# VUmcCGP/wisecondor

Measured on NVIDIA B200. Metric: newref_bin_pairs_per_s, higher is better.
Workload: dtype f64

## Files before the change

### wisecondor_b200/csrc/wc_common.cuh

```cuda
#pragma once
#include <cuda.h>
#include <cuda_runtime.h>
#include <stdint.h>
#include <stdio.h>
#include <string.h>
#include <math.h>
#include <string>
#include <vector>
#include <algorithm>
#include "../../include/wisecondor_b200.h"

void wc_set_error(const char* fmt, ...);

#define WC_CUDA(expr)                                                                                   \
    do {                                                                                                \
        cudaError_t _e = (expr);                                                                        \
        if (_e != cudaSuccess) {                                                                        \
            wc_set_error("%s failed: %s (%s:%d)", #expr, cudaGetErrorString(_e), __FILE__, __LINE__);   \
            return WC_ERR_CUDA;                                                                         \
        }                                                                                               \
    } while (0)

#define WC_CHECK_ARG(cond)                                                                              \
    do {                                                                                                \
        if (!(cond)) {                                                                                  \
            wc_set_error("bad argument: %s (%s:%d)", #cond, __FILE__, __LINE__);                        \
            return WC_ERR_ARG;                                                                          \
        }                                                                                               \
    } while (0)

struct wc_buf {
    void* p = nullptr;
    size_t bytes = 0;
};

enum { WC_NBUF = 56, WC_NPHASE = 12, WC_NCOUNTER = 12 };

enum {
    SLOT_XC = 0, SLOT_NORMS, SLOT_ROWCS, SLOT_ROWCE, SLOT_RBMETA, SLOT_CAND_D, SLOT_CAND_J, SLOT_SEGCNT,
    SLOT_SEGFLAG, SLOT_SLOW, SLOT_SCRATCH, SLOT_IO_X, SLOT_IO_IDX, SLOT_IO_DIST, SLOT_ROWTHR,
    SLOT_IN_KEY, SLOT_IN_J, SLOT_IN_CNT, SLOT_N32, SLOT_F16STAT,
    SLOT_PROF = 20, SLOT_PIV_IDS = 21, SLOT_PIV_X = 22, SLOT_PIV_N = 23, SLOT_PIV_META = 37, SLOT_S_STACK = 38,
    SLOT_T_COPY = 24, SLOT_T_ZT, SLOT_T_RT, SLOT_T_NT, SLOT_T_SD, SLOT_T_FLAGS, SLOT_T_TOTALS, SLOT_T_PROJ,
    SLOT_T_REVCNT = 44, SLOT_T_REVCUR, SLOT_T_DIRTY, SLOT_T_PAIRS,
    SLOT_S_ZC = 32, SLOT_S_META, SLOT_S_STATUS, SLOT_S_RC, SLOT_S_AUX,
    SLOT_P_FIRST = 40,
    SLOT_FIN_J = 48, SLOT_FIN_D, SLOT_FIN_P, SLOT_FIN_GRP
};

struct wc_shard_plan {
    int valid = 0;
    int N = 0, S = 0, k = 0, cap = 0, in_cap = 0, world = 1, rank = 0;
    int nb = 0, bp = 0, b0 = 0, b1 = 0;
    int row0 = 0, row1 = 0, rows_per = 0;
    int nkc = 0, nd_last = 0, extra_h = 0, ld = 0, nstages = 0, nrb = 0, nseg = 0, gridA = 0, gridB = 0;
    size_t Npad = 0, smem = 0, nlistA = 0;
    long long tilesA = 0, tilesB = 0, tiles_plain = 0;
    double mcoef = 0.0, madd = 0.0;
    int f16 = 0, ldh = 0;
    int pivots = 0;
    const double* corrected = nullptr;
    const unsigned long long* thr = nullptr;
    int stage = 0;
};

struct wc_ctx {
    int device = 0;
    int sm_count = 0;
    wc_buf buf[WC_NBUF];
    cudaEvent_t ev[2 * WC_NPHASE];
    double phase_ms[WC_NPHASE];
    long long counter[WC_NCOUNTER];
    const int* zs_npairs_d = nullptr;
    int zs_repeats = 0;
    long long zs_pair_limit = 0, zs_all_pairs = 0;
    int32_t* d2h_idx_h = nullptr; double* d2h_dist_h = nullptr; size_t d2h_rows_done = 0;
    cudaStream_t d2h_stream = nullptr; cudaEvent_t d2h_ev = nullptr;
    void* search_plan = nullptr;
    void (*search_plan_free)(void*) = nullptr;
    unsigned long long sched_hash = 0;
    unsigned timed_mask = 0;
    int k5_stages = 0;
    int k5_group = 0;
    int k5_sym = 8;
    int k5_f16 = 2;
    int k5_f16_checked = 1;
    int k5_pivots = 1;
    unsigned long long piv_hash = 0;
    float* dbg_scores = nullptr;
    int dbg_ld = 0;
    const int* k6_stats_d = nullptr;
    int k6_g4 = 0;
    int k6_parts = 4;
    int k6_select = 1;
    int k6_split = 1;
    int k6_chunk = 0, k6_warps = 0, k6_prod = 0;
    int k5_lag = 0;
    int debug_profile = 0;
    void* encode_tiled = nullptr;
    wc_shard_plan shard;
};

int wc_reserve(wc_ctx* ctx, int slot, size_t bytes, void** out);

__device__ __forceinline__ uint32_t smem_u32(const void* p) {
    return static_cast<uint32_t>(__cvta_generic_to_shared(p));
}

__device__ __forceinline__ void mbar_init(uint64_t* bar, uint32_t count) {
    asm volatile("mbarrier.init.shared::cta.b64 [%0], %1;" ::"r"(smem_u32(bar)), "r"(count) : "memory");
}
__device__ __forceinline__ void mbar_fence_init() {
    asm volatile("fence.mbarrier_init.release.cluster;" ::: "memory");
}
__device__ __forceinline__ void mbar_arrive(uint64_t* bar) {
    asm volatile("mbarrier.arrive.shared::cta.b64 _, [%0];" ::"r"(smem_u32(bar)) : "memory");
}
__device__ __forceinline__ void mbar_arrive_expect_tx(uint64_t* bar, uint32_t bytes) {
    asm volatile("mbarrier.arrive.expect_tx.shared::cta.b64 _, [%0], %1;" ::"r"(smem_u32(bar)), "r"(bytes) : "memory");
}
__device__ __forceinline__ bool mbar_try_wait(uint64_t* bar, uint32_t parity) {
    uint32_t ok;
    asm volatile(
        "{\n"
        ".reg .pred p;\n"
        "mbarrier.try_wait.parity.shared::cta.b64 p, [%1], %2;\n"
        "selp.u32 %0, 1, 0, p;\n"
        "}\n"
        : "=r"(ok)
        : "r"(smem_u32(bar)), "r"(parity)
        : "memory");
    return ok != 0;
}
__device__ __forceinline__ bool mbar_test_wait(uint64_t* bar, uint32_t parity) {
    uint32_t ok;
    asm volatile(
        "{\n"
        ".reg .pred p;\n"
        "mbarrier.test_wait.parity.shared::cta.b64 p, [%1], %2;\n"
        "selp.u32 %0, 1, 0, p;\n"
        "}\n"
        : "=r"(ok)
        : "r"(smem_u32(bar)), "r"(parity)
        : "memory");
    return ok != 0;
}
__device__ __forceinline__ void mbar_wait(uint64_t* bar, uint32_t parity) {
    while (!mbar_try_wait(bar, parity)) {
    }
}
__device__ __forceinline__ void tma_load_2d(void* smem_dst, const CUtensorMap* map, int c0, int c1, uint64_t* bar) {
    asm volatile(
        "cp.async.bulk.tensor.2d.shared::cluster.global.mbarrier::complete_tx::bytes [%0], [%1, {%2, %3}], [%4];" ::"r"(
            smem_u32(smem_dst)),
        "l"(reinterpret_cast<uint64_t>(map)), "r"(c0), "r"(c1), "r"(smem_u32(bar))
        : "memory");
}
__device__ __forceinline__ void tma_prefetch_desc(const CUtensorMap* map) {
    asm volatile("prefetch.tensormap [%0];" ::"l"(reinterpret_cast<uint64_t>(map)) : "memory");
}
__device__ __forceinline__ double lds_f64(uint32_t addr) {
    double v;
    asm volatile("ld.shared.f64 %0, [%1];" : "=d"(v) : "r"(addr));
    return v;
}
__device__ __forceinline__ void lds_v2f64(uint32_t addr, double& v0, double& v1) {
    asm volatile("ld.shared.v2.f64 {%0, %1}, [%2];" : "=d"(v0), "=d"(v1) : "r"(addr));
}
__device__ __forceinline__ void dmma_8x8x4(double& c0, double& c1, double a, double b) {
    asm("mma.sync.aligned.m8n8k4.row.col.f64.f64.f64.f64 {%0,%1}, {%2}, {%3}, {%0,%1};"
                 : "+d"(c0), "+d"(c1)
                 : "d"(a), "d"(b));
}
__device__ __forceinline__ void named_bar_sync(int id, int nthreads) {
    asm volatile("bar.sync %0, %1;" ::"r"(id), "r"(nthreads) : "memory");
}
__device__ __forceinline__ double ld_cg_f64(const double* p) {
    double v;
    asm volatile("ld.global.cg.f64 %0, [%1];" : "=d"(v) : "l"(p));
    return v;
}
__device__ __forceinline__ int ld_cg_s32(const int* p) {
    int v;
    asm volatile("ld.global.cg.s32 %0, [%1];" : "=r"(v) : "l"(p));
    return v;
}
```

### wisecondor_b200/csrc/wc_search.cu

```cuda
#include "wc_common.cuh"
#include <cuda_fp16.h>

namespace {

typedef unsigned long long u64;

constexpr int BM = 128;
constexpr int BN = 128;
constexpr int BK = 16;
constexpr int CONSUMER_WARPS = 8;
constexpr int CONSUMER_THREADS = CONSUMER_WARPS * 32;
constexpr int WROWS = BM / CONSUMER_WARPS;
constexpr int PRODUCER_WARPS = 4;
constexpr int TOPK_THREADS = CONSUMER_THREADS + PRODUCER_WARPS * 32;
constexpr int TILE_BYTES = BM * BK * 8;
constexpr int STAGE_BYTES = 2 * TILE_BYTES;
constexpr int MAX_STAGES = 6;
constexpr int HIST_BINS = 256;
constexpr int FIN_THREADS = 128;
constexpr int FIN_CHUNK = 32;
constexpr int FIN_BUCKETS = 1024;
constexpr int FIN_ECAP = 1360;
constexpr int EXH_THREADS = 256;
constexpr int STG = 128;
// ... 282 lines not shown
            else
                prune_row<32>(rk, rj, n, a.k, w_nrm[rw], a.mcoef, madd_of(a), lane, w_sk, w_sj, &thr, &kept);
            if (lane == 0) {
                if (kept > a.cap - BN) {
                    w_flag[rw] = 1;
                    w_thr[rw] = KEY_NEVER;
                    w_cnt[rw] = 0;
                } else {
                    const int row = a.row_begin + rb * BM + r0w + rw;
                    const u64 other = atomicMin(a.row_thr + (row - a.row_begin), thr);
                    w_thr[rw] = other < thr ? other : thr;
                    w_cnt[rw] = kept;
                }
            }
            __syncwarp();
        }
    };
    auto flush_incoming = [&]() {
        __syncwarp();
        int n = *w_stgc;
        if (n > STG) n = STG;
        for (int e = lane; e < n; e += 32) {
            const uint4 v = w_stg[e];
            const int j = (int)v.z;
            const int w = atomicAdd(a.in_cnt + j, 1);
            if (w < a.in_cap) {
                a.in_key[(size_t)j * a.in_cap + w] = ((u64)v.y << 32) | (u64)v.x;
                a.in_j[(size_t)j * a.in_cap + w] = (int)v.w;
            }
        }
        __syncwarp();
        if (lane == 0) *w_stgc = 0;
        __syncwarp();
    };
    int tcount = 0;
    while (true) {
        if (q >= q1) {
            __syncwarp();
            if (SYM) flush_incoming();
            if (a.final_prune) {
                const unsigned need = __ballot_sync(0xffffffffu, lane < WROWS && w_cnt[lane] > a.k + 24 &&
                                                                     w_cnt[lane] <= a.cap && !w_flag[lane]);
                prune_rows(need, a.cand_key + (size_t)seg * seg_stride, a.cand_j + (size_t)seg * seg_stride);
            }
            if (lane < WROWS) {
                a.seg_cnt[(size_t)seg * BM + r0w + lane] = w_cnt[lane] > a.cap ? a.cap : w_cnt[lane];
                a.seg_flag[(size_t)seg * BM + r0w + lane] = w_flag[lane];
            }
            if (++pi >= pe) break;
            pc = a.pieces + (size_t)pi * 5;
            rb = pc[0]; q = pc[1]; q1 = pc[2]; qs = pc[3]; seg = pc[4];
            skip_lo = a.rb_skip_lo[rb]; skip_n = a.rb_skip_n[rb];
            tl = a.tile_list ? a.tile_list + a.rb_list_off[rb] : nullptr;
            new_piece = true;
            continue;
        }
        if (new_piece) {
            new_piece = false;
            __syncwarp();
            if (lane < WROWS) {
                const int row = a.row_begin + rb * BM + r0w + lane;
                const bool valid = row < a.row_end;
                w_nrm[lane] = valid ? a.norms[row] : 0.0;
                w_thr[lane] = valid ? __ldcg(a.row_thr + (row - a.row_begin)) : KEY_NEVER;
                w_cnt[lane] = 0;
                w_flag[lane] = 0;
            }
#pragma unroll
            for (int mt = 0; mt < 2; ++mt) {
                const int row = a.row_begin + rb * BM + r0w + mt * 8 + pg;
                const bool valid = row < a.row_end;
                my_cs[mt] = valid ? a.row_cs[row] : 0;
                my_ce[mt] = valid ? a.row_ce[row] : 0;
            }
            __syncwarp();
        }
        const int t = tl ? tl[q] : (q < skip_lo ? q : q + skip_n);
        const int col0 = t * BN;
        q += qs;
        if (SYM) {
            __syncwarp();
            cp_async_16(w_ct + 2 * lane, a.col_thr + col0 + 2 * lane);
            cp_async_16(w_ct + 64 + 2 * lane, a.col_thr + col0 + 64 + 2 * lane);
            cp_async_commit();
        }
        u64 shared_thr = ~0ull;
        if (lane < WROWS) {
            const int row = a.row_begin + rb * BM + r0w + lane;
            if (row < a.row_end) shared_thr = __ldcg(a.row_thr + (row - a.row_begin));
        }
        const bool tr_on = a.trace != nullptr && blockIdx.x == 0 && (warp & 3) == 0 && lane == 0 && tcount < 64;
        long long* tr = tr_on ? a.trace + ((size_t)(warp >> 2) * 64 + tcount) * 4 : nullptr;
        ++tcount;
        if (tr_on) tr[0] = clock64();

        double acc[2][16][2];
#pragma unroll
        for (int mt = 0; mt < 2; ++mt)
#pragma unroll
            for (int nt = 0; nt < 16; ++nt) acc[mt][nt][0] = acc[mt][nt][1] = 0.0;

        for (int kc = 0; kc < a.nkc; ++kc) {
            if (!ready) {
                const long long pf_w0 = clock64();
                mbar_wait(&sm.full[stage], phase);
                pf_wait += clock64() - pf_w0;
            }
            const uint32_t base = tiles_u32 + (uint32_t)stage * STAGE_BYTES;
            int nstage = stage + 1;
            uint32_t nphase = phase;
            if (nstage == STAGES) { nstage = 0; nphase ^= 1u; }
            const bool ready_next = mbar_test_wait(&sm.full[nstage], nphase);
            const bool last = kc == a.nkc - 1;
            const int nd = last ? a.nd_last : 2;
#pragma unroll
            for (int h = 0; h < 2; ++h) {
                if (h < nd) {
                    double fa[2][2];
#pragma unroll
                    for (int mt = 0; mt < 2; ++mt) lds_v2f64(base + a_off + mt * 1024 + sw[h], fa[mt][0], fa[mt][1]);
#pragma unroll
                    for (int half = 0; half < 2; ++half) {
                        double fb[8][2];
#pragma unroll
                        for (int i = 0; i < 8; ++i)
                            lds_v2f64(base + b_off + (half * 8 + i) * 1024 + sw[h], fb[i][0], fb[i][1]);
#pragma unroll
                        for (int u = 0; u < 2; ++u)
#pragma unroll
                            for (int mt = 0; mt < 2; ++mt)
#pragma unroll
                                for (int i = 0; i < 8; ++i)
                                    dmma_8x8x4(acc[mt][half * 8 + i][0], acc[mt][half * 8 + i][1], fa[mt][u], fb[i][u]);
                    }
                }
            }
            if (last) {
                double fa[2][2];
#pragma unroll
                for (int mt = 0; mt < 2; ++mt) lds_v2f64(base + a_off + mt * 1024 + swx, fa[mt][0], fa[mt][1]);
#pragma unroll
                for (int half = 0; half < 2; ++half) {
                    double fb[8][2];
#pragma unroll
                    for (int i = 0; i < 8; ++i)
                        lds_v2f64(base + b_off + (half * 8 + i) * 1024 + swx, fb[i][0], fb[i][1]);
#pragma unroll
                    for (int u = 0; u < 2; ++u)
#pragma unroll
                        for (int mt = 0; mt < 2; ++mt)
#pragma unroll
                            for (int i = 0; i < 8; ++i)
                                dmma_8x8x4(acc[mt][half * 8 + i][0], acc[mt][half * 8 + i][1], fa[mt][u], fb[i][1 - u]);
                }
            }
            __syncwarp();
            if (lane == 0) mbar_arrive(&sm.empty[stage]);
            if (gate_left > 0 && --gate_left == 0) {
                if (lane == 0) mbar_arrive(&sm.gate);
                gate_left = -1;
            }
            stage = nstage;
            phase = nphase;
            ready = ready_next;
        }

        const long long pf_e0 = clock64();
        if (tr_on) tr[1] = pf_e0;
        if (lane < WROWS && shared_thr < w_thr[lane]) w_thr[lane] = shared_thr;
        if (SYM) cp_async_wait<0>();
        __syncwarp();
        u64* ck = a.cand_key + (size_t)seg * seg_stride;
        int* cj = a.cand_j + (size_t)seg * seg_stride;
#pragma unroll
        for (int mt = 0; mt < 2; ++mt) {
            const int rw = mt * 8 + pg;
            const u64 thr = w_thr[rw];
            unsigned mask = 0, cmask = 0;
#pragma unroll
            for (int nt = 0; nt < 16; ++nt) {
#pragma unroll
                for (int e = 0; e < 2; ++e) {
                    const u64 bits = (u64)__double_as_longlong(acc[mt][nt][e]);
                    if (bits <= thr) mask |= 1u << (nt * 2 + e);
                    if (SYM && bits <= w_ct[nt * 8 + 4 * e + q4]) cmask |= 1u << (nt * 2 + e);
                }
            }
            if (mask | cmask) {
                u64* tmp = w_sk + lane;
#pragma unroll
                for (int nt = 0; nt < 16; ++nt) {
                    tmp[(nt * 2) * 32] = (u64)__double_as_longlong(acc[mt][nt][0]);
                    tmp[(nt * 2 + 1) * 32] = (u64)__double_as_longlong(acc[mt][nt][1]);
                }
                const int cs = my_cs[mt];
                const unsigned clen = (unsigned)(my_ce[mt] - cs);
                unsigned m2 = mask;
                while (m2) {
                    const int bit = __ffs(m2) - 1;
                    m2 &= m2 - 1;
                    const int cl = (bit >> 1) * 8 + 4 * (bit & 1) + q4;
                    const unsigned hi32 = (unsigned)(tmp[bit * 32] >> 32);
                    if ((hi32 & 0x7ff00000u) == 0x7ff00000u || (unsigned)(col0 + cl - cs) < clen) mask &= ~(1u << bit);
                }
                if (mask) {
                    pf_emit += __popc(mask);
                    int w = atomicAdd(&w_cnt[rw], __popc(mask));
                    u64* rk = ck + (size_t)(r0w + rw) * a.cap;
                    int* rj = cj + (size_t)(r0w + rw) * a.cap;
                    while (mask) {
                        const int bit = __ffs(mask) - 1;
                        mask &= mask - 1;
                        const int cl = (bit >> 1) * 8 + 4 * (bit & 1) + q4;
                        if (w < a.cap) {
                            rk[w] = tmp[bit * 32];
                            rj[w] = col0 + cl;
                        } else {
                            w_flag[rw] = 1;
                        }
                        ++w;
                    }
                }
                if (SYM && cmask) {
                    const int i = a.row_begin + rb * BM + r0w + rw;
                    while (cmask) {
                        const int bit = __ffs(cmask) - 1;
                        cmask &= cmask - 1;
                        const int j = col0 + (bit >> 1) * 8 + 4 * (bit & 1) + q4;
                        const u64 key = tmp[bit * 32];
                        if (((unsigned)(key >> 32) & 0x7ff00000u) == 0x7ff00000u || j >= a.N || i >= a.row_end) continue;
                        if ((unsigned)(j - cs) < clen) continue;
                        const int pos = atomicAdd(w_stgc, 1);
                        if (pos < STG) {
                            w_stg[pos] = make_uint4((unsigned)key, (unsigned)(key >> 32), (unsigned)j, (unsigned)i);
                        } else {
                            const int w = atomicAdd(a.in_cnt + j, 1);
                            if (w < a.in_cap) {
                                a.in_key[(size_t)j * a.in_cap + w] = key;
                                a.in_j[(size_t)j * a.in_cap + w] = i;
                            }
                        }
                        ++pf_emit;
                    }
                }
            }
        }
        __syncwarp();
        if (SYM && *w_stgc >= 32) flush_incoming();
        const long long pf_p0 = clock64();
        pf_epi += pf_p0 - pf_e0;
        if (tr_on) tr[2] = pf_p0;
        prune_rows(__ballot_sync(0xffffffffu, lane < WROWS && w_cnt[lane] > a.cap - BN && !w_flag[lane]), ck, cj);
        pf_prune += clock64() - pf_p0;
        if (tr_on) tr[3] = clock64();
    }
    if (gate_left > 0 && lane == 0) mbar_arrive(&sm.gate);
    __syncwarp();
    if (a.prof != nullptr && warp == 0 && lane == 0) {
        long long* o = a.prof + (size_t)blockIdx.x * 8;
        o[0] = clock64() - pf_t0; o[1] = pf_wait; o[2] = pf_epi; o[3] = pf_prune;
        o[4] = tcount; o[5] = pf_nprune; o[6] = pf_emit; o[7] = 0;
    }
}

#include "wc_search_f16.cuh"
#include "wc_search_tc.cuh"

__global__ void wc_fill_u64_kernel(u64* p, size_t n, u64 v) {
    const size_t i = (size_t)blockIdx.x * blockDim.x + threadIdx.x;
    if (i < n) p[i] = v;
}

__global__ void wc_prepare_kernel(const double* __restrict__ X, int N, int Npad, int S, int ld, int Sx,
                                  double* __restrict__ Xc, double* __restrict__ norms) {
    const int row = (blockIdx.x * blockDim.x + threadIdx.x) >> 5;
    const int lane = threadIdx.x & 31;
    if (row >= Npad) return;
    double* dst = Xc + (size_t)row * ld;
    double acc = 0.0;
    if (row < N) {
        const double* src = X + (size_t)row * S;
        for (int s = lane; s < ld; s += 32) {
            double v = s < S ? src[s] - 1.0 : 0.0;
            dst[s] = v;
            acc = fma(v, v, acc);
        }
    } else {
        for (int s = lane; s < ld; s += 32) dst[s] = 0.0;
    }
#pragma unroll
    for (int o = 16; o > 0; o >>= 1) acc += __shfl_xor_sync(0xffffffffu, acc, o);
    __syncwarp();
    if (lane == 0) {
        norms[row] = row < N ? acc : 0.0;
        dst[Sx] = 1.0;
        dst[Sx + 1] = row < N ? -0.5 * acc : -INFINITY;
    }
}

__device__ __forceinline__ bool pair_less(double da, int ja, double db, int jb) {
    return da < db || (da == db && ja < jb);
}

struct FinArgs {
    const double* X;
    int N, S;
    const double* norms;
    const int* row_cs;
    const int* row_ce;
    int row_begin, row_end;
    const int* rb_seg_first;
    const int* rb_seg_count;
    const u64* cand_key;
    const int* cand_j;
    const int* seg_cnt;
    const int* seg_flag;
    int cap;
    int k;
    int shortcap;
    double mcoef;
    int* idx_out;
    double* dist_out;
    int* slow_list;
    int* slow_count;
    int slow_bias;
    int vec;
    const u64* in_key;
    const int* in_j;
    const int* in_cnt;
    int in_cap;
    double madd;
    const double* madd_p;
    const u64* row_thr;
    int in_nsrc;
    int in_src_rows;
    int* sl_j;
    u64* sl_k;
    int* sl_p;
    int* grp;
    int* grp_count;
    const int* row_list;
    const int* row_count;
    int* stats;
    int* sl_b;
    int* bkt_hist;
    int bkt_shift;
};

template <int FT, bool SPLIT>
__device__ __forceinline__ void finalize_row(const FinArgs& a, const int rloc, unsigned char* fin_raw) {
    constexpr int ecap = FIN_ECAP;
    double* ex_d = reinterpret_cast<double*>(fin_raw + (size_t)ecap * 12);
    int* ex_j = reinterpret_cast<int*>(ex_d + a.shortcap);
    int* hist = ex_j + a.shortcap;
    __shared__ double s_red[2][FT / 32];
    __shared__ int s_total, s_flag, s_p, s_bstar, s_valid;

    const int tid = threadIdx.x, lane = tid & 31, warp = tid >> 5;
    const int row = a.row_begin + rloc;
    const int rb = rloc / BM, rl = rloc % BM;
    const int seg0 = a.rb_seg_first[rb], nseg = a.rb_seg_count[rb];
    int* out_i = a.idx_out + (size_t)rloc * a.k;
    double* out_d = a.dist_out + (size_t)rloc * a.k;

    const int nsrc = nseg + (a.in_key != nullptr ? a.in_nsrc : 0);
    auto source = [&](int s, const u64*& keys, const int*& js, int& flagged) -> int {
        if (s < nseg) {
            const size_t off = ((size_t)(seg0 + s) * BM + rl) * a.cap;
            keys = a.cand_key + off;
            js = a.cand_j + off;
            flagged = a.seg_flag[(size_t)(seg0 + s) * BM + rl];
            return a.seg_cnt[(size_t)(seg0 + s) * BM + rl];
        }
        const size_t r = (size_t)(s - nseg) * a.in_src_rows + rloc;
        keys = a.in_key + r * a.in_cap;
        js = a.in_j + r * a.in_cap;
        const int n = a.in_cnt[r];
        flagged = n > a.in_cap ? 1 : 0;
        return n < a.in_cap ? n : a.in_cap;
    };
    u64* en_k = reinterpret_cast<u64*>(fin_raw);
    int* en_j = reinterpret_cast<int*>(en_k + ecap);
    if (tid == 0) { s_total = 0; s_flag = 0; s_p = 0; s_valid = 0; }
    for (int b = tid; b < HIST_BINS; b += FT) hist[b] = 0;
    const u64 tfinal = a.row_thr != nullptr ? __ldcg(a.row_thr + rloc) : ~0ull;
    __syncthreads();
    for (int s = warp; s < nsrc; s += FT / 32) {
        const u64* cd;
        const int* cjs;
        int fl;
        const int n = source(s, cd, cjs, fl);
        if (fl) { if (lane == 0) s_flag = 1; continue; }
        for (int e0 = 0; e0 < n; e0 += 32) {
            const int e = e0 + lane;
            const u64 key = e < n ? cd[e] : ~0ull;
            const bool keep = e < n && key <= tfinal;
            const unsigned bm = __ballot_sync(0xffffffffu, keep);
            if (bm == 0u) continue;
            int base = 0;
            if (lane == 0) base = atomicAdd(&s_total, __popc(bm));
            base = __shfl_sync(0xffffffffu, base, 0) + __popc(bm & ((1u << lane) - 1u));
            if (keep && base < ecap) {
                en_k[base] = key;
                en_j[base] = cjs[e];
            }
        }
    }
    __syncthreads();
    const int total = s_total;
    if (s_flag) {
        if (tid == 0) {
            a.slow_list[atomicAdd(a.slow_count, 1)] = rloc + a.slow_bias;
            if (SPLIT) a.sl_p[rloc] = -1;
        }
        return;
    }
    if (total == 0) {
        for (int e = tid; e < a.k; e += FT) { out_i[e] = -1; out_d[e] = 1e10; }
        if (SPLIT && tid == 0) a.sl_p[rloc] = -1;
        return;
    }
    const bool in_smem = total <= ecap;
    auto for_each_entry = [&](auto&& f) {
        if (in_smem) {
            for (int e = tid; e < total; e += FT) f(en_k[e], en_j[e]);
        } else {
            for (int s2 = 0; s2 < nsrc; ++s2) {
                const u64* cd;
                const int* cjs;
                int fl;
                const int n = source(s2, cd, cjs, fl);
                for (int e = tid; e < n; e += FT) {
                    const u64 key = cd[e];
                    if (key <= tfinal) f(key, cjs[e]);
                }
            }
        }
    };

    double mn = INFINITY, mx = -INFINITY;
    for_each_entry([&](u64 key, int) {
        const double d = dist_of_key(key);
        mn = fmin(mn, d);
        mx = fmax(mx, d);
    });
    mn = warp_min(mn);
    mx = warp_max(mx);
    if (lane == 0) { s_red[0][warp] = mn; s_red[1][warp] = mx; }
    __syncthreads();
#pragma unroll
    for (int w = 0; w < FT / 32; ++w) { mn = fmin(mn, s_red[0][w]); mx = fmax(mx, s_red[1][w]); }
    const float scale = (mx > mn) ? (float)(HIST_BINS - 1) / (float)(mx - mn) : 0.0f;
    for_each_entry([&](u64 key, int) { atomicAdd(&hist[bucket_of(dist_of_key(key), mn, scale)], 1); });
    __syncthreads();
    if (warp == 0) {
        int c[HIST_BINS / 32], sum = 0;
#pragma unroll
        for (int t = 0; t < HIST_BINS / 32; ++t) { c[t] = hist[lane * (HIST_BINS / 32) + t]; sum += c[t]; }
        int incl = sum;
#pragma unroll
        for (int o = 1; o < 32; o <<= 1) {
            int v = __shfl_up_sync(0xffffffffu, incl, o);
            if (lane >= o) incl += v;
        }
        int run = incl - sum, bl = -1;
#pragma unroll
        for (int t = 0; t < HIST_BINS / 32; ++t) {
            run += c[t];
            if (bl < 0 && run >= a.k) bl = lane * (HIST_BINS / 32) + t;
        }
        unsigned m = __ballot_sync(0xffffffffu, bl >= 0);
        int bstar = HIST_BINS - 1;
        if (m) bstar = __shfl_sync(0xffffffffu, bl, __ffs(m) - 1);
        if (lane == 0) s_bstar = bstar;
    }
    __syncthreads();
    const int bstar = s_bstar;
    double vstar = -INFINITY;
    for_each_entry([&](u64 key, int) {
        const double d = dist_of_key(key);
        if (bucket_of(d, mn, scale) <= bstar) vstar = fmax(vstar, d);
    });
    vstar = warp_max(vstar);
    __syncthreads();
    if (lane == 0) s_red[0][warp] = vstar;
    __syncthreads();
#pragma unroll
    for (int w = 0; w < FT / 32; ++w) vstar = fmax(vstar, s_red[0][w]);
    const double window = vstar + a.mcoef * (a.norms[row] + fabs(vstar)) + madd_of(a);
    for_each_entry([&](u64 key, int j) {
        if (dist_of_key(key) <= window) {
            const int slot = atomicAdd(&s_p, 1);
            if (slot < a.shortcap) ex_j[slot] = j;
        }
    });
    __syncthreads();
    const int p = s_p;
    if (p > a.shortcap) {
        if (tid == 0) {
            a.slow_list[atomicAdd(a.slow_count, 1)] = rloc + a.slow_bias;
            if (SPLIT) a.sl_p[rloc] = -1;
        }
        return;
    }
    if (SPLIT) {
        for (int e = tid; e < p; e += FT) a.sl_j[(size_t)rloc * a.shortcap + e] = ex_j[e];
        if (tid == 0) {
            a.sl_p[rloc] = p;
            const int ng = (p + 31) >> 5;
            int jmin = 0x7fffffff;
            for (int e = 0; e < p; ++e) jmin = min(jmin, ex_j[e]);
            const int bkt = min(jmin >> a.bkt_shift, FIN_BUCKETS - 1);
            a.sl_b[rloc] = bkt;
            atomicAdd(a.bkt_hist + bkt, ng);
            if (a.stats != nullptr) { atomicAdd(a.stats, total); atomicAdd(a.stats + 1, p); }
        }
        return;
    }

    const double* xrow = a.X + (size_t)row * a.S;
    double* xi_s = reinterpret_cast<double*>(fin_raw);
    const bool xi_in_smem = (size_t)a.S * 8 <= (size_t)ecap * 12;
    __syncthreads();
    if (xi_in_smem)
        for (int t = tid; t < a.S; t += FT) xi_s[t] = xrow[t];
    __syncthreads();
    const uint32_t xi_u32 = smem_u32(xi_s);
    for (int c0 = 0; c0 < p; c0 += FT) {
        if (c0 + warp * 32 < p) {
            const bool live = c0 + tid < p;
            const int j = ex_j[live ? c0 + tid : p - 1];
            const double* xr = a.X + (size_t)j * a.S;
            double accd = 0.0;
            int t0 = 0;
            if (a.vec == 4 && xi_in_smem) {
                for (; t0 + 32 <= a.S; t0 += 32) {
                    double v[32];
#pragma unroll
                    for (int u = 0; u < 8; ++u) ldg_nc_v4f64(xr + t0 + 4 * u, v[4 * u], v[4 * u + 1], v[4 * u + 2], v[4 * u + 3]);
                    __syncwarp();
#pragma unroll
                    for (int u = 0; u < 16; ++u) {
                        double x0, x1;
                        lds_v2f64(xi_u32 + (uint32_t)(t0 + 2 * u) * 8u, x0, x1);
                        double d = __dsub_rn(v[2 * u], x0);
                        accd = __dadd_rn(accd, __dmul_rn(d, d));
                        d = __dsub_rn(v[2 * u + 1], x1);
                        accd = __dadd_rn(accd, __dmul_rn(d, d));
                    }
                }
                for (; t0 + 4 <= a.S; t0 += 4) {
                    double v0, v1, v2, v3;
                    ldg_nc_v4f64(xr + t0, v0, v1, v2, v3);
                    double d = __dsub_rn(v0, xi_s[t0]);     accd = __dadd_rn(accd, __dmul_rn(d, d));
                    d = __dsub_rn(v1, xi_s[t0 + 1]);        accd = __dadd_rn(accd, __dmul_rn(d, d));
                    d = __dsub_rn(v2, xi_s[t0 + 2]);        accd = __dadd_rn(accd, __dmul_rn(d, d));
                    d = __dsub_rn(v3, xi_s[t0 + 3]);        accd = __dadd_rn(accd, __dmul_rn(d, d));
                }
            }
            if (xi_in_smem) {
                for (; t0 < a.S; ++t0) {
                    const double d = __dsub_rn(__ldg(xr + t0), xi_s[t0]);
                    accd = __dadd_rn(accd, __dmul_rn(d, d));
                }
            } else {
                for (; t0 < a.S; ++t0) {
                    const double d = __dsub_rn(__ldg(xr + t0), __ldg(xrow + t0));
                    accd = __dadd_rn(accd, __dmul_rn(d, d));
                }
            }
            __syncwarp();
            if (live) {
                const bool ok = accd < 1e10;
                ex_d[c0 + tid] = ok ? accd : INFINITY;
                ex_j[c0 + tid] = ok ? j : 0x7fffffff;
            }
        }
    }
    __syncthreads();

    const int cs = a.row_cs[row], ce = a.row_ce[row];
    int nvalid_local = 0;
    for (int e = tid; e < p; e += FT) {
        const double d = ex_d[e];
        const int j = ex_j[e];
        if (j == 0x7fffffff) continue;
        ++nvalid_local;
        int rank = 0;
        for (int u = 0; u < p; ++u) rank += pair_less(ex_d[u], ex_j[u], d, j) ? 1 : 0;
        if (rank < a.k) {
            out_i[rank] = j >= ce ? j - (ce - cs) : j;
            out_d[rank] = d;
        }
    }
    atomicAdd(&s_valid, nvalid_local);
    __syncthreads();
    for (int e = s_valid + tid; e < a.k; e += FT) { out_i[e] = -1; out_d[e] = 1e10; }
}

template <int FT, bool SPLIT>
__global__ void __launch_bounds__(FT) wc_finalize_kernel(const FinArgs a) {
    extern __shared__ __align__(32) unsigned char fin_raw[];
    if (a.row_list == nullptr) {
        finalize_row<FT, SPLIT>(a, (int)blockIdx.x, fin_raw);
        return;
    }
    const int n = *a.row_count;
    for (int b = blockIdx.x; b < n; b += gridDim.x) {
        finalize_row<FT, SPLIT>(a, a.row_list[b], fin_raw);
        __syncthreads();
    }
}

struct ExhArgs {
    const double* X;
    int N, S;
    const int* row_cs;
    const int* row_ce;
    int row_begin;
    const int* slow_list;
    int list_off;
    double* scratch;
    int k;
    int* idx_out;
    double* dist_out;
};

__global__ void __launch_bounds__(EXH_THREADS) wc_exhaustive_kernel(const ExhArgs a) {
    __shared__ double s_d[EXH_THREADS / 32];
    __shared__ int s_j[EXH_THREADS / 32];
    __shared__ double s_bd;
    __shared__ int s_bj;
    const int tid = threadIdx.x, lane = tid & 31, warp = tid >> 5;
    const int rloc = a.slow_list[a.list_off + blockIdx.x];
    const int row = a.row_begin + rloc;
    const int cs = a.row_cs[row], ce = a.row_ce[row];
    double* dd = a.scratch + (size_t)blockIdx.x * a.N;
    const double* xrow = a.X + (size_t)row * a.S;
    for (int j = tid; j < a.N; j += EXH_THREADS) {
        double acc = INFINITY;
        if (j < cs || j >= ce) {
            const double* xj = a.X + (size_t)j * a.S;
            acc = 0.0;
            for (int s = 0; s < a.S; ++s) {
                double v = __dsub_rn(xj[s], xrow[s]);
                acc = __dadd_rn(acc, __dmul_rn(v, v));
            }
            if (!(acc < 1e10)) acc = INFINITY;
        }
        dd[j] = acc;
    }
    __syncthreads();
    double last_d = -INFINITY;
    int last_j = -1;
    int* out_i = a.idx_out + (size_t)rloc * a.k;
    double* out_d = a.dist_out + (size_t)rloc * a.k;
    for (int t = 0; t < a.k; ++t) {
        double bd = INFINITY;
        int bj = 0x7fffffff;
        for (int j = tid; j < a.N; j += EXH_THREADS) {
            double d = dd[j];
            bool after = d > last_d || (d == last_d && j > last_j);
            if (after && pair_less(d, j, bd, bj)) { bd = d; bj = j; }
        }
#pragma unroll
        for (int o = 16; o > 0; o >>= 1) {
            double od = __shfl_xor_sync(0xffffffffu, bd, o);
            int oj = __shfl_xor_sync(0xffffffffu, bj, o);
            if (pair_less(od, oj, bd, bj)) { bd = od; bj = oj; }
        }
        if (lane == 0) { s_d[warp] = bd; s_j[warp] = bj; }
        __syncthreads();
        if (tid == 0) {
            for (int w = 1; w < EXH_THREADS / 32; ++w)
                if (pair_less(s_d[w], s_j[w], bd, bj)) { bd = s_d[w]; bj = s_j[w]; }
            s_bd = bd;
            s_bj = bj;
            if (bd < INFINITY) {
                out_i[t] = bj >= ce ? bj - (ce - cs) : bj;
                out_d[t] = bd;
            } else {
                out_i[t] = -1;
                out_d[t] = 1e10;
            }
        }
        __syncthreads();
        last_d = s_bd;
        last_j = s_bj;
        if (!(last_d < INFINITY)) {
            for (int e = t + 1 + tid; e < a.k; e += EXH_THREADS) { out_i[e] = -1; out_d[e] = 1e10; }
            break;
        }
    }
}

typedef CUresult (*PFN_encodeTiled)(CUtensorMap*, CUtensorMapDataType, cuuint32_t, void*, const cuuint64_t*,
                                    const cuuint64_t*, const cuuint32_t*, const cuuint32_t*, CUtensorMapInterleave,
                                    CUtensorMapSwizzle, CUtensorMapL2promotion, CUtensorMapFloatOOBfill);

}

namespace {
#include "wc_search_fin.cuh"

struct Piece { int cta, rb, q0, q1, step, seg, pass; };
void schedule_pieces(const std::vector<int>& prefix, int nrb, int grid, int G, bool rounds_on, int pass,
                     std::vector<Piece>& pieces) {
    std::vector<long long> load(grid, 0);
    if (G > grid) G = grid;
    if (G < 1) G = 1;
    const int groups = grid / G;
    const int rounds = rounds_on ? nrb / groups : 0;
    for (int r = 0; r < rounds; ++r)
        for (int g = 0; g < groups; ++g) {
            const int rb = r * groups + g;
            const int nv = prefix[rb + 1] - prefix[rb];
            for (int j = 0; j < G && j < nv; ++j) {
                pieces.push_back({g * G + j, rb, j, nv, G, 0, pass});
                load[g * G + j] += (nv - j + G - 1) / G;
            }
        }
    const int rb_left = rounds * groups;
    long long left = prefix[nrb] - prefix[rb_left];
    if (left > 0) {
        long long lo = 0, hi = 0;
        for (int c = 0; c < grid; ++c) hi = std::max(hi, load[c]);
        hi += left;
        while (lo < hi) {
            const long long mid = (lo + hi) / 2;
            long long cap_sum = 0;
            for (int c = 0; c < grid; ++c) cap_sum += std::max(0ll, mid - load[c]);
            if (cap_sum >= left) hi = mid; else lo = mid + 1;
        }
        int rb = rb_left, q = 0;
        for (int c = 0; c < grid && left > 0; ++c) {
            long long want = std::min(left, std::max(0ll, lo - load[c]));
            while (want > 0) {
                const int nv = prefix[rb + 1] - prefix[rb];
                if (q >= nv) { ++rb; q = 0; continue; }
                const int take = (int)std::min<long long>(want, nv - q);
                pieces.push_back({c, rb, q, q + take, 1, 0, pass});
                load[c] += take;
                q += take;
                want -= take;
                left -= take;
            }
        }
    }
}

void pair_lists(int nb, const std::vector<int>& skip_lo, const std::vector<int>& skip_n, int frac, int b0, int b1,
                std::vector<int>& list_a, std::vector<int>& off_a, std::vector<int>& list_b, std::vector<int>& off_b) {
    auto in_sample = [&](int I, int J) { return I == J || (I + J) % frac == 0; };
    auto valid = [&](int I, int t) { return !(t >= skip_lo[I] && t < skip_lo[I] + skip_n[I]); };
    list_a.clear();
    list_b.clear();
    off_a.assign(b1 - b0 + 1, 0);
    off_b.assign(b1 - b0 + 1, 0);
    for (int I = b0; I < b1; ++I) {
        for (int t = 0; t < nb; ++t)
            if (valid(I, t) && in_sample(I, t)) list_a.push_back(t);
        off_a[I - b0 + 1] = (int)list_a.size();
        for (int dlt = 1; dlt <= nb / 2; ++dlt) {
            if (2 * dlt == nb && I >= nb / 2) continue;
            const int t = (I + dlt) % nb;
            if (valid(I, t) && !in_sample(I, t)) list_b.push_back(t);
        }
        off_b[I - b0 + 1] = (int)list_b.size();
    }
}

void block_skips(int N, const int* chrom_bins_h, int nchrom, std::vector<int>& row_cs, std::vector<int>& row_ce,
                 std::vector<int>& skip_lo, std::vector<int>& skip_n) {
    row_cs.assign(N, 0);
    row_ce.assign(N, 0);
    int pos = 0;
    for (int c = 0; c < nchrom; ++c) {
        for (int i = 0; i < chrom_bins_h[c]; ++i) { row_cs[pos + i] = pos; row_ce[pos + i] = pos + chrom_bins_h[c]; }
        pos += chrom_bins_h[c];
    }
    const int nb = (N + BM - 1) / BM;
    skip_lo.assign(nb, nb);
    skip_n.assign(nb, 0);
    for (int I = 0; I < nb; ++I) {
        const int r0 = I * BM, r1 = std::min(N, r0 + BM) - 1;
        if (row_cs[r0] == row_cs[r1]) {
            const int first = (row_cs[r0] + BN - 1) / BN, last = row_ce[r0] / BN;
            if (last > first) { skip_lo[I] = first; skip_n[I] = last - first; }
        }
    }
}

}


namespace {
int encode_f16_map(wc_ctx* ctx, CUtensorMap* tmap, const void* base, int ldh, size_t rows) {
    if (!ctx->encode_tiled) {
        wc_set_error("cuTensorMapEncodeTiled is not available from this driver");
        return WC_ERR_CUDA;
    }
    cuuint64_t dims[2] = {(cuuint64_t)ldh, (cuuint64_t)rows};
    cuuint64_t strides[1] = {(cuuint64_t)ldh * sizeof(__half)};
    cuuint32_t box[2] = {(cuuint32_t)BKH, BM};
    cuuint32_t estr[2] = {1, 1};
    CUresult r = reinterpret_cast<PFN_encodeTiled>(ctx->encode_tiled)(
        tmap, CU_TENSOR_MAP_DATA_TYPE_FLOAT16, 2, const_cast<void*>(base), dims, strides, box, estr, CU_TENSOR_MAP_INTERLEAVE_NONE,
        CU_TENSOR_MAP_SWIZZLE_128B, CU_TENSOR_MAP_L2_PROMOTION_L2_256B, CU_TENSOR_MAP_FLOAT_OOB_FILL_NONE);
    if (r != CUDA_SUCCESS) {
        wc_set_error("cuTensorMapEncodeTiled failed with CUresult %d", (int)r);
        return WC_ERR_CUDA;
    }
    return WC_OK;
}

int pivot_count(int N, int k) {
    return (k <= 128 && (long long)TC_PIVOTS * 4 <= N) ? TC_PIVOTS : 0;
}

int tc_pivot_pass(wc_ctx* ctx, cudaStream_t stream, const CUtensorMap& tmap_a, TopkArgs ta, const __half* Xh, int ldh, int ldx, int N,
                  int nrb, const std::vector<int>& rb_seg_first, int R) {
    int* ids; __half* P; float* n32p; int* meta;
    int rc;
    if ((rc = wc_reserve(ctx, SLOT_PIV_IDS, (size_t)R * sizeof(int), (void**)&ids))) return rc;
    if ((rc = wc_reserve(ctx, SLOT_PIV_X, (size_t)R * ldh * sizeof(__half), (void**)&P))) return rc;
    if ((rc = wc_reserve(ctx, SLOT_PIV_N, (size_t)R * sizeof(float), (void**)&n32p))) return rc;
    if (R != TC_PIVOTS) { wc_set_error("pivot pass: %d pivots unsupported", R); return WC_ERR_INTERNAL; }
    const int gridP = std::max(1, std::min(ctx->sm_count, nrb));
    std::vector<int> m((size_t)gridP + 1 + (size_t)nrb * 5);
    {
        int w = 0;
        for (int c = 0; c < gridP; ++c) {
            m[c] = w;
            for (int rb = c; rb < nrb; rb += gridP, ++w) {
                int* pc = &m[(size_t)gridP + 1 + (size_t)w * 5];
                pc[0] = rb; pc[1] = 0; pc[2] = R / BN; pc[3] = 1; pc[4] = rb_seg_first[rb];
            }
        }
        m[gridP] = w;
    }
    if ((rc = wc_reserve(ctx, SLOT_PIV_META, m.size() * sizeof(int), (void**)&meta))) return rc;
    unsigned long long h = 1469598103934665603ull;
    for (int v : m) { h ^= (unsigned)v; h *= 1099511628211ull; }
    h ^= (unsigned long long)(uintptr_t)meta;
    if (h != ctx->piv_hash) {
        WC_CUDA(cudaMemcpyAsync(meta, m.data(), m.size() * sizeof(int), cudaMemcpyHostToDevice, stream));
        ctx->piv_hash = h;
    }
    wc_pivot_select_kernel<<<1, 1024, 0, stream>>>(ta.n32, N, R, ids);
    wc_pivot_gather_kernel<<<R, 128, 0, stream>>>(Xh, ldh, ldx, ta.n32, ids, P, n32p);
    WC_CUDA(cudaGetLastError());
    CUtensorMap tmap_p;
    if ((rc = encode_f16_map(ctx, &tmap_p, P, ldh, (size_t)R))) return rc;
    ta.cta_piece_begin = meta; ta.pieces = meta + gridP + 1;
    ta.tile_list = nullptr; ta.rb_list_off = nullptr; ta.final_prune = 1;
    ta.in_key = nullptr; ta.in_j = nullptr; ta.in_cnt = nullptr; ta.in_cap = 0; ta.col_thr = nullptr;
    ta.coln32 = n32p; ta.col_ids = ids; ta.dbg = nullptr; ta.dbg_ld = 0; ta.prof = nullptr; ta.trace = nullptr;
    ta.kb_last = ldh - BKH;
    WC_CUDA(cudaFuncSetAttribute(wc_dist_topk_tc_kernel<2, false>, cudaFuncAttributeMaxDynamicSharedMemorySize, (int)TC_SMEM_BYTES));
    wc_dist_topk_tc_kernel<2, false><<<gridP, TC_THREADS, TC_SMEM_BYTES, stream>>>(tmap_a, tmap_p, ta);
    WC_CUDA(cudaGetLastError());
    return WC_OK;
}
}

extern "C" int wc_debug_sym_plan(int N, const int* chrom_bins_h, int nchrom, int frac, int world, int rank, int grid,
                                 int group, int rounds_on, int* out, long long out_ints, long long* used) {
    WC_CHECK_ARG(N > 0 && chrom_bins_h != nullptr && nchrom > 0 && frac >= 2 && world >= 1 && rank >= 0 && rank < world);
    WC_CHECK_ARG(grid >= 1 && group >= 1 && out != nullptr && used != nullptr);
    long long tot = 0;
    for (int c = 0; c < nchrom; ++c) { WC_CHECK_ARG(chrom_bins_h[c] >= 0); tot += chrom_bins_h[c]; }
    WC_CHECK_ARG(tot == N);
    std::vector<int> row_cs, row_ce, skip_lo, skip_n, la, oa, lb, ob;
    block_skips(N, chrom_bins_h, nchrom, row_cs, row_ce, skip_lo, skip_n);
    const int nb = (N + BM - 1) / BM;
    const int bp = (nb + world - 1) / world;
    const int b0 = std::min(nb, rank * bp), b1 = std::min(nb, b0 + bp), nrb = b1 - b0;
    pair_lists(nb, skip_lo, skip_n, frac, b0, b1, la, oa, lb, ob);
    std::vector<Piece> pa, pb;
    if (!la.empty()) schedule_pieces(oa, nrb, std::max(1, std::min<int>(grid, ((int)la.size() + 7) / 8)), 1, false, 0, pa);
    if (!lb.empty()) schedule_pieces(ob, nrb, std::max(1, std::min<int>(grid, ((int)lb.size() + 7) / 8)), group, rounds_on != 0, 1, pb);
    const long long need = 8 + 2ll * (nrb + 1) + (long long)la.size() + (long long)lb.size() + 5ll * (pa.size() + pb.size()) + 2ll * nb;
    *used = need;
    if (need > out_ints) { wc_set_error("wc_debug_sym_plan: %lld ints needed", need); return WC_ERR_ARG; }
    int* o = out;
    *o++ = nb; *o++ = b0; *o++ = b1; *o++ = (int)la.size(); *o++ = (int)lb.size(); *o++ = (int)pa.size(); *o++ = (int)pb.size(); *o++ = 0;
    for (int v : oa) *o++ = v;
    for (int v : ob) *o++ = v;
    for (int v : la) *o++ = v;
    for (int v : lb) *o++ = v;
    for (const std::vector<Piece>* pv : {&pa, &pb})
        for (const Piece& pc : *pv) { *o++ = pc.cta; *o++ = pc.rb; *o++ = pc.q0; *o++ = pc.q1; *o++ = pc.step; }
    for (int v : skip_lo) *o++ = v;
    for (int v : skip_n) *o++ = v;
    return WC_OK;
}

namespace {
__global__ void wc_f16_margin_kernel(const unsigned long long* __restrict__ stats, int S, double eps16, double* __restrict__ out) {
    const double nmax = __longlong_as_double((long long)stats[0]);
    out[0] = 2.0 * eps16 * nmax + ldexp(1.0, -20) * sqrt((double)S * nmax);
}
}

namespace {
struct SearchPlan {
    unsigned long long key = 0, content_hash = 0;
    bool valid = false;
    std::vector<int> row_cs, row_ce, skip_lo, skip_n, rb_seg_first, rb_seg_count, cta_piece_begin, piece_tab, sym_tab;
    int nrb = 0, total_tiles = 0, grid = 0, sym = 0, sym_frac = 0, gridA = 0, gridB = 0, grid0 = 0, nseg = 0;
    long long tilesA = 0, tilesB = 0;
    size_t listA_size = 0;
};
// ... 136 lines not shown
            if (pc.pass == 0) { per_cta0[pc.cta + 1]++; ++n0; } else { per_cta1[pc.cta + 1]++; }
            piece_tab[(size_t)i * 5 + 0] = pc.rb;
            piece_tab[(size_t)i * 5 + 1] = pc.q0;
            piece_tab[(size_t)i * 5 + 2] = pc.q1;
            piece_tab[(size_t)i * 5 + 3] = pc.step;
            piece_tab[(size_t)i * 5 + 4] = pc.seg;
        }
        for (int c = 0; c < grid0; ++c) per_cta0[c + 1] += per_cta0[c];
        cta_piece_begin = per_cta0;
        if (sym) {
            per_cta1[0] = n0;
            for (int c = 0; c < gridB; ++c) per_cta1[c + 1] += per_cta1[c];
            cta_piece_begin.insert(cta_piece_begin.end(), per_cta1.begin(), per_cta1.end());
        }
    }
    std::vector<int> sym_tab;
    if (sym) {
        sym_tab.insert(sym_tab.end(), offA.begin(), offA.end());
        sym_tab.insert(sym_tab.end(), offB.begin(), offB.end());
        sym_tab.insert(sym_tab.end(), listA.begin(), listA.end());
        sym_tab.insert(sym_tab.end(), listB.begin(), listB.end());
    }

    P.row_cs.swap(row_cs); P.row_ce.swap(row_ce); P.skip_lo.swap(skip_lo); P.skip_n.swap(skip_n);
    P.rb_seg_first.swap(rb_seg_first); P.rb_seg_count.swap(rb_seg_count); P.cta_piece_begin.swap(cta_piece_begin);
    P.piece_tab.swap(piece_tab); P.sym_tab.swap(sym_tab);
    P.nrb = nrb; P.total_tiles = total_tiles; P.grid = grid; P.sym = sym ? 1 : 0; P.sym_frac = sym_frac; P.gridA = gridA; P.gridB = gridB;
    P.grid0 = grid0; P.nseg = nseg; P.tilesA = tilesA; P.tilesB = tilesB; P.listA_size = listA.size();
    {
        unsigned long long h = 1469598103934665603ull;
        auto mix = [&](const void* p, size_t bytes) {
            const unsigned char* c = static_cast<const unsigned char*>(p);
            for (size_t i = 0; i < bytes; ++i) { h ^= c[i]; h *= 1099511628211ull; }
        };
        mix(chrom_bins_h, (size_t)nchrom * sizeof(int));
        const int dims[8] = {N, row_begin, row_end, grid0, nrb, nseg, sym ? sym_frac : 0, gridB};
        mix(dims, sizeof(dims));
        mix(P.piece_tab.data(), P.piece_tab.size() * sizeof(int));
        mix(P.cta_piece_begin.data(), P.cta_piece_begin.size() * sizeof(int));
        P.content_hash = h;
    }
    P.key = plan_key;
    P.valid = true;
    }
    const std::vector<int>& row_cs = P.row_cs; const std::vector<int>& row_ce = P.row_ce;
    const std::vector<int>& skip_lo = P.skip_lo; const std::vector<int>& skip_n = P.skip_n;
    const std::vector<int>& rb_seg_first = P.rb_seg_first; const std::vector<int>& rb_seg_count = P.rb_seg_count;
    const std::vector<int>& cta_piece_begin = P.cta_piece_begin; const std::vector<int>& piece_tab = P.piece_tab;
    const std::vector<int>& sym_tab = P.sym_tab;
    const int nrb = P.nrb, total_tiles = P.total_tiles, grid = P.grid, gridA = P.gridA, gridB = P.gridB, grid0 = P.grid0, nseg = P.nseg;
    const bool sym = P.sym != 0;
    const int sym_frac = P.sym_frac;
    const long long tilesA = P.tilesA, tilesB = P.tilesB;
    const size_t listA_size = P.listA_size;

    double* Xc; double* norms; int* d_row_cs; int* d_row_ce; int* d_meta;
    u64* cand_key; int* cand_j; int* seg_cnt; int* seg_flag; int* slow;
    int rc;
    if ((rc = wc_reserve(ctx, SLOT_XC, std::max(Npad * ld * sizeof(double), Npad * ((size_t)(S + 4 + 2 * BKH) / BKH * BKH + BKH) * sizeof(__half)), (void**)&Xc))) return rc;
    if ((rc = wc_reserve(ctx, SLOT_NORMS, Npad * sizeof(double), (void**)&norms))) return rc;
    if ((rc = wc_reserve(ctx, SLOT_ROWCS, (size_t)N * sizeof(int), (void**)&d_row_cs))) return rc;
    if ((rc = wc_reserve(ctx, SLOT_ROWCE, (size_t)N * sizeof(int), (void**)&d_row_ce))) return rc;
    const size_t meta_ints = 4 * (size_t)nrb + cta_piece_begin.size() + piece_tab.size() + sym_tab.size();
    if ((rc = wc_reserve(ctx, SLOT_RBMETA, meta_ints * sizeof(int), (void**)&d_meta))) return rc;
    const size_t cand_n = (size_t)std::max(nseg, 1) * BM * cap;
    if ((rc = wc_reserve(ctx, SLOT_CAND_D, cand_n * sizeof(u64), (void**)&cand_key))) return rc;
    if ((rc = wc_reserve(ctx, SLOT_CAND_J, cand_n * sizeof(int), (void**)&cand_j))) return rc;
    if ((rc = wc_reserve(ctx, SLOT_SEGCNT, (size_t)std::max(nseg, 1) * BM * sizeof(int), (void**)&seg_cnt))) return rc;
    if ((rc = wc_reserve(ctx, SLOT_SEGFLAG, (size_t)std::max(nseg, 1) * BM * sizeof(int), (void**)&seg_flag))) return rc;
    if ((rc = wc_reserve(ctx, SLOT_SLOW, ((size_t)rows + 1) * sizeof(int), (void**)&slow))) return rc;
    u64* row_thr;
    const size_t thr_n = (size_t)nrb * BM + BN;
    if ((rc = wc_reserve(ctx, SLOT_ROWTHR, thr_n * sizeof(u64), (void**)&row_thr))) return rc;
    u64* in_key = nullptr; int* in_j = nullptr; int* in_cnt = nullptr;
    int in_cap = 0;
    if (sym) {
        in_cap = 256;
        while (in_cap < 2 * k * sym_frac) in_cap *= 2;
        if ((rc = wc_reserve(ctx, SLOT_IN_KEY, (size_t)rows * in_cap * sizeof(u64), (void**)&in_key))) return rc;
        if ((rc = wc_reserve(ctx, SLOT_IN_J, (size_t)rows * in_cap * sizeof(int), (void**)&in_j))) return rc;
        if ((rc = wc_reserve(ctx, SLOT_IN_CNT, (size_t)rows * sizeof(int), (void**)&in_cnt))) return rc;
    }
    int* d_skip_lo = d_meta;
    int* d_skip_n = d_skip_lo + nrb;
    int* d_seg_first = d_skip_n + nrb;
    int* d_seg_count = d_seg_first + nrb;
    int* d_cta_piece = d_seg_count + nrb;
    int* d_pieces = d_cta_piece + cta_piece_begin.size();
    int* d_sym = d_pieces + piece_tab.size();

    {
        unsigned long long h = P.content_hash;
        const unsigned long long ptrs[2] = {(unsigned long long)(uintptr_t)d_row_cs, (unsigned long long)(uintptr_t)d_meta};
        for (int i = 0; i < 2; ++i) { h ^= ptrs[i]; h *= 1099511628211ull; }
        if (h != ctx->sched_hash) {
            WC_CUDA(cudaMemcpyAsync(d_row_cs, row_cs.data(), (size_t)N * sizeof(int), cudaMemcpyHostToDevice, stream));
            WC_CUDA(cudaMemcpyAsync(d_row_ce, row_ce.data(), (size_t)N * sizeof(int), cudaMemcpyHostToDevice, stream));
            WC_CUDA(cudaMemcpyAsync(d_skip_lo, skip_lo.data(), (size_t)nrb * sizeof(int), cudaMemcpyHostToDevice, stream));
            WC_CUDA(cudaMemcpyAsync(d_skip_n, skip_n.data(), (size_t)nrb * sizeof(int), cudaMemcpyHostToDevice, stream));
            WC_CUDA(cudaMemcpyAsync(d_seg_first, rb_seg_first.data(), (size_t)nrb * sizeof(int), cudaMemcpyHostToDevice, stream));
            WC_CUDA(cudaMemcpyAsync(d_seg_count, rb_seg_count.data(), (size_t)nrb * sizeof(int), cudaMemcpyHostToDevice, stream));
            WC_CUDA(cudaMemcpyAsync(d_cta_piece, cta_piece_begin.data(), cta_piece_begin.size() * sizeof(int), cudaMemcpyHostToDevice, stream));
            WC_CUDA(cudaMemcpyAsync(d_pieces, piece_tab.data(), piece_tab.size() * sizeof(int), cudaMemcpyHostToDevice, stream));
            if (sym)
                WC_CUDA(cudaMemcpyAsync(d_sym, sym_tab.data(), sym_tab.size() * sizeof(int), cudaMemcpyHostToDevice, stream));
            ctx->sched_hash = h;
        }
    }
    WC_CUDA(cudaMemsetAsync(slow, 0, sizeof(int), stream));
    WC_CUDA(cudaMemsetAsync(seg_cnt, 0, (size_t)std::max(nseg, 1) * BM * sizeof(int), stream));
    WC_CUDA(cudaMemsetAsync(seg_flag, 0, (size_t)std::max(nseg, 1) * BM * sizeof(int), stream));
    if (sym) WC_CUDA(cudaMemsetAsync(in_cnt, 0, (size_t)rows * sizeof(int), stream));

    bool f16 = ctx->k5_f16 != 0;
    const bool tc = ctx->k5_f16 == 2;
    const int ldh = tc ? (S + 4 + BKH - 1) / BKH * BKH : (S + BKH - 1) / BKH * BKH;
    const int ldx = tc ? ldh + BKH : ldh;
    float* n32 = nullptr;
    double nmax = 0.0;
    const double eps16 = ldexp(1.0, -10) * (1.0 + ldexp(1.0, -11)) + (tc ? 2.0 : 1.0) * (double)ldh * ldexp(1.0, -23) +
                         (tc ? ldexp(1.0, -20) : ldexp(1.0, -21));
    const unsigned long long* f16_stats_d = nullptr;
    WC_CUDA(cudaEventRecord(ctx->ev[0], stream));
    if (f16) {
        unsigned long long* stats;
        if ((rc = wc_reserve(ctx, SLOT_N32, Npad * sizeof(float), (void**)&n32))) return rc;
        if ((rc = wc_reserve(ctx, SLOT_F16STAT, 4 * sizeof(unsigned long long), (void**)&stats))) return rc;
        WC_CUDA(cudaMemsetAsync(stats, 0, 2 * sizeof(unsigned long long), stream));
        wc_prepare_f16_kernel<<<(int)((Npad * 32 + 255) / 256), 256, 0, stream>>>(corrected_d, N, (int)Npad, S, ldh, ldx, tc ? 1 : 0,
                                                                                  reinterpret_cast<__half*>(Xc), norms, n32, stats);
        WC_CUDA(cudaGetLastError());
        if (ctx->k5_f16_checked != 0) {
            f16_stats_d = stats;
            wc_f16_margin_kernel<<<1, 1, 0, stream>>>(stats, S, eps16, reinterpret_cast<double*>(stats + 2));
        } else {
            unsigned long long st_h[2] = {0, 0};
            WC_CUDA(cudaMemcpyAsync(st_h, stats, sizeof(st_h), cudaMemcpyDeviceToHost, stream));
            WC_CUDA(cudaStreamSynchronize(stream));
            memcpy(&nmax, &st_h[0], sizeof(double));
            if (st_h[1] != 0) f16 = false;
        }
    }
    if (!f16) {
        const int blocks = (int)((Npad * 32 + 255) / 256);
        wc_prepare_kernel<<<blocks, 256, 0, stream>>>(corrected_d, N, (int)Npad, S, ld, Sx, Xc, norms);
    }
    WC_CUDA(cudaGetLastError());
    WC_CUDA(cudaEventRecord(ctx->ev[1], stream));
    const double filt_mcoef = f16 ? 2.0 * eps16 : mcoef;
    const double filt_madd = f16 ? 2.0 * eps16 * nmax + ldexp(1.0, -20) * sqrt((double)S * nmax) : 0.0;

    CUtensorMap tmap;
    {
        if (!ctx->encode_tiled) {
            wc_set_error("cuTensorMapEncodeTiled is not available from this driver");
            return WC_ERR_CUDA;
        }
        cuuint64_t dims[2] = {(cuuint64_t)(f16 ? ldx : ld), (cuuint64_t)Npad};
        cuuint64_t strides[1] = {f16 ? (cuuint64_t)ldx * sizeof(__half) : (cuuint64_t)ld * sizeof(double)};
        cuuint32_t box[2] = {(cuuint32_t)(f16 ? BKH : BK), BM};
        cuuint32_t estr[2] = {1, 1};
        CUresult r = reinterpret_cast<PFN_encodeTiled>(ctx->encode_tiled)(
            &tmap, f16 ? CU_TENSOR_MAP_DATA_TYPE_FLOAT16 : CU_TENSOR_MAP_DATA_TYPE_FLOAT64, 2, Xc, dims, strides, box, estr,
            CU_TENSOR_MAP_INTERLEAVE_NONE, CU_TENSOR_MAP_SWIZZLE_128B, CU_TENSOR_MAP_L2_PROMOTION_L2_256B,
            CU_TENSOR_MAP_FLOAT_OOB_FILL_NONE);
        if (r != CUDA_SUCCESS) {
            wc_set_error("cuTensorMapEncodeTiled failed with CUresult %d", (int)r);
            return WC_ERR_CUDA;
        }
    }
    TopkArgs ta;
    ta.norms = norms; ta.row_cs = d_row_cs; ta.row_ce = d_row_ce; ta.N = N;
    ta.row_begin = row_begin; ta.row_end = row_end; ta.nkc = nkc; ta.nd_last = nd_last; ta.extra_h = extra_h;
    ta.rb_skip_lo = d_skip_lo; ta.rb_skip_n = d_skip_n; ta.nrb = nrb;
    ta.cta_piece_begin = d_cta_piece; ta.pieces = d_pieces;
    ta.cand_key = cand_key; ta.cand_j = cand_j; ta.seg_cnt = seg_cnt; ta.seg_flag = seg_flag;
    ta.cap = cap; ta.k = k; ta.mcoef = filt_mcoef; ta.tau_init = f16 ? 3e38 : 1e10 * (1.0 + 1e-6);
    ta.row_thr = row_thr;
    ta.lag = ctx->k5_lag;
    ta.nstages = cap <= 512 ? (sym ? 4 : 5) : 3;
    if (f16) { ta.nstages = 4; ta.nkc = ldh / BKH; }
    ta.kb_last = f16 ? (tc ? ldh : ldh - BKH) : 0;
    if (ctx->k5_stages >= 3 && ctx->k5_stages <= MAX_STAGES) ta.nstages = ctx->k5_stages;
    ta.tile_list = nullptr; ta.rb_list_off = nullptr; ta.final_prune = sym ? 1 : 0;
    ta.in_key = in_key; ta.in_j = in_j; ta.in_cnt = in_cnt; ta.in_cap = in_cap; ta.col_thr = row_thr;
    ta.madd = filt_madd; ta.n32 = n32;
    ta.madd_p = f16_stats_d != nullptr ? reinterpret_cast<const double*>(f16_stats_d + 2) : nullptr;
    ta.dbg = f16 && tc ? ctx->dbg_scores : nullptr; ta.dbg_ld = ctx->dbg_ld;
    ta.prof = nullptr;
    ta.trace = nullptr;
    const int grid_prof = sym ? std::max(gridA, gridB) : grid;
    if (ctx->debug_profile) {
        if ((rc = wc_reserve(ctx, SLOT_PROF, ((size_t)grid_prof * 8 + 512) * sizeof(long long), (void**)&ta.prof))) return rc;
        WC_CUDA(cudaMemsetAsync(ta.prof, 0, ((size_t)grid_prof * 8 + 512) * sizeof(long long), stream));
        ta.trace = ta.prof + (size_t)grid_prof * 8;
    }
    const size_t topk_smem_legacy = f16
        ? (size_t)ta.nstages * STAGE_BYTES + sizeof(TopkState) + (size_t)CONSUMER_WARPS * F16_SCRATCH +
              (size_t)CONSUMER_WARPS * (BN * sizeof(u64) + STG * sizeof(uint4) + (2 * BN + 32) * sizeof(float))
        : (size_t)ta.nstages * STAGE_BYTES + sizeof(TopkState) +
              (size_t)CONSUMER_WARPS * std::max<size_t>((size_t)cap * 12, 8192) +
              (sym ? (size_t)CONSUMER_WARPS * (BN * sizeof(u64) + STG * sizeof(uint4)) : 0);
    const bool use_tc = f16 && tc;
    const size_t topk_smem = use_tc ? TC_SMEM_BYTES : topk_smem_legacy;
    if (topk_smem > 227 * 1024) { wc_set_error("K5 shared memory %zu exceeds 227 KiB", topk_smem); return WC_ERR_INTERNAL; }
    const bool dbg = use_tc && ta.dbg != nullptr;
    {
        const int sm_bytes = (int)topk_smem;
        if (use_tc) {
            WC_CUDA(cudaFuncSetAttribute(wc_dist_topk_tc_kernel<0, false>, cudaFuncAttributeMaxDynamicSharedMemorySize, sm_bytes));
            WC_CUDA(cudaFuncSetAttribute(wc_dist_topk_tc_kernel<1, false>, cudaFuncAttributeMaxDynamicSharedMemorySize, sm_bytes));
            if (dbg) {
                WC_CUDA(cudaFuncSetAttribute(wc_dist_topk_tc_kernel<0, true>, cudaFuncAttributeMaxDynamicSharedMemorySize, sm_bytes));
                WC_CUDA(cudaFuncSetAttribute(wc_dist_topk_tc_kernel<1, true>, cudaFuncAttributeMaxDynamicSharedMemorySize, sm_bytes));
            }
        } else if (f16) {
            WC_CUDA(cudaFuncSetAttribute(wc_dist_topk_f16_kernel<false>, cudaFuncAttributeMaxDynamicSharedMemorySize, sm_bytes));
            WC_CUDA(cudaFuncSetAttribute(wc_dist_topk_f16_kernel<true>, cudaFuncAttributeMaxDynamicSharedMemorySize, sm_bytes));
        } else {
            WC_CUDA(cudaFuncSetAttribute(wc_dist_topk_kernel<false>, cudaFuncAttributeMaxDynamicSharedMemorySize, sm_bytes));
            WC_CUDA(cudaFuncSetAttribute(wc_dist_topk_kernel<true>, cudaFuncAttributeMaxDynamicSharedMemorySize, sm_bytes));
        }
    }
    wc_fill_u64_kernel<<<(unsigned)((rows + 255) / 256), 256, 0, stream>>>(row_thr, (size_t)rows, host_key_of_tau(ta.tau_init));
    wc_fill_u64_kernel<<<(unsigned)((thr_n - rows + 255) / 256), 256, 0, stream>>>(row_thr + rows, thr_n - (size_t)rows, KEY_NEVER);
    WC_CUDA(cudaEventRecord(ctx->ev[2], stream));
    ta.coln32 = n32; ta.col_ids = nullptr;
    auto launch = [&](bool symmetric, int g) {
        if (use_tc) {
            auto kern = symmetric ? (dbg ? wc_dist_topk_tc_kernel<1, true> : wc_dist_topk_tc_kernel<1, false>)
                                  : (dbg ? wc_dist_topk_tc_kernel<0, true> : wc_dist_topk_tc_kernel<0, false>);
            kern<<<g, TC_THREADS, topk_smem, stream>>>(tmap, tmap, ta);
        } else if (f16) {
            if (symmetric) wc_dist_topk_f16_kernel<true><<<g, TOPK_THREADS, topk_smem, stream>>>(tmap, ta);
            else wc_dist_topk_f16_kernel<false><<<g, TOPK_THREADS, topk_smem, stream>>>(tmap, ta);
        } else {
            if (symmetric) wc_dist_topk_kernel<true><<<g, TOPK_THREADS, topk_smem, stream>>>(tmap, ta);
            else wc_dist_topk_kernel<false><<<g, TOPK_THREADS, topk_smem, stream>>>(tmap, ta);
        }
    };
    long long pivot_launches = 0;
    const int R = (use_tc && !dbg && ctx->k5_pivots != 0 && rows >= 2 * BM) ? pivot_count(N, k) : 0;
    if (R > 0) {
        if ((rc = tc_pivot_pass(ctx, stream, tmap, ta, reinterpret_cast<const __half*>(Xc), ldh, ldx, N, nrb, rb_seg_first, R))) return rc;
        pivot_launches = 3;
    }
    WC_CUDA(cudaEventRecord(ctx->ev[17], stream));
    if (!sym) {
        launch(false, grid);
    } else {
        const int nb1 = nrb + 1;
        ta.tile_list = d_sym + 2 * nb1;
        ta.rb_list_off = d_sym;
        launch(false, gridA);
        WC_CUDA(cudaGetLastError());
        WC_CUDA(cudaEventRecord(ctx->ev[16], stream));
        ta.tile_list = d_sym + 2 * nb1 + (int)listA_size;
        ta.rb_list_off = d_sym + nb1;
        ta.cta_piece_begin = d_cta_piece + (gridA + 1);
        launch(true, gridB);
    }
    WC_CUDA(cudaGetLastError());
    WC_CUDA(cudaEventRecord(ctx->ev[3], stream));

    FinArgs fa;
    fa.X = corrected_d; fa.N = N; fa.S = S; fa.norms = norms; fa.row_cs = d_row_cs; fa.row_ce = d_row_ce;
    fa.row_begin = row_begin; fa.row_end = row_end; fa.rb_seg_first = d_seg_first; fa.rb_seg_count = d_seg_count;
    fa.cand_key = cand_key; fa.cand_j = cand_j; fa.seg_cnt = seg_cnt; fa.seg_flag = seg_flag; fa.cap = cap; fa.k = k;
    fa.shortcap = k <= (f16 ? 96 : 128) ? 256 : 512;
    fa.mcoef = filt_mcoef; fa.idx_out = idx_d; fa.dist_out = dist_d; fa.slow_list = slow + 1; fa.slow_count = slow;
    fa.vec = (S % 4 == 0 && (reinterpret_cast<uintptr_t>(corrected_d) & 31) == 0) ? 4 : 1;
    fa.in_key = in_key; fa.in_j = in_j; fa.in_cnt = in_cnt; fa.in_cap = in_cap; fa.in_nsrc = 1; fa.in_src_rows = 0;
    fa.madd = filt_madd; fa.row_thr = row_thr; fa.madd_p = ta.madd_p;
    fa.slow_bias = 0;
    WC_CUDA(cudaEventRecord(ctx->ev[4], stream));
    long long fin_launches = 0;
    const int nparts = (ctx->d2h_idx_h != nullptr && rows >= 16 * BM) ? std::max(1, ctx->k6_parts) : 1;
    ctx->d2h_rows_done = 0;
    for (int pi = 0, r0 = 0; pi < nparts; ++pi) {
        const int r1 = pi + 1 == nparts ? (int)rows : (int)((long long)rows * (pi + 1) / nparts) / BM * BM;
        if (r1 <= r0) continue;
        FinArgs f = fa;
        const int hb = r0 / BM;
        f.row_begin = row_begin + r0; f.row_end = row_begin + r1;
        f.rb_seg_first += hb; f.rb_seg_count += hb;
        f.idx_out += (size_t)r0 * k; f.dist_out += (size_t)r0 * k;
        f.slow_bias = r0;
        if (f.row_thr != nullptr) f.row_thr += r0;
        if (f.in_key != nullptr) { f.in_key += (size_t)r0 * in_cap; f.in_j += (size_t)r0 * in_cap; f.in_cnt += r0; }
        long long l = 0;
        if ((rc = launch_finalize(ctx, stream, f, r1 - r0, f16 != 0, &l))) return rc;
        fin_launches += l;
        if (pi + 1 < nparts) {
            WC_CUDA(cudaEventRecord(ctx->d2h_ev, stream));
            WC_CUDA(cudaStreamWaitEvent(ctx->d2h_stream, ctx->d2h_ev, 0));
            WC_CUDA(cudaMemcpyAsync(ctx->d2h_idx_h + (size_t)r0 * k, idx_d + (size_t)r0 * k, (size_t)(r1 - r0) * k * sizeof(int32_t), cudaMemcpyDeviceToHost, ctx->d2h_stream));
            WC_CUDA(cudaMemcpyAsync(ctx->d2h_dist_h + (size_t)r0 * k, dist_d + (size_t)r0 * k, (size_t)(r1 - r0) * k * sizeof(double), cudaMemcpyDeviceToHost, ctx->d2h_stream));
            ctx->d2h_rows_done = (size_t)r1;
        }
        r0 = r1;
    }
    WC_CUDA(cudaEventRecord(ctx->ev[5], stream));

    int nslow = 0, k6_stats[4] = {0, 0, 0, 0};
    WC_CUDA(cudaMemcpyAsync(&nslow, slow, sizeof(int), cudaMemcpyDeviceToHost, stream));
    if (ctx->k6_stats_d != nullptr) WC_CUDA(cudaMemcpyAsync(k6_stats, ctx->k6_stats_d, 4 * sizeof(int), cudaMemcpyDeviceToHost, stream));
    unsigned long long f16_flag = 0;
    if (f16_stats_d != nullptr) WC_CUDA(cudaMemcpyAsync(&f16_flag, f16_stats_d + 1, sizeof(f16_flag), cudaMemcpyDeviceToHost, stream));
    WC_CUDA(cudaStreamSynchronize(stream));
    if (f16_flag != 0) {
        const int keep = ctx->k5_f16;
        ctx->k5_f16 = 0;
        rc = wc_newref_topk(ctx, corrected_d, N, S, chrom_bins_h, nchrom, row_begin, row_end, refsize, idx_d, dist_d, stream_v);
        ctx->k5_f16 = keep;
        return rc;
    }
    ctx->counter[8] = k6_stats[1];
    ctx->counter[9] = k6_stats[2];
    ctx->counter[10] = k6_stats[0];
    ctx->counter[11] = k6_stats[3];
    long long launches = (sym ? 5 : 4) + pivot_launches + fin_launches;
    if (nslow > 0) {
        ctx->d2h_rows_done = 0;
        const int batch = 64;
        double* scratch;
        if ((rc = wc_reserve(ctx, SLOT_SCRATCH, (size_t)std::min(nslow, batch) * N * sizeof(double), (void**)&scratch)))
            return rc;
        WC_CUDA(cudaEventRecord(ctx->ev[6], stream));
        for (int off = 0; off < nslow; off += batch) {
            ExhArgs ea;
            ea.X = corrected_d; ea.N = N; ea.S = S; ea.row_cs = d_row_cs; ea.row_ce = d_row_ce; ea.row_begin = row_begin;
            ea.slow_list = slow + 1; ea.list_off = off; ea.scratch = scratch; ea.k = k; ea.idx_out = idx_d; ea.dist_out = dist_d;
            wc_exhaustive_kernel<<<std::min(batch, nslow - off), EXH_THREADS, 0, stream>>>(ea);
            ++launches;
        }
        WC_CUDA(cudaGetLastError());
        WC_CUDA(cudaEventRecord(ctx->ev[7], stream));
        WC_CUDA(cudaStreamSynchronize(stream));
    }
    float ms;
    WC_CUDA(cudaEventElapsedTime(&ms, ctx->ev[0], ctx->ev[1])); ctx->phase_ms[0] = ms;
    WC_CUDA(cudaEventElapsedTime(&ms, ctx->ev[2], ctx->ev[3])); ctx->phase_ms[1] = ms;
    ctx->phase_ms[8] = 0.0;
    if (sym) { WC_CUDA(cudaEventElapsedTime(&ms, ctx->ev[2], ctx->ev[16])); ctx->phase_ms[8] = ms; }
    WC_CUDA(cudaEventElapsedTime(&ms, ctx->ev[4], ctx->ev[5])); ctx->phase_ms[2] = ms;
    if (nslow > 0) { WC_CUDA(cudaEventElapsedTime(&ms, ctx->ev[6], ctx->ev[7])); ctx->phase_ms[3] = ms; }
    ctx->counter[0] = launches;
    ctx->counter[1] = nslow;
    ctx->counter[2] = total_tiles;
    ctx->counter[3] = sym ? tilesA + tilesB : total_tiles;
    ctx->counter[4] = sym ? std::max(gridA, gridB) : grid;
    ctx->counter[7] = (f16 ? ctx->k5_f16 : 0) | (R << 4);
    return WC_OK;
}

extern "C" int wc_newref_topk_host(wc_ctx* ctx, const double* corrected_h, int N, int S, const int* chrom_bins_h,
                                   int nchrom, int row_begin, int row_end, int refsize, int32_t* idx_h,
                                   double* dist_h) {
    WC_CHECK_ARG(ctx != nullptr && corrected_h != nullptr);
    WC_CHECK_ARG(N > 0 && S > 0 && refsize >= 1);
    WC_CHECK_ARG(row_begin >= 0 && row_begin <= row_end && row_end <= N);
    WC_CUDA(cudaSetDevice(ctx->device));
    const size_t rows = (size_t)(row_end - row_begin);
    double* X; int32_t* idx; double* dist;
    int rc;
    if ((rc = wc_reserve(ctx, SLOT_IO_X, (size_t)N * S * sizeof(double), (void**)&X))) return rc;
    if ((rc = wc_reserve(ctx, SLOT_IO_IDX, std::max<size_t>(rows, 1) * refsize * sizeof(int32_t), (void**)&idx))) return rc;
    if ((rc = wc_reserve(ctx, SLOT_IO_DIST, std::max<size_t>(rows, 1) * refsize * sizeof(double), (void**)&dist))) return rc;
    WC_CUDA(cudaMemcpyAsync(X, corrected_h, (size_t)N * S * sizeof(double), cudaMemcpyHostToDevice, 0));
    if (rows) WC_CHECK_ARG(idx_h != nullptr && dist_h != nullptr);
    if (ctx->d2h_stream == nullptr) {
        WC_CUDA(cudaStreamCreateWithFlags(&ctx->d2h_stream, cudaStreamNonBlocking));
        WC_CUDA(cudaEventCreateWithFlags(&ctx->d2h_ev, cudaEventDisableTiming));
    }
    ctx->d2h_idx_h = idx_h; ctx->d2h_dist_h = dist_h; ctx->d2h_rows_done = 0;
    rc = wc_newref_topk(ctx, X, N, S, chrom_bins_h, nchrom, row_begin, row_end, refsize, idx, dist, nullptr);
    const size_t done = rc ? 0 : ctx->d2h_rows_done;
    ctx->d2h_idx_h = nullptr; ctx->d2h_dist_h = nullptr; ctx->d2h_rows_done = 0;
    if (rc) { cudaStreamSynchronize(ctx->d2h_stream); return rc; }
    if (done == 0) WC_CUDA(cudaStreamSynchronize(ctx->d2h_stream));
    if (rows) {
        WC_CUDA(cudaMemcpyAsync(idx_h + done * refsize, idx + done * refsize, (rows - done) * refsize * sizeof(int32_t), cudaMemcpyDeviceToHost, 0));
        WC_CUDA(cudaMemcpyAsync(dist_h + done * refsize, dist + done * refsize, (rows - done) * refsize * sizeof(double), cudaMemcpyDeviceToHost, 0));
        WC_CUDA(cudaStreamSynchronize(0));
        WC_CUDA(cudaStreamSynchronize(ctx->d2h_stream));
    }
    return WC_OK;
}

#include "wc_search_shard.cuh"

extern "C" int wc_debug_profile(wc_ctx* ctx, int enable, long long* out_h, int max_ctas) {
    WC_CHECK_ARG(ctx != nullptr);
    ctx->debug_profile = enable;
    if (out_h == nullptr || max_ctas <= 0) return 0;
    int grid = (int)ctx->counter[4];
    if (grid > max_ctas) grid = max_ctas;
    if (grid <= 0 || ctx->buf[SLOT_PROF].p == nullptr) return 0;
    WC_CUDA(cudaMemcpy(out_h, ctx->buf[SLOT_PROF].p, (size_t)grid * 8 * sizeof(long long), cudaMemcpyDeviceToHost));
    if (max_ctas >= grid + 64)
        WC_CUDA(cudaMemcpy(out_h + (size_t)grid * 8, (long long*)ctx->buf[SLOT_PROF].p + (size_t)ctx->counter[4] * 8,
                           512 * sizeof(long long), cudaMemcpyDeviceToHost));
    return grid;
}

extern "C" int wc_debug_filter_scores(wc_ctx* ctx, float* out_d, int ld) {
    WC_CHECK_ARG(ctx != nullptr && (out_d == nullptr || ld > 0));
    ctx->dbg_scores = out_d;
    ctx->dbg_ld = out_d ? ld : 0;
    return WC_OK;
}

extern "C" int wc_debug_pivot_select(wc_ctx* ctx, const float* n32_d, int N, int R, int* ids_d) {
    WC_CHECK_ARG(ctx != nullptr && n32_d != nullptr && ids_d != nullptr && N > 0 && R > 0 && R <= N);
    WC_CUDA(cudaSetDevice(ctx->device));
    wc_pivot_select_kernel<<<1, 1024>>>(n32_d, N, R, ids_d);
    WC_CUDA(cudaGetLastError());
    WC_CUDA(cudaDeviceSynchronize());
    return WC_OK;
}

extern "C" int wc_set_option(wc_ctx* ctx, const char* key, double value) {
    WC_CHECK_ARG(ctx != nullptr && key != nullptr);
    if (strcmp(key, "k5_lag") == 0) {
        WC_CHECK_ARG(value >= 0 && value <= MAX_STAGES - 2);
        ctx->k5_lag = (int)value;
        return WC_OK;
    }
    if (strcmp(key, "k5_group") == 0) {
        WC_CHECK_ARG(value >= 0 && value <= 64);
        ctx->k5_group = (int)value;
        return WC_OK;
    }
    if (strcmp(key, "k5_sym") == 0) {
        if (value != 0 && (value < 2 || value > 64)) { wc_set_error("k5_sym must be 0 or 2..64"); return WC_ERR_ARG; }
        ctx->k5_sym = (int)value;
        return WC_OK;
    }
    if (strcmp(key, "k5_f16") == 0) {
        WC_CHECK_ARG(value == 0 || value == 1 || value == 2);
        ctx->k5_f16 = (int)value;
        return WC_OK;
    }
    if (strcmp(key, "k5_pivots") == 0) {
        ctx->k5_pivots = value != 0 ? 1 : 0;
        return WC_OK;
    }
    if (strcmp(key, "k6_split") == 0) { ctx->k6_split = value != 0 ? 1 : 0; return WC_OK; }
    if (strcmp(key, "k6_g4") == 0) { ctx->k6_g4 = value != 0 ? 1 : 0; return WC_OK; }
    if (strcmp(key, "k6_select") == 0) { ctx->k6_select = value != 0 ? 1 : 0; return WC_OK; }
    if (strcmp(key, "k6_parts") == 0) { WC_CHECK_ARG(value >= 1 && value <= 16); ctx->k6_parts = (int)value; return WC_OK; }
    if (strcmp(key, "k6_chunk") == 0) { WC_CHECK_ARG(value >= 0 && value <= 480); ctx->k6_chunk = (int)value; return WC_OK; }
    if (strcmp(key, "k6_warps") == 0) { WC_CHECK_ARG(value >= 0 && value <= 16); ctx->k6_warps = (int)value; return WC_OK; }
    if (strcmp(key, "k6_prod") == 0) { WC_CHECK_ARG(value >= 0 && value <= 8); ctx->k6_prod = (int)value; return WC_OK; }
    if (strcmp(key, "k5_stages") == 0) {
        WC_CHECK_ARG(value == 0 || (value >= 3 && value <= MAX_STAGES));
        ctx->k5_stages = (int)value;
        return WC_OK;
    }
    wc_set_error("unknown option %s", key);
    return WC_ERR_ARG;
}
```

### wisecondor_b200/csrc/wc_search_fin.cuh

```cuda
#pragma once

constexpr int SEL_WARPS = 4;
constexpr int SEL_ECAP = 1024;
constexpr int SEL_EPL = SEL_ECAP / 32;
constexpr int SEL_U = 4;
constexpr int SEL_MAXSRC = 255;
constexpr size_t SEL_WARP_BYTES = (size_t)SEL_ECAP * 12 + (SEL_MAXSRC + 1) * 4 + 12;
constexpr size_t SEL_WARP_STRIDE = (SEL_WARP_BYTES + 15) / 16 * 16;

__global__ void __launch_bounds__(SEL_WARPS * 32) wc_fin_select_kernel(const FinArgs a, int* __restrict__ big_list,
                                                                       int* __restrict__ big_count, int* __restrict__ stats) {
    extern __shared__ __align__(16) unsigned char sel_raw[];
    const int lane = threadIdx.x & 31, warp = threadIdx.x >> 5;
    const int rloc = blockIdx.x * SEL_WARPS + warp;
    const int rows = a.row_end - a.row_begin;
    if (rloc >= rows) return;
    u64* en_k = reinterpret_cast<u64*>(sel_raw + (size_t)warp * SEL_WARP_STRIDE);
    int* en_j = reinterpret_cast<int*>(en_k + SEL_ECAP);
    int* pre = en_j + SEL_ECAP;
    const int row = a.row_begin + rloc;
    const int rb = rloc / BM, rl = rloc % BM;
    const int seg0 = a.rb_seg_first[rb], nseg = a.rb_seg_count[rb];
    const int nsrc = nseg + (a.in_key != nullptr ? a.in_nsrc : 0);
    int* out_i = a.idx_out + (size_t)rloc * a.k;
    double* out_d = a.dist_out + (size_t)rloc * a.k;
    auto to_big = [&]() {
        if (lane == 0) {
            big_list[atomicAdd(big_count, 1)] = rloc;
            a.sl_p[rloc] = -1;
        }
    };
    if (nsrc > SEL_MAXSRC) { to_big(); return; }
    int flagged = 0;
    for (int s0 = 0; s0 < nsrc; s0 += 32) {
        const int s = s0 + lane;
        int n = 0;
        if (s < nsrc) {
            if (s < nseg) {
                n = a.seg_cnt[(size_t)(seg0 + s) * BM + rl];
                flagged |= a.seg_flag[(size_t)(seg0 + s) * BM + rl];
            } else {
                n = a.in_cnt[(size_t)(s - nseg) * a.in_src_rows + rloc];
                if (n > a.in_cap) { flagged = 1; n = a.in_cap; }
            }
        }
        int incl = n;
#pragma unroll
        for (int o = 1; o < 32; o <<= 1) {
            const int v = __shfl_up_sync(0xffffffffu, incl, o);
            if (lane >= o) incl += v;
        }
        const int base = s0 == 0 ? 0 : pre[s0];
        if (s < nsrc) pre[s + 1] = base + incl;
        if (s0 == 0 && lane == 0) pre[0] = 0;
        __syncwarp();
    }
    if (__any_sync(0xffffffffu, flagged != 0)) {
        if (lane == 0) {
            a.slow_list[atomicAdd(a.slow_count, 1)] = rloc + a.slow_bias;
            a.sl_p[rloc] = -1;
        }
        return;
    }
    const int total_raw = pre[nsrc];
    const u64 tfinal = a.row_thr != nullptr ? __ldcg(a.row_thr + rloc) : ~0ull;
    int kept = 0;
    for (int t0 = 0; t0 < total_raw; t0 += 32 * SEL_U) {
        u64 key[SEL_U];
        int jj[SEL_U];
#pragma unroll
        for (int u = 0; u < SEL_U; ++u) {
            const int t = t0 + u * 32 + lane;
            key[u] = ~0ull;
            jj[u] = 0;
            if (t < total_raw) {
                int lo = 0, hi = nsrc;
                while (hi - lo > 1) {
                    const int m = (lo + hi) >> 1;
                    if (pre[m] <= t) lo = m; else hi = m;
                }
                const int e = t - pre[lo];
                size_t off;
                const u64* kb;
                const int* jb;
                if (lo < nseg) {
                    off = ((size_t)(seg0 + lo) * BM + rl) * a.cap + e;
                    kb = a.cand_key;
                    jb = a.cand_j;
                } else {
                    off = ((size_t)(lo - nseg) * a.in_src_rows + rloc) * a.in_cap + e;
                    kb = a.in_key;
                    jb = a.in_j;
                }
                key[u] = kb[off];
                jj[u] = jb[off];
            }
        }
#pragma unroll
        for (int u = 0; u < SEL_U; ++u) {
            const bool keep = t0 + u * 32 + lane < total_raw && key[u] <= tfinal;
            const unsigned bm = __ballot_sync(0xffffffffu, keep);
            const int pos = kept + __popc(bm & ((1u << lane) - 1u));
            if (keep && pos < SEL_ECAP) {
                en_k[pos] = key[u];
                en_j[pos] = jj[u];
            }
            kept += __popc(bm);
        }
    }
    if (kept > SEL_ECAP) { to_big(); return; }
    if (kept == 0) {
        for (int e = lane; e < a.k; e += 32) { out_i[e] = -1; out_d[e] = 1e10; }
        if (lane == 0) a.sl_p[rloc] = -1;
        return;
    }
    __syncwarp();
    u64 d[SEL_EPL];
#pragma unroll
    for (int t = 0; t < SEL_EPL; ++t) d[t] = t * 32 + lane < kept ? en_k[t * 32 + lane] : ~0ull;
    u64 lo = ~0ull, hi = 0ull;
#pragma unroll
    for (int t = 0; t < SEL_EPL; ++t) {
        if (t * 32 + lane < kept) {
            lo = d[t] < lo ? d[t] : lo;
            hi = d[t] > hi ? d[t] : hi;
        }
    }
    lo = warp_min_u64(lo);
    hi = warp_max_u64(hi);
    u64 blo = lo, bhi = hi, cut = hi;
    int c_hi = kept;
    for (int it = 0; it < 70 && c_hi > a.k; ++it) {
        if (bhi - blo < 2) break;
        const u64 mid = blo + ((bhi - blo) >> 1);
        int c = 0;
#pragma unroll
        for (int t = 0; t < SEL_EPL; ++t) c += d[t] <= mid ? 1 : 0;
#pragma unroll
        for (int o = 16; o > 0; o >>= 1) c += __shfl_xor_sync(0xffffffffu, c, o);
        if (c >= a.k) { bhi = mid; c_hi = c; cut = mid; } else { blo = mid; }
    }
    u64 vstar = 0ull;
#pragma unroll
    for (int t = 0; t < SEL_EPL; ++t)
        if (d[t] <= cut && d[t] > vstar) vstar = d[t];
    vstar = warp_max_u64(vstar);
    const double dv = dist_of_key(vstar);
    double window = fmax(dv, 0.0) + a.mcoef * (a.norms[row] + fabs(dv)) + madd_of(a);
    if (!(window > 1e-300)) window = 1e-300;
    const u64 wkey = key_of_tau(window);
    int p = 0, jmin = 0x7fffffff;
#pragma unroll
    for (int t = 0; t < SEL_EPL; ++t) {
        const bool keep = t * 32 + lane < kept && d[t] <= wkey;
        const unsigned bm = __ballot_sync(0xffffffffu, keep);
        const int pos = p + __popc(bm & ((1u << lane) - 1u));
        if (keep && pos < a.shortcap) {
            const int j = en_j[t * 32 + lane];
            a.sl_j[(size_t)rloc * a.shortcap + pos] = j;
            jmin = min(jmin, j);
        }
        p += __popc(bm);
    }
#pragma unroll
    for (int o = 16; o > 0; o >>= 1) jmin = min(jmin, __shfl_xor_sync(0xffffffffu, jmin, o));
    if (lane == 0) {
        if (p > a.shortcap) {
            a.slow_list[atomicAdd(a.slow_count, 1)] = rloc + a.slow_bias;
            a.sl_p[rloc] = -1;
        } else {
            a.sl_p[rloc] = p;
            const int bkt = min(jmin >> a.bkt_shift, FIN_BUCKETS - 1);
            a.sl_b[rloc] = bkt;
            atomicAdd(a.bkt_hist + bkt, (p + 31) >> 5);
            if (stats != nullptr) { atomicAdd(stats, kept); atomicAdd(stats + 1, p); atomicMax(stats + 2, kept); }
        }
    }
}

constexpr int SELH_WARPS = 8;
constexpr int SELH_BINS = 1024;

__global__ void __launch_bounds__(SELH_WARPS * 32, 5) wc_fin_select_hist_kernel(const FinArgs a, int* __restrict__ big_list,
                                                                            int* __restrict__ big_count, int* __restrict__ stats) {
    __shared__ int s_hist[SELH_WARPS][SELH_BINS];
    __shared__ int s_pre[SELH_WARPS][SEL_MAXSRC + 1];
    const int lane = threadIdx.x & 31, warp = threadIdx.x >> 5;
    const int rloc = blockIdx.x * SELH_WARPS + warp;
    const int rows = a.row_end - a.row_begin;
    if (rloc >= rows) return;
    int* hist = s_hist[warp];
    int* pre = s_pre[warp];
    const int row = a.row_begin + rloc;
    const int rb = rloc / BM, rl = rloc % BM;
    const int seg0 = a.rb_seg_first[rb], nseg = a.rb_seg_count[rb];
    const int nsrc = nseg + (a.in_key != nullptr ? a.in_nsrc : 0);
    int* out_i = a.idx_out + (size_t)rloc * a.k;
    double* out_d = a.dist_out + (size_t)rloc * a.k;
    if (nsrc > SEL_MAXSRC) {
        if (lane == 0) { big_list[atomicAdd(big_count, 1)] = rloc; a.sl_p[rloc] = -1; }
        return;
    }
    for (int b = lane; b < SELH_BINS; b += 32) hist[b] = 0;
    int flagged = 0;
    for (int s0 = 0; s0 < nsrc; s0 += 32) {
        const int s = s0 + lane;
        int n = 0;
        if (s < nsrc) {
            if (s < nseg) {
                n = a.seg_cnt[(size_t)(seg0 + s) * BM + rl];
                flagged |= a.seg_flag[(size_t)(seg0 + s) * BM + rl];
            } else {
                n = a.in_cnt[(size_t)(s - nseg) * a.in_src_rows + rloc];
                if (n > a.in_cap) { flagged = 1; n = a.in_cap; }
            }
        }
        int incl = n;
#pragma unroll
        for (int o = 1; o < 32; o <<= 1) {
            const int v = __shfl_up_sync(0xffffffffu, incl, o);
            if (lane >= o) incl += v;
        }
        const int base = s0 == 0 ? 0 : pre[s0];
        if (s < nsrc) pre[s + 1] = base + incl;
        if (s0 == 0 && lane == 0) pre[0] = 0;
        __syncwarp();
    }
    if (__any_sync(0xffffffffu, flagged != 0)) {
        if (lane == 0) { a.slow_list[atomicAdd(a.slow_count, 1)] = rloc + a.slow_bias; a.sl_p[rloc] = -1; }
        return;
    }
    const u64 tfinal = a.row_thr != nullptr ? __ldcg(a.row_thr + rloc) : ~0ull;
    auto sweep = [&](auto&& f) {
        int s = 0, e0 = 0, ns = nsrc > 0 ? pre[1] : 0;
        bool more = true;
        while (more) {
            u64 key[SEL_U];
            int jj[SEL_U];
            bool ok[SEL_U];
#pragma unroll
            for (int u = 0; u < SEL_U; ++u) {
                while (s < nsrc && e0 >= ns) { ++s; e0 = 0; ns = s < nsrc ? pre[s + 1] - pre[s] : 0; }
                key[u] = ~0ull;
                jj[u] = 0;
                ok[u] = false;
                if (s < nsrc) {
                    const int e = e0 + lane;
                    if (e < ns) {
                        ok[u] = true;
                        if (s < nseg) {
                            const size_t off = ((size_t)(seg0 + s) * BM + rl) * a.cap + e;
                            key[u] = a.cand_key[off];
                            jj[u] = a.cand_j[off];
                        } else {
                            const size_t off = ((size_t)(s - nseg) * a.in_src_rows + rloc) * a.in_cap + e;
                            key[u] = a.in_key[off];
                            jj[u] = a.in_j[off];
                        }
                    }
                    e0 += 32;
                } else {
                    more = false;
                }
            }
#pragma unroll
            for (int u = 0; u < SEL_U; ++u) f(key[u], jj[u], ok[u]);
        }
    };
    double d0 = 0.0, dmax = dist_of_key(tfinal);
    if (!(dmax < 1e10)) {
        const double cut = 1e10 + a.mcoef * (a.norms[row] + 1e10) + madd_of(a);
        double mn = INFINITY, mx = -INFINITY;
        sweep([&](u64 key, int, bool valid) {
            const double d = dist_of_key(key);
            if (valid && key <= tfinal && d <= cut) { mn = fmin(mn, d); mx = fmax(mx, d); }
        });
#pragma unroll
        for (int o = 16; o > 0; o >>= 1) {
            mn = fmin(mn, __shfl_xor_sync(0xffffffffu, mn, o));
            mx = fmax(mx, __shfl_xor_sync(0xffffffffu, mx, o));
        }
        if (mx >= mn) { d0 = mn; dmax = mx; } else { dmax = 0.0; }
    }
    const float scale = dmax - d0 > 1e-5 * fabs(dmax) ? (float)SELH_BINS / (float)(dmax - d0) : 0.0f;
    auto bucket = [&](double d) -> int {
        const float x = (float)(d - d0) * scale;
        return x < (float)SELH_BINS ? (x >= 0.0f ? (int)x : 0) : SELH_BINS - 1;
    };
    int kept = 0;
    sweep([&](u64 key, int, bool valid) {
        const bool live = valid && key <= tfinal;
        if (live) atomicAdd(&hist[bucket(dist_of_key(key))], 1);
        kept += __popc(__ballot_sync(0xffffffffu, live));
    });
    if (kept == 0) {
        for (int e = lane; e < a.k; e += 32) { out_i[e] = -1; out_d[e] = 1e10; }
        if (lane == 0) a.sl_p[rloc] = -1;
        return;
    }
    __syncwarp();
    auto kth_bucket = [&](int kk, int& below) -> int {
        constexpr int PER = SELH_BINS / 32;
        static_assert(PER % 32 == 0, "one bank per lane in the rotated read");
        int sum = 0;
#pragma unroll 8
        for (int t = 0; t < PER; ++t) sum += hist[lane * PER + ((t + lane) & (PER - 1))];
        int incl = sum;
#pragma unroll
        for (int o = 1; o < 32; o <<= 1) {
            const int v = __shfl_up_sync(0xffffffffu, incl, o);
            if (lane >= o) incl += v;
        }
        const unsigned m = __ballot_sync(0xffffffffu, incl >= kk);
        below = 0;
        if (!m) return -1;
        const int lstar = __ffs(m) - 1;
        int base = __shfl_sync(0xffffffffu, incl - sum, lstar);
        for (int r = 0; r < PER / 32; ++r) {
            const int v = hist[lstar * PER + r * 32 + lane];
            int inc2 = v;
#pragma unroll
            for (int o = 1; o < 32; o <<= 1) {
                const int w = __shfl_up_sync(0xffffffffu, inc2, o);
                if (lane >= o) inc2 += w;
            }
            const unsigned m2 = __ballot_sync(0xffffffffu, base + inc2 >= kk);
            if (m2) {
                const int l2 = __ffs(m2) - 1;
                below = base + __shfl_sync(0xffffffffu, inc2 - v, l2);
                return lstar * PER + r * 32 + l2;
            }
            base += __shfl_sync(0xffffffffu, inc2, 31);
        }
        return -1;
    };
    int below = 0;
    int bstar = kth_bucket(a.k, below);
    const bool refine = bstar >= 0 && bstar < SELH_BINS - 1 && scale > 0.0f;
    double vstar = dmax;
    if (refine) vstar = fmin(dmax, d0 + (double)(__fdividef((float)(bstar + 1), scale) * (1.0f + 8.0f * 1.1920929e-7f)));
    auto window_key = [&](double v) -> u64 {
        double window = fmax(v, 0.0) + a.mcoef * (a.norms[row] + fabs(v)) + madd_of(a);
        if (!(window > 1e-300)) window = 1e-300;
        const u64 wk = key_of_tau(window);
        return wk > tfinal ? tfinal : wk;
    };
    const u64 wkey = window_key(vstar);
    const int edge_cnt = refine ? hist[bucket(dist_of_key(wkey))] : 0;
    __syncwarp();
    for (int bb = lane; bb < SELH_BINS; bb += 32) hist[bb] = 0;
    __syncwarp();
    const double dscale = (double)scale;
    u64* my_k = a.sl_k + (size_t)rloc * a.shortcap;
    int* my_j = a.sl_j + (size_t)rloc * a.shortcap;
    int p = 0, jmin = 0x7fffffff;
    sweep([&](u64 key, int j, bool valid) {
        const bool keep = valid && key <= wkey;
        const unsigned bm = __ballot_sync(0xffffffffu, keep);
        const int pos = p + __popc(bm & ((1u << lane) - 1u));
        if (keep && pos < a.shortcap) {
            my_j[pos] = j;
            my_k[pos] = key;
            jmin = min(jmin, j);
        }
        p += __popc(bm);
        if (refine && keep) {
            const double d = dist_of_key(key);
            if (bucket(d) == bstar) {
                const double f = ((d - d0) * dscale - (double)bstar) * (double)SELH_BINS;
                atomicAdd(&hist[f < (double)SELH_BINS ? (f >= 0.0 ? (int)f : 0) : SELH_BINS - 1], 1);
            }
        }
    });
    if (p > a.shortcap) {
        if (lane == 0) {
            a.slow_list[atomicAdd(a.slow_count, 1)] = rloc + a.slow_bias;
            a.sl_p[rloc] = -1;
        }
        return;
    }
    __syncwarp();
    if (refine && p > a.k && ((p - 1) >> 5) != ((max(a.k, p - 2 * edge_cnt - 2) - 1) >> 5)) {
        int below2 = 0;
        const int sstar = kth_bucket(a.k - below, below2);
        if (sstar >= 0 && sstar < SELH_BINS - 1) {
            const double v2 = d0 + ((double)bstar + ((double)(sstar + 1) + 1e-3) / (double)SELH_BINS) / dscale;
            const u64 wkey2 = window_key(fmin(vstar, v2));
            if (wkey2 < wkey) {
                int q = 0;
                jmin = 0x7fffffff;
                for (int e0 = 0; e0 < p; e0 += 32) {
                    const int e = e0 + lane;
                    const bool keep = e < p && __ldcg(my_k + e) <= wkey2;
                    const int j = e < p ? __ldcg(my_j + e) : 0;
                    __syncwarp();
                    const unsigned bm = __ballot_sync(0xffffffffu, keep);
                    if (keep) {
                        my_j[q + __popc(bm & ((1u << lane) - 1u))] = j;
                        jmin = min(jmin, j);
                    }
                    q += __popc(bm);
                }
                p = q;
            }
        }
    }
#pragma unroll
    for (int o = 16; o > 0; o >>= 1) jmin = min(jmin, __shfl_xor_sync(0xffffffffu, jmin, o));
    if (lane == 0) {
        a.sl_p[rloc] = p;
        const int bkt = min(jmin >> a.bkt_shift, FIN_BUCKETS - 1);
        a.sl_b[rloc] = bkt;
        atomicAdd(a.bkt_hist + bkt, (p + 31) >> 5);
        if (stats != nullptr) { atomicAdd(stats, kept); atomicAdd(stats + 1, p); atomicMax(stats + 2, kept); }
    }
}

__global__ void __launch_bounds__(FIN_BUCKETS) wc_fin_bucket_scan_kernel(int* __restrict__ hist, int* __restrict__ total) {
    __shared__ int s_w[32];
    const int tid = threadIdx.x, lane = tid & 31, warp = tid >> 5;
    const int v = hist[tid];
    int incl = v;
#pragma unroll
    for (int o = 1; o < 32; o <<= 1) {
        const int t = __shfl_up_sync(0xffffffffu, incl, o);
        if (lane >= o) incl += t;
    }
    if (lane == 31) s_w[warp] = incl;
    __syncthreads();
    int base = 0;
    for (int w = 0; w < warp; ++w) base += s_w[w];
    hist[tid] = base + incl - v;
    if (tid == FIN_BUCKETS - 1) *total = base + incl;
}

__global__ void wc_fin_bucket_scatter_kernel(int rows, const int* __restrict__ sl_p, const int* __restrict__ sl_b,
                                             int* __restrict__ cursor, int* __restrict__ grp) {
    const int r = blockIdx.x * blockDim.x + threadIdx.x;
    if (r >= rows) return;
    const int p = sl_p[r];
    if (p <= 0) return;
    const int ng = (p + 31) >> 5;
    const int base = atomicAdd(cursor + sl_b[r], ng);
    for (int g = 0; g < ng; ++g) grp[base + g] = (r << 4) | g;
}

struct RescoreArgs {
    const double* X;
    int S;
    int row_begin;
    int shortcap;
    const int* sl_j;
    double* sl_d;
    const int* sl_p;
    const int* grp;
    const int* grp_count;
    int C;
    int nchunks;
    int stride;
    int nslot;
    int gstride;
    int slot_bytes;
};

constexpr int RS_HEADER = 1024;
constexpr int RS_MAX_SLOTS = 64;

__device__ __forceinline__ void bulk_g2s(uint32_t dst, const void* src, uint32_t bytes, uint64_t* bar) {
    asm volatile("cp.async.bulk.shared::cluster.global.mbarrier::complete_tx::bytes [%0], [%1], %2, [%3];" ::"r"(dst),
                 "l"(src), "r"(bytes), "r"(smem_u32(bar))
                 : "memory");
}

__device__ __forceinline__ void tma_gather4(uint32_t dst, const CUtensorMap* map, int col, int r0, int r1, int r2, int r3, uint64_t* bar) {
    asm volatile(
        "cp.async.bulk.tensor.2d.shared::cluster.global.tile::gather4.mbarrier::complete_tx::bytes [%0], [%1, {%2, %3, %4, %5, %6}], [%7];" ::"r"(dst),
        "l"(reinterpret_cast<uint64_t>(map)), "r"(col), "r"(r0), "r"(r1), "r"(r2), "r"(r3), "r"(smem_u32(bar))
        : "memory");
}
constexpr int RS_G4_SHIFT = 8;

template <int W, int R, bool G4>
__global__ void __launch_bounds__((W + W * R) * 32, 1) wc_fin_rescore_kernel(const __grid_constant__ CUtensorMap xmap, const RescoreArgs a) {
    extern __shared__ __align__(128) unsigned char rs_raw[];
    uint64_t* full = reinterpret_cast<uint64_t*>(rs_raw);
    uint64_t* empty = full + RS_MAX_SLOTS;
    const uint32_t slots_u32 = smem_u32(rs_raw + RS_HEADER);
    const int tid = threadIdx.x, lane = tid & 31, warp = tid >> 5;
    const int nslot = a.nslot;
    const int D = nslot / W;
    const uint32_t slot_bytes = G4 ? (uint32_t)a.slot_bytes : 33u * (uint32_t)a.stride;
    if (tid == 0) {
        for (int s = 0; s < nslot; ++s) { mbar_init(&full[s], 1); mbar_init(&empty[s], 32); }
        mbar_fence_init();
        if (G4) tma_prefetch_desc(&xmap);
    }
    __syncthreads();
    const int ngroups = *a.grp_count;
    const int grid = gridDim.x, b = blockIdx.x;
    const int per_wave = W * grid;
    const int nfull = ngroups / per_wave;
    const int rem = ngroups - nfull * per_wave;
    const int nact = rem > b ? (rem - b + grid - 1) / grid : 0;
    const int nwaves = nfull + (nact > 0 ? 1 : 0);
    const int nchunks = a.nchunks, C = a.C;
    const size_t row_bytes = (size_t)a.S * 8;

    if (warp < W) {
        const int w = warp;
        for (int wave = 0; wave < nwaves; ++wave) {
            const int wact = wave < nfull ? W : nact;
            if (w >= wact) break;
            const int desc = a.grp[(size_t)(wave * W + w) * grid + b];
            const int rloc = desc >> 4, gi = desc & 15;
            const int p = a.sl_p[rloc];
            const int cnt = min(32, p - gi * 32);
            const int mylane = lane < cnt ? lane : cnt - 1;
            double acc = 0.0;
            const int k0 = wave * nchunks;
            for (int c = 0; c < nchunks; ++c) {
                const int use = (k0 + c) / D, slot = w * D + (k0 + c) - use * D;
                mbar_wait(&full[slot], (uint32_t)(use & 1));
                const uint32_t sb = slots_u32 + (uint32_t)slot * slot_bytes;
                const uint32_t cb = G4 ? sb + (uint32_t)(lane >> 2) * (uint32_t)a.gstride + (uint32_t)(lane & 3) * (uint32_t)a.stride +
                                             (((lane >> 2) & 1) ? RS_G4_SHIFT * 8u : 0u)
                                       : sb + (uint32_t)mylane * (uint32_t)a.stride;
                const uint32_t xb = G4 ? sb + 8u * (uint32_t)a.gstride : sb + 32u * (uint32_t)a.stride;
                const int n = min(C, a.S - c * C);
                int t = 0;
                for (; t + 8 <= n; t += 8) {
                    double v[8], x[8];
#pragma unroll
                    for (int u = 0; u < 4; ++u) {
                        lds_v2f64(cb + (uint32_t)(t + 2 * u) * 8u, v[2 * u], v[2 * u + 1]);
                        lds_v2f64(xb + (uint32_t)(t + 2 * u) * 8u, x[2 * u], x[2 * u + 1]);
                    }
#pragma unroll
                    for (int u = 0; u < 8; ++u) {
                        const double d = __dsub_rn(v[u], x[u]);
                        acc = __dadd_rn(acc, __dmul_rn(d, d));
                    }
                }
                for (; t < n; t += 2) {
                    double v0, v1, x0, x1;
                    lds_v2f64(cb + (uint32_t)t * 8u, v0, v1);
                    lds_v2f64(xb + (uint32_t)t * 8u, x0, x1);
                    double d = __dsub_rn(v0, x0);
                    acc = __dadd_rn(acc, __dmul_rn(d, d));
                    d = __dsub_rn(v1, x1);
                    acc = __dadd_rn(acc, __dmul_rn(d, d));
                }
                mbar_arrive(&empty[slot]);
            }
            if (lane < cnt) a.sl_d[(size_t)rloc * a.shortcap + gi * 32 + lane] = acc;
        }
    } else {
        const int w = (warp - W) % W, r = (warp - W) / W;
        const bool mine = lane % R == r;
        for (int wave = 0; wave < nwaves; ++wave) {
            const int wact = wave < nfull ? W : nact;
            if (w >= wact) break;
            const int desc = a.grp[(size_t)(wave * W + w) * grid + b];
            const int rloc = desc >> 4, gi = desc & 15;
            const int p = a.sl_p[rloc];
            const int cnt = min(32, p - gi * 32);
            const double* src = nullptr;
            if (!G4 && mine && lane < cnt) src = a.X + (size_t)a.sl_j[(size_t)rloc * a.shortcap + gi * 32 + lane] * a.S;
            int j0 = 0, j1 = 0, j2 = 0, j3 = 0;
            bool issue = false;
            if (G4) {
                j0 = a.sl_j[(size_t)rloc * a.shortcap + gi * 32 + min(lane, cnt - 1)];
                j1 = __shfl_down_sync(0xffffffffu, j0, 1);
                j2 = __shfl_down_sync(0xffffffffu, j0, 2);
                j3 = __shfl_down_sync(0xffffffffu, j0, 3);
                issue = (lane & 3) == 0 && (lane >> 2) % R == r;
            }
            const double* xsrc = a.X + (size_t)(a.row_begin + rloc) * a.S;
            const int k0 = wave * nchunks;
            for (int c = 0; c < nchunks; ++c) {
                const uint32_t bytes = (uint32_t)min(C, a.S - c * C) * 8u;
                const size_t off = (size_t)c * C;
                const int use = (k0 + c) / D, slot = w * D + (k0 + c) - use * D;
                if (use > 0) mbar_wait(&empty[slot], (uint32_t)((use - 1) & 1));
                const uint32_t sb = slots_u32 + (uint32_t)slot * slot_bytes;
                if (G4) {
                    if (r == 0 && lane == 0) {
                        mbar_arrive_expect_tx(&full[slot], 32u * (uint32_t)a.stride + bytes);
                        bulk_g2s(sb + 8u * (uint32_t)a.gstride, xsrc + off, bytes, &full[slot]);
                    }
                    if (issue) {
                        const int q = lane >> 2;
                        tma_gather4(sb + (uint32_t)q * (uint32_t)a.gstride, &xmap, c * C - ((q & 1) ? RS_G4_SHIFT : 0), j0, j1, j2, j3, &full[slot]);
                    }
                } else {
                    if (r == 0 && lane == 0) {
                        mbar_arrive_expect_tx(&full[slot], (uint32_t)(cnt + 1) * bytes);
                        bulk_g2s(sb + 32u * (uint32_t)a.stride, xsrc + off, bytes, &full[slot]);
                    }
                    if (src != nullptr) bulk_g2s(sb + (uint32_t)lane * (uint32_t)a.stride, src + off, bytes, &full[slot]);
                }
            }
        }
    }
    (void)row_bytes;
}

struct RankArgs {
    int rows, k, shortcap;
    const int* sl_j;
    const double* sl_d;
    const int* sl_p;
    const int* row_cs;
    const int* row_ce;
    int row_begin;
    int* idx_out;
    double* dist_out;
};
constexpr int RK_WARPS = 8;

__device__ __forceinline__ unsigned pair_less96(u64 a, int ja, u64 b, int jb) {
    unsigned r;
    asm("{\n"
        ".reg .u32 t;\n"
        "sub.cc.u32 t, %1, %4;\n"
        "subc.cc.u32 t, %2, %5;\n"
        "subc.cc.u32 t, %3, %6;\n"
        "subc.u32 %0, 0, 0;\n"
        "}\n"
        : "=r"(r)
        : "r"((unsigned)ja), "r"((unsigned)(a & 0xffffffffu)), "r"((unsigned)(a >> 32)), "r"((unsigned)jb),
          "r"((unsigned)(b & 0xffffffffu)), "r"((unsigned)(b >> 32)));
    return r;
}

template <int EPL, int STRIDE>
__device__ __forceinline__ void rank_step(u64 (&key)[EPL], int (&bin)[EPL], int lane, int size) {
#pragma unroll
    for (int t = 0; t < EPL; ++t) {
        const int e = t * 32 + lane;
        const bool up = (e & size) == 0;
        if (STRIDE >= 32) {
            const int t2 = t ^ (STRIDE >> 5);
            if (t2 > t) {
                const bool less2 = pair_less96(key[t2], bin[t2], key[t], bin[t]) != 0u;
                if (less2 == up) {
                    const u64 tk = key[t]; key[t] = key[t2]; key[t2] = tk;
                    const int tb = bin[t]; bin[t] = bin[t2]; bin[t2] = tb;
                }
            }
        } else {
            const u64 ok = __shfl_xor_sync(0xffffffffu, key[t], STRIDE);
            const int ob = __shfl_xor_sync(0xffffffffu, bin[t], STRIDE);
            const bool want_min = ((lane & STRIDE) == 0) == up;
            const bool other_less = pair_less96(ok, ob, key[t], bin[t]) != 0u;
            if (other_less == want_min) { key[t] = ok; bin[t] = ob; }
        }
    }
}

template <int EPL>
__device__ __forceinline__ void rank_sort(u64 (&key)[EPL], int (&bin)[EPL], int lane) {
#pragma unroll 1
    for (int size = 2; size <= 32 * EPL; size <<= 1) {
        if (EPL >= 16 && size > 256) rank_step<EPL, (EPL >= 16 ? 256 : 1)>(key, bin, lane, size);
        if (EPL >= 8 && size > 128) rank_step<EPL, (EPL >= 8 ? 128 : 1)>(key, bin, lane, size);
        if (EPL >= 4 && size > 64) rank_step<EPL, (EPL >= 4 ? 64 : 1)>(key, bin, lane, size);
        if (EPL >= 2 && size > 32) rank_step<EPL, (EPL >= 2 ? 32 : 1)>(key, bin, lane, size);
        if (size > 16) rank_step<EPL, 16>(key, bin, lane, size);
        if (size > 8) rank_step<EPL, 8>(key, bin, lane, size);
        if (size > 4) rank_step<EPL, 4>(key, bin, lane, size);
        if (size > 2) rank_step<EPL, 2>(key, bin, lane, size);
        rank_step<EPL, 1>(key, bin, lane, size);
    }
}

template <int EPL>
__device__ __forceinline__ void rank_row(const RankArgs& a, int rloc, int p, int lane) {
    u64 key[EPL];
    int bin[EPL];
    int nvalid = 0;
#pragma unroll
    for (int t = 0; t < EPL; ++t) {
        const int e = t * 32 + lane;
        key[t] = ~0ull;
        bin[t] = 0x7fffffff;
        if (e < p) {
            const double d = a.sl_d[(size_t)rloc * a.shortcap + e];
            const bool ok = d < 1e10;
            if (ok) { key[t] = (u64)__double_as_longlong(d); bin[t] = a.sl_j[(size_t)rloc * a.shortcap + e]; }
            nvalid += ok ? 1 : 0;
        }
    }
#pragma unroll
    for (int o = 16; o > 0; o >>= 1) nvalid += __shfl_xor_sync(0xffffffffu, nvalid, o);
    rank_sort<EPL>(key, bin, lane);
    const int row = a.row_begin + rloc;
    const int cs = a.row_cs[row], ce = a.row_ce[row];
    int* out_i = a.idx_out + (size_t)rloc * a.k;
    double* out_d = a.dist_out + (size_t)rloc * a.k;
    const int nout = nvalid < a.k ? nvalid : a.k;
#pragma unroll
    for (int t = 0; t < EPL; ++t) {
        const int e = t * 32 + lane;
        if (e < nout) {
            out_i[e] = bin[t] >= ce ? bin[t] - (ce - cs) : bin[t];
            out_d[e] = __longlong_as_double((long long)key[t]);
        }
    }
    for (int e = nvalid + lane; e < a.k; e += 32) { out_i[e] = -1; out_d[e] = 1e10; }
}

__global__ void __launch_bounds__(RK_WARPS * 32) wc_fin_rank_kernel(const RankArgs a) {
    const int lane = threadIdx.x & 31, warp = threadIdx.x >> 5;
    const int rloc = blockIdx.x * RK_WARPS + warp;
    if (rloc >= a.rows) return;
    const int p = a.sl_p[rloc];
    if (p < 0) return;
    if (p <= 128) rank_row<4>(a, rloc, p, lane);
    else if (p <= 256) rank_row<8>(a, rloc, p, lane);
    else rank_row<16>(a, rloc, p, lane);
}

template <int W, int R>
static int launch_rescore(const RescoreArgs& ra, const CUtensorMap& xmap, bool g4, int grid, size_t smem, cudaStream_t stream) {
    if (g4) {
        WC_CUDA(cudaFuncSetAttribute(wc_fin_rescore_kernel<W, R, true>, cudaFuncAttributeMaxDynamicSharedMemorySize, (int)smem));
        wc_fin_rescore_kernel<W, R, true><<<grid, (W + W * R) * 32, smem, stream>>>(xmap, ra);
        return WC_OK;
    }
    WC_CUDA(cudaFuncSetAttribute(wc_fin_rescore_kernel<W, R, false>, cudaFuncAttributeMaxDynamicSharedMemorySize, (int)smem));
    wc_fin_rescore_kernel<W, R, false><<<grid, (W + W * R) * 32, smem, stream>>>(xmap, ra);
    return WC_OK;
}

static int launch_finalize(wc_ctx* ctx, cudaStream_t stream, FinArgs fa, int rows, bool wide, long long* launches) {
    const size_t fin_smem = (size_t)FIN_ECAP * 12 + (size_t)fa.shortcap * 12 + HIST_BINS * 4;
    const bool split = ctx->k6_split != 0 && fa.S % 2 == 0 && fa.S >= 8 && (reinterpret_cast<uintptr_t>(fa.X) & 15) == 0 && rows > 0;
    fa.sl_j = nullptr; fa.sl_p = nullptr; fa.grp = nullptr; fa.grp_count = nullptr; fa.row_list = nullptr; fa.row_count = nullptr; fa.stats = nullptr;
    ctx->k6_stats_d = nullptr;
    ctx->phase_ms[10] = 0.0;
    ctx->timed_mask &= ~(1u << 10);
    if (!split) {
        if (wide) {
            WC_CUDA(cudaFuncSetAttribute(wc_finalize_kernel<160, false>, cudaFuncAttributeMaxDynamicSharedMemorySize, (int)fin_smem));
            wc_finalize_kernel<160, false><<<rows, 160, fin_smem, stream>>>(fa);
        } else {
            WC_CUDA(cudaFuncSetAttribute(wc_finalize_kernel<FIN_THREADS, false>, cudaFuncAttributeMaxDynamicSharedMemorySize, (int)fin_smem));
            wc_finalize_kernel<FIN_THREADS, false><<<rows, FIN_THREADS, fin_smem, stream>>>(fa);
        }
        WC_CUDA(cudaGetLastError());
        *launches = 1;
        return WC_OK;
    }
    int rc;
    double* sl_d;
    const int gpr = fa.shortcap / 32;
    if ((rc = wc_reserve(ctx, SLOT_FIN_J, (size_t)rows * fa.shortcap * sizeof(int), (void**)&fa.sl_j))) return rc;
    if ((rc = wc_reserve(ctx, SLOT_FIN_D, (size_t)rows * fa.shortcap * sizeof(double), (void**)&sl_d))) return rc;
    fa.sl_k = reinterpret_cast<u64*>(sl_d);
    if ((rc = wc_reserve(ctx, SLOT_FIN_P, (2 * (size_t)rows + 8 + FIN_BUCKETS) * sizeof(int), (void**)&fa.sl_p))) return rc;
    if ((rc = wc_reserve(ctx, SLOT_FIN_GRP, (size_t)rows * (gpr + 1) * sizeof(int), (void**)&fa.grp))) return rc;
    fa.grp_count = fa.sl_p + rows;
    int* big_count = fa.sl_p + rows + 1;
    int* stats = fa.sl_p + rows + 2;
    fa.sl_b = fa.sl_p + rows + 8;
    fa.bkt_hist = fa.sl_b + rows;
    fa.bkt_shift = 0;
    while (((fa.N - 1) >> fa.bkt_shift) >= FIN_BUCKETS) ++fa.bkt_shift;
    WC_CUDA(cudaMemsetAsync(fa.bkt_hist, 0, FIN_BUCKETS * sizeof(int), stream));
    int* big_list = fa.grp + (size_t)rows * gpr;
    WC_CUDA(cudaMemsetAsync(fa.grp_count, 0, 5 * sizeof(int), stream));
    fa.row_list = nullptr; fa.row_count = nullptr; fa.stats = stats;
    if (ctx->k6_select != 0) {
        wc_fin_select_hist_kernel<<<(rows + SELH_WARPS - 1) / SELH_WARPS, SELH_WARPS * 32, 0, stream>>>(fa, big_list, big_count, stats);
    } else {
        const size_t sel_smem = SEL_WARPS * SEL_WARP_STRIDE;
        WC_CUDA(cudaFuncSetAttribute(wc_fin_select_kernel, cudaFuncAttributeMaxDynamicSharedMemorySize, (int)sel_smem));
        wc_fin_select_kernel<<<(rows + SEL_WARPS - 1) / SEL_WARPS, SEL_WARPS * 32, sel_smem, stream>>>(fa, big_list, big_count, stats);
    }
    WC_CUDA(cudaGetLastError());
    {
        fa.row_list = big_list; fa.row_count = big_count;
        const int g = std::min(rows, 8 * ctx->sm_count);
        if (wide) {
            WC_CUDA(cudaFuncSetAttribute(wc_finalize_kernel<160, true>, cudaFuncAttributeMaxDynamicSharedMemorySize, (int)fin_smem));
            wc_finalize_kernel<160, true><<<g, 160, fin_smem, stream>>>(fa);
        } else {
            WC_CUDA(cudaFuncSetAttribute(wc_finalize_kernel<FIN_THREADS, true>, cudaFuncAttributeMaxDynamicSharedMemorySize, (int)fin_smem));
            wc_finalize_kernel<FIN_THREADS, true><<<g, FIN_THREADS, fin_smem, stream>>>(fa);
        }
        WC_CUDA(cudaGetLastError());
    }
    wc_fin_bucket_scan_kernel<<<1, FIN_BUCKETS, 0, stream>>>(fa.bkt_hist, fa.grp_count);
    wc_fin_bucket_scatter_kernel<<<(rows + 255) / 256, 256, 0, stream>>>(rows, fa.sl_p, fa.sl_b, fa.bkt_hist, fa.grp);
    WC_CUDA(cudaGetLastError());
    WC_CUDA(cudaEventRecord(ctx->ev[20], stream));
    RescoreArgs ra;
    ra.X = fa.X; ra.S = fa.S; ra.row_begin = fa.row_begin; ra.shortcap = fa.shortcap; ra.sl_j = fa.sl_j; ra.sl_d = sl_d;
    ra.sl_p = fa.sl_p; ra.grp = fa.grp; ra.grp_count = fa.grp_count;
    const int W = ctx->k6_warps > 0 ? ctx->k6_warps : 4;
    const int R = ctx->k6_prod > 0 ? ctx->k6_prod : 2;
    bool g4 = ctx->k6_g4 != 0 && ctx->encode_tiled != nullptr && fa.S >= 64 && fa.N >= 4;
    int C = ctx->k6_chunk > 0 ? ctx->k6_chunk : (g4 ? 86 : 100);
    CUtensorMap xmap;
    memset(&xmap, 0, sizeof(xmap));
    size_t slot_bytes = 0;
    if (g4) {
        const int nch = (fa.S + C - 1) / C;
        C = (fa.S + nch - 1) / nch;
        C += C & 1;
        if ((((C + RS_G4_SHIFT) / 2) & 1) == 0) C += 2;
        const int cbox = C + RS_G4_SHIFT;
        if (cbox > 256) g4 = false;
        else {
            ra.C = C;
            ra.nchunks = (fa.S + C - 1) / C;
            ra.stride = cbox * 8;
            ra.gstride = (4 * ra.stride + 127) / 128 * 128;
            ra.slot_bytes = 8 * ra.gstride + (C * 8 + 127) / 128 * 128;
            slot_bytes = (size_t)ra.slot_bytes;
            cuuint64_t dims[2] = {(cuuint64_t)fa.S, (cuuint64_t)fa.N};
            cuuint64_t strides[1] = {(cuuint64_t)fa.S * sizeof(double)};
            cuuint32_t box[2] = {(cuuint32_t)cbox, 1};
            cuuint32_t estr[2] = {1, 1};
            CUresult r = reinterpret_cast<PFN_encodeTiled>(ctx->encode_tiled)(
                &xmap, CU_TENSOR_MAP_DATA_TYPE_FLOAT64, 2, const_cast<double*>(fa.X), dims, strides, box, estr, CU_TENSOR_MAP_INTERLEAVE_NONE,
                CU_TENSOR_MAP_SWIZZLE_NONE, CU_TENSOR_MAP_L2_PROMOTION_L2_256B, CU_TENSOR_MAP_FLOAT_OOB_FILL_NONE);
            if (r != CUDA_SUCCESS) g4 = false;
        }
    }
    if (!g4) {
        C = ctx->k6_chunk > 0 ? ctx->k6_chunk : 100;
        C = std::max(4, std::min(C & ~3, 480));
        if (C > fa.S) C = (fa.S + 3) & ~3;
        ra.C = C;
        ra.nchunks = (fa.S + C - 1) / C;
        ra.stride = C * 8 + 16;
        ra.gstride = 0; ra.slot_bytes = 0;
        slot_bytes = (size_t)33 * ra.stride;
    }
    ra.nslot = (int)std::min<size_t>(RS_MAX_SLOTS, ((size_t)226 * 1024 - RS_HEADER) / slot_bytes);
    if (ra.nslot < 2 * W) { wc_set_error("K6: chunk of %d samples leaves %d ring slots for %d consumer warps", C, ra.nslot, W); return WC_ERR_ARG; }
    ra.nslot = ra.nslot / W * W;
    const size_t smem = RS_HEADER + (size_t)ra.nslot * slot_bytes;
    const int grid = ctx->sm_count;
    if (W == 2 && R == 4) rc = launch_rescore<2, 4>(ra, xmap, g4, grid, smem, stream);
    else if (W == 2 && R == 8) rc = launch_rescore<2, 8>(ra, xmap, g4, grid, smem, stream);
    else if (W == 4 && R == 1) rc = launch_rescore<4, 1>(ra, xmap, g4, grid, smem, stream);
    else if (W == 4 && R == 2) rc = launch_rescore<4, 2>(ra, xmap, g4, grid, smem, stream);
    else if (W == 4 && R == 4) rc = launch_rescore<4, 4>(ra, xmap, g4, grid, smem, stream);
    else if (W == 4 && R == 7) rc = launch_rescore<4, 7>(ra, xmap, g4, grid, smem, stream);
    else if (W == 8 && R == 1) rc = launch_rescore<8, 1>(ra, xmap, g4, grid, smem, stream);
    else if (W == 8 && R == 2) rc = launch_rescore<8, 2>(ra, xmap, g4, grid, smem, stream);
    else if (W == 8 && R == 3) rc = launch_rescore<8, 3>(ra, xmap, g4, grid, smem, stream);
    else { wc_set_error("K6: no kernel for %d consumer warps x %d producer warps each", W, R); return WC_ERR_ARG; }
    if (rc) return rc;
    WC_CUDA(cudaGetLastError());
    WC_CUDA(cudaEventRecord(ctx->ev[21], stream));
    RankArgs ka;
    ka.rows = rows; ka.k = fa.k; ka.shortcap = fa.shortcap; ka.sl_j = fa.sl_j; ka.sl_d = sl_d; ka.sl_p = fa.sl_p;
    ka.row_cs = fa.row_cs; ka.row_ce = fa.row_ce; ka.row_begin = fa.row_begin; ka.idx_out = fa.idx_out; ka.dist_out = fa.dist_out;
    wc_fin_rank_kernel<<<(rows + RK_WARPS - 1) / RK_WARPS, RK_WARPS * 32, 0, stream>>>(ka);
    WC_CUDA(cudaGetLastError());
    ctx->timed_mask |= 1u << 10;
    ctx->k6_stats_d = big_count;
    *launches = 6;
    return WC_OK;
}
```

### wisecondor_b200/csrc/wc_search_shard.cuh

```cuda
#pragma once

namespace {

struct ShardDims { int nb, bp, b0, b1, row0, row1, rows_per, in_cap, frac; size_t thr_len; };

ShardDims shard_dims(const wc_ctx* ctx, int N, int k, int world, int rank) {
    ShardDims d;
    d.frac = (ctx != nullptr && ctx->k5_sym >= 2) ? ctx->k5_sym : 8;
    d.nb = (N + BM - 1) / BM;
    d.bp = (d.nb + world - 1) / world;
    d.b0 = std::min(d.nb, rank * d.bp);
    d.b1 = std::min(d.nb, d.b0 + d.bp);
    d.row0 = std::min(N, d.b0 * BM);
    d.row1 = std::min(N, d.b1 * BM);
    d.rows_per = d.bp * BM;
    d.thr_len = (size_t)world * d.rows_per + BN;
    const int want = world == 1 ? 2 * k * d.frac : (4 * k * d.frac + world - 1) / world;
    d.in_cap = 256;
    while (d.in_cap < want) d.in_cap *= 2;
    return d;
}

int shard_launch_pass(wc_ctx* ctx, int pass, unsigned long long* thr_d, unsigned long long* in_key_d, int* in_j_d,
                      int* in_cnt_d, cudaStream_t stream, const std::vector<int>* seg_first = nullptr, int pivots = 0) {
// ... 36 lines not shown
    ta.nkc = pl.nkc; ta.nd_last = pl.nd_last; ta.extra_h = pl.extra_h;
    ta.rb_skip_lo = d_meta; ta.rb_skip_n = d_meta + nrb1; ta.nrb = pl.nrb;
    ta.cta_piece_begin = pass == 0 ? d_ctaA : d_ctaB;
    ta.pieces = d_pieces;
    ta.cand_key = static_cast<u64*>(ctx->buf[SLOT_CAND_D].p); ta.cand_j = static_cast<int*>(ctx->buf[SLOT_CAND_J].p);
    ta.seg_cnt = static_cast<int*>(ctx->buf[SLOT_SEGCNT].p); ta.seg_flag = static_cast<int*>(ctx->buf[SLOT_SEGFLAG].p);
    ta.cap = pl.cap; ta.k = pl.k; ta.mcoef = pl.mcoef; ta.tau_init = pl.f16 ? 3e38 : 1e10 * (1.0 + 1e-6);
    ta.prof = nullptr; ta.trace = nullptr;
    ta.row_thr = thr_d + pl.row0;
    ta.col_thr = thr_d;
    ta.lag = ctx->k5_lag; ta.nstages = pl.nstages;
    ta.tile_list = pass == 0 ? d_listA : d_listB;
    ta.rb_list_off = pass == 0 ? d_offA : d_offB;
    ta.final_prune = 1;
    ta.in_key = in_key_d; ta.in_j = in_j_d; ta.in_cnt = in_cnt_d; ta.in_cap = pl.in_cap;
    ta.madd_p = nullptr;
    ta.kb_last = pl.f16 ? (pl.f16 == 2 ? pl.ldh : pl.ldh - BKH) : 0;
    ta.madd = pl.madd; ta.n32 = pl.f16 ? static_cast<float*>(ctx->buf[SLOT_N32].p) : nullptr;
    ta.dbg = nullptr; ta.dbg_ld = 0; ta.coln32 = ta.n32; ta.col_ids = nullptr;
    const bool tc = pl.f16 == 2;
    if (pass == 2)
        return tc_pivot_pass(ctx, stream, tmap, ta, static_cast<const __half*>(ctx->buf[SLOT_XC].p), pl.ldh, pl.f16 == 2 ? pl.ldh + BKH : pl.ldh, pl.N, pl.nrb, *seg_first, pivots);
    if (tc) {
        auto kern = pass == 0 ? wc_dist_topk_tc_kernel<0, false> : wc_dist_topk_tc_kernel<1, false>;
        WC_CUDA(cudaFuncSetAttribute(kern, cudaFuncAttributeMaxDynamicSharedMemorySize, (int)pl.smem));
        kern<<<pass == 0 ? pl.gridA : pl.gridB, TC_THREADS, pl.smem, stream>>>(tmap, tmap, ta);
        WC_CUDA(cudaGetLastError());
        return WC_OK;
    }
    auto kernel = pass == 0 ? (pl.f16 ? wc_dist_topk_f16_kernel<false> : wc_dist_topk_kernel<false>)
                            : (pl.f16 ? wc_dist_topk_f16_kernel<true> : wc_dist_topk_kernel<true>);
    WC_CUDA(cudaFuncSetAttribute(kernel, cudaFuncAttributeMaxDynamicSharedMemorySize, (int)pl.smem));
    kernel<<<pass == 0 ? pl.gridA : pl.gridB, TOPK_THREADS, pl.smem, stream>>>(tmap, ta);
    WC_CUDA(cudaGetLastError());
    return WC_OK;
}

}

extern "C" int wc_newref_shard_dims(const wc_ctx* ctx, int N, int refsize, int world, int rank, long long* out6) {
    WC_CHECK_ARG(out6 != nullptr);
    WC_CHECK_ARG(N > 0 && refsize >= 1 && refsize <= 384 && world >= 1 && rank >= 0 && rank < world);
    const ShardDims d = shard_dims(ctx, N, refsize, world, rank);
    out6[0] = d.rows_per; out6[1] = d.in_cap; out6[2] = (long long)d.thr_len; out6[3] = d.row0; out6[4] = d.row1; out6[5] = d.nb;
    return WC_OK;
}

extern "C" int wc_newref_shard_begin(wc_ctx* ctx, const double* corrected_d, int N, int S, const int* chrom_bins_h,
                                     int nchrom, int refsize, int rank, int world, unsigned long long* thr_d,
                                     void* stream_v) {
    WC_CHECK_ARG(ctx != nullptr && corrected_d != nullptr && chrom_bins_h != nullptr && thr_d != nullptr);
    WC_CHECK_ARG(N > 0 && S > 0 && nchrom > 0 && refsize >= 1 && refsize <= 384);
    WC_CHECK_ARG(world >= 1 && rank >= 0 && rank < world);
    long long tot = 0;
    for (int c = 0; c < nchrom; ++c) {
        WC_CHECK_ARG(chrom_bins_h[c] >= 0);
        tot += chrom_bins_h[c];
    }
    WC_CHECK_ARG(tot == N);
    cudaStream_t stream = static_cast<cudaStream_t>(stream_v);
    WC_CUDA(cudaSetDevice(ctx->device));
    wc_shard_plan& pl = ctx->shard;
    pl = wc_shard_plan();
    ctx->sched_hash = 0;
    for (int i = 0; i < 4; ++i) ctx->phase_ms[i] = 0.0;
    ctx->phase_ms[8] = ctx->phase_ms[9] = 0.0;
    for (int i = 0; i < 5; ++i) ctx->counter[i] = 0;
    ctx->timed_mask &= ~0xfu;

    const ShardDims d = shard_dims(ctx, N, refsize, world, rank);
    const int k = refsize;
    const int cap = k <= 128 ? 512 : 1024;
    const int nblocks = (S + 7) / 8;
    const int Sx = nblocks * 8;
    const int nkc = nblocks / 2 + 1;
    const int nd_last = nblocks - 2 * (nkc - 1);
    const int ld = nkc * BK;
    const size_t Npad = (size_t)(N + BN - 1) / BN * BN + BN;
    const int nb = d.nb, nrb = d.b1 - d.b0;

    std::vector<int> row_cs(N), row_ce(N), skip_lo(nb), skip_n(nb);
    {
        int pos = 0;
        for (int c = 0; c < nchrom; ++c) {
            for (int i = 0; i < chrom_bins_h[c]; ++i) { row_cs[pos + i] = pos; row_ce[pos + i] = pos + chrom_bins_h[c]; }
            pos += chrom_bins_h[c];
        }
    }
    long long tiles_plain = 0;
    for (int I = 0; I < nb; ++I) {
        const int r0 = I * BM, r1 = std::min(N, r0 + BM) - 1;
        int lo = nb, n = 0;
        if (row_cs[r0] == row_cs[r1]) {
            const int first = (row_cs[r0] + BN - 1) / BN, last = row_ce[r0] / BN;
            if (last > first) { lo = first; n = last - first; }
        }
        skip_lo[I] = lo;
        skip_n[I] = n;
        if (I >= d.b0 && I < d.b1) tiles_plain += nb - n;
    }
    std::vector<int> listA, listB, offA, offB;
    pair_lists(nb, skip_lo, skip_n, d.frac, d.b0, d.b1, listA, offA, listB, offB);
    const long long tilesA = (long long)listA.size(), tilesB = (long long)listB.size();
    const int gridA = tilesA ? (int)std::max(1ll, std::min<long long>(ctx->sm_count, (tilesA + 7) / 8)) : 0;
    const int gridB = tilesB ? (int)std::max(1ll, std::min<long long>(ctx->sm_count, (tilesB + 7) / 8)) : 0;
    std::vector<Piece> pieces;
    if (gridA) schedule_pieces(offA, nrb, gridA, 1, false, 0, pieces);
    if (gridB) {
        const double tile_bytes = (double)BM * ld * sizeof(double);
        const double matrix_bytes = (double)Npad * ld * sizeof(double);
        int G = ctx->k5_group;
        if (G <= 0) {
            G = 1;
            if (matrix_bytes > 64e6)
                while (G < 8 && (double)(gridB / G) * tile_bytes > 48e6) G *= 2;
        }
        schedule_pieces(offB, nrb, gridB, G, matrix_bytes > 64e6 || ctx->k5_group > 0, 1, pieces);
    }
    const int spp = ctx->k5_f16 == 2 ? TC_SEGS_PER_PIECE : 1;
    const int npieces = (int)pieces.size();
    const int nseg = npieces * spp;
    std::vector<int> seg_first(std::max(nrb, 1), 0), seg_count(std::max(nrb, 1), 0), ctaA(gridA + 1, 0), ctaB(gridB + 1, 0);
    std::vector<int> piece_tab((size_t)std::max(npieces, 1) * 5, 0);
    {
        for (const Piece& pc : pieces) seg_count[pc.rb] += spp;
        int run = 0;
        for (int rb = 0; rb < nrb; ++rb) { seg_first[rb] = run; run += seg_count[rb]; }
        std::vector<int> next(seg_first);
        for (Piece& pc : pieces) { pc.seg = next[pc.rb]; next[pc.rb] += spp; }
        std::stable_sort(pieces.begin(), pieces.end(), [](const Piece& x, const Piece& y) {
            return x.pass != y.pass ? x.pass < y.pass : x.cta < y.cta;
        });
        int n0 = 0;
        for (int i = 0; i < npieces; ++i) {
            const Piece& pc = pieces[i];
            if (pc.pass == 0) { ctaA[pc.cta + 1]++; ++n0; } else { ctaB[pc.cta + 1]++; }
            piece_tab[(size_t)i * 5 + 0] = pc.rb;
            piece_tab[(size_t)i * 5 + 1] = pc.q0;
            piece_tab[(size_t)i * 5 + 2] = pc.q1;
            piece_tab[(size_t)i * 5 + 3] = pc.step;
            piece_tab[(size_t)i * 5 + 4] = pc.seg;
        }
        for (int c = 0; c < gridA; ++c) ctaA[c + 1] += ctaA[c];
        ctaB[0] = n0;
        for (int c = 0; c < gridB; ++c) ctaB[c + 1] += ctaB[c];
    }
    const int nrb1 = std::max(nrb, 1);
    std::vector<int> meta;
    meta.insert(meta.end(), (size_t)2 * nrb1, 0);
    meta.insert(meta.end(), seg_first.begin(), seg_first.end());
    meta.insert(meta.end(), seg_count.begin(), seg_count.end());
    meta.insert(meta.end(), ctaA.begin(), ctaA.end());
    meta.insert(meta.end(), ctaB.begin(), ctaB.end());
    meta.insert(meta.end(), piece_tab.begin(), piece_tab.end());
    meta.insert(meta.end(), offA.begin(), offA.end());
    meta.insert(meta.end(), offB.begin(), offB.end());
    meta.insert(meta.end(), listA.begin(), listA.end());
    meta.insert(meta.end(), listB.begin(), listB.end());

    double* Xc; double* norms; int* d_row_cs; int* d_row_ce; int* d_meta;
    u64* cand_key; int* cand_j; int* seg_cnt; int* seg_flag; int* slow;
    int rc;
    if ((rc = wc_reserve(ctx, SLOT_XC, std::max(Npad * ld * sizeof(double), Npad * ((size_t)(S + 4 + 2 * BKH) / BKH * BKH + BKH) * sizeof(__half)), (void**)&Xc))) return rc;
    if ((rc = wc_reserve(ctx, SLOT_NORMS, Npad * sizeof(double), (void**)&norms))) return rc;
    if ((rc = wc_reserve(ctx, SLOT_ROWCS, (size_t)N * sizeof(int), (void**)&d_row_cs))) return rc;
    if ((rc = wc_reserve(ctx, SLOT_ROWCE, (size_t)N * sizeof(int), (void**)&d_row_ce))) return rc;
    if ((rc = wc_reserve(ctx, SLOT_RBMETA, meta.size() * sizeof(int), (void**)&d_meta))) return rc;
    const size_t cand_n = (size_t)std::max(nseg, 1) * BM * cap;
    if ((rc = wc_reserve(ctx, SLOT_CAND_D, cand_n * sizeof(u64), (void**)&cand_key))) return rc;
    if ((rc = wc_reserve(ctx, SLOT_CAND_J, cand_n * sizeof(int), (void**)&cand_j))) return rc;
    if ((rc = wc_reserve(ctx, SLOT_SEGCNT, (size_t)std::max(nseg, 1) * BM * sizeof(int), (void**)&seg_cnt))) return rc;
    if ((rc = wc_reserve(ctx, SLOT_SEGFLAG, (size_t)std::max(nseg, 1) * BM * sizeof(int), (void**)&seg_flag))) return rc;
    const int rows = d.row1 - d.row0;
    if ((rc = wc_reserve(ctx, SLOT_SLOW, ((size_t)std::max(rows, 0) + 1) * sizeof(int), (void**)&slow))) return rc;
    WC_CUDA(cudaMemcpyAsync(d_row_cs, row_cs.data(), (size_t)N * sizeof(int), cudaMemcpyHostToDevice, stream));
    WC_CUDA(cudaMemcpyAsync(d_row_ce, row_ce.data(), (size_t)N * sizeof(int), cudaMemcpyHostToDevice, stream));
    WC_CUDA(cudaMemcpyAsync(d_meta, meta.data(), meta.size() * sizeof(int), cudaMemcpyHostToDevice, stream));
    WC_CUDA(cudaMemsetAsync(slow, 0, sizeof(int), stream));
    WC_CUDA(cudaMemsetAsync(seg_cnt, 0, (size_t)std::max(nseg, 1) * BM * sizeof(int), stream));
    WC_CUDA(cudaMemsetAsync(seg_flag, 0, (size_t)std::max(nseg, 1) * BM * sizeof(int), stream));

    bool f16 = ctx->k5_f16 != 0;
    const bool tcf = ctx->k5_f16 == 2;
    const int ldh = tcf ? (S + 4 + BKH - 1) / BKH * BKH : (S + BKH - 1) / BKH * BKH;
    const int ldx = tcf ? ldh + BKH : ldh;
    double nmax = 0.0;
    WC_CUDA(cudaEventRecord(ctx->ev[0], stream));
    if (f16) {
        float* n32;
        unsigned long long* stats;
        if ((rc = wc_reserve(ctx, SLOT_N32, Npad * sizeof(float), (void**)&n32))) return rc;
        if ((rc = wc_reserve(ctx, SLOT_F16STAT, 2 * sizeof(unsigned long long), (void**)&stats))) return rc;
        WC_CUDA(cudaMemsetAsync(stats, 0, 2 * sizeof(unsigned long long), stream));
        wc_prepare_f16_kernel<<<(int)((Npad * 32 + 255) / 256), 256, 0, stream>>>(corrected_d, N, (int)Npad, S, ldh, ldx, tcf ? 1 : 0,
                                                                                  reinterpret_cast<__half*>(Xc), norms, n32, stats);
        WC_CUDA(cudaGetLastError());
        unsigned long long st_h[2] = {0, 0};
        WC_CUDA(cudaMemcpyAsync(st_h, stats, sizeof(st_h), cudaMemcpyDeviceToHost, stream));
        WC_CUDA(cudaStreamSynchronize(stream));
        memcpy(&nmax, &st_h[0], sizeof(double));
        if (st_h[1] != 0) f16 = false;
    }
    if (!f16)
        wc_prepare_kernel<<<(int)((Npad * 32 + 255) / 256), 256, 0, stream>>>(corrected_d, N, (int)Npad, S, ld, Sx, Xc, norms);
    WC_CUDA(cudaGetLastError());
    WC_CUDA(cudaEventRecord(ctx->ev[1], stream));
    const double eps16 = ldexp(1.0, -10) * (1.0 + ldexp(1.0, -11)) + (tcf ? 2.0 : 1.0) * (double)ldh * ldexp(1.0, -23) +
                         (tcf ? ldexp(1.0, -20) : ldexp(1.0, -21));
    const double tau_init = f16 ? 3e38 : 1e10 * (1.0 + 1e-6);
    wc_fill_u64_kernel<<<(unsigned)((N + 255) / 256), 256, 0, stream>>>(thr_d, (size_t)N, host_key_of_tau(tau_init));
    wc_fill_u64_kernel<<<(unsigned)((d.thr_len - N + 255) / 256), 256, 0, stream>>>(thr_d + N, d.thr_len - (size_t)N, KEY_NEVER);
    WC_CUDA(cudaGetLastError());

    pl.N = N; pl.S = S; pl.k = k; pl.cap = cap; pl.in_cap = d.in_cap; pl.world = world; pl.rank = rank;
    pl.nb = nb; pl.bp = d.bp; pl.b0 = d.b0; pl.b1 = d.b1; pl.row0 = d.row0; pl.row1 = d.row1; pl.rows_per = d.rows_per;
    pl.nkc = nkc; pl.nd_last = nd_last; pl.extra_h = nd_last; pl.ld = ld; pl.nrb = nrb; pl.nseg = npieces;
    pl.gridA = gridA; pl.gridB = gridB; pl.Npad = Npad; pl.nlistA = listA.size();
    pl.tilesA = tilesA; pl.tilesB = tilesB; pl.tiles_plain = tiles_plain;
    pl.f16 = f16 ? ctx->k5_f16 : 0;
    pl.ldh = ldh;
    pl.mcoef = f16 ? 2.0 * eps16 : 16.0 * (double)(S + 16) * 1.1102230246251565e-16;
    pl.madd = f16 ? 2.0 * eps16 * nmax + ldexp(1.0, -20) * sqrt((double)S * nmax) : 0.0;
    if (f16) pl.nkc = ldh / BKH;
    pl.corrected = corrected_d;
    pl.nstages = f16 ? 4 : (cap <= 512 ? 4 : 3);
    pl.smem = f16 && ctx->k5_f16 == 2 ? TC_SMEM_BYTES : f16
        ? (size_t)pl.nstages * STAGE_BYTES + sizeof(TopkState) + (size_t)CONSUMER_WARPS * F16_SCRATCH +
              (size_t)CONSUMER_WARPS * (BN * sizeof(u64) + STG * sizeof(uint4) + (2 * BN + 32) * sizeof(float))
        : (size_t)pl.nstages * STAGE_BYTES + sizeof(TopkState) +
              (size_t)CONSUMER_WARPS * std::max<size_t>((size_t)cap * 12, 8192) +
              (size_t)CONSUMER_WARPS * (BN * sizeof(u64) + STG * sizeof(uint4));
    if (pl.smem > 227 * 1024) { wc_set_error("K5 shared memory %zu exceeds 227 KiB", pl.smem); return WC_ERR_INTERNAL; }

    WC_CUDA(cudaEventRecord(ctx->ev[2], stream));
    pl.pivots = (pl.f16 == 2 && ctx->k5_pivots != 0 && nrb > 0 && nb >= 24) ? pivot_count(N, k) : 0;
    if (pl.pivots > 0) {
        if ((rc = shard_launch_pass(ctx, 2, thr_d, nullptr, nullptr, nullptr, stream, &seg_first, pl.pivots))) return rc;
    }
    if (gridA > 0) {
        if ((rc = shard_launch_pass(ctx, 0, thr_d, nullptr, nullptr, nullptr, stream))) return rc;
    }
    WC_CUDA(cudaEventRecord(ctx->ev[16], stream));
    pl.valid = 1;
    pl.stage = 1;
    return WC_OK;
}

extern "C" int wc_newref_shard_sweep(wc_ctx* ctx, unsigned long long* thr_d, unsigned long long* in_key_d, int* in_j_d,
                                     int* in_cnt_d, void* stream_v) {
    WC_CHECK_ARG(ctx != nullptr && thr_d != nullptr && in_key_d != nullptr && in_j_d != nullptr && in_cnt_d != nullptr);
    wc_shard_plan& pl = ctx->shard;
    if (!pl.valid || pl.stage != 1) { wc_set_error("wc_newref_shard_sweep: call wc_newref_shard_begin first"); return WC_ERR_ARG; }
    cudaStream_t stream = static_cast<cudaStream_t>(stream_v);
    WC_CUDA(cudaSetDevice(ctx->device));
    pl.thr = thr_d;
    WC_CUDA(cudaMemsetAsync(in_cnt_d, 0, (size_t)pl.world * pl.rows_per * sizeof(int), stream));
    WC_CUDA(cudaEventRecord(ctx->ev[18], stream));
    if (pl.gridB > 0) {
        int rc;
        if ((rc = shard_launch_pass(ctx, 1, thr_d, in_key_d, in_j_d, in_cnt_d, stream))) return rc;
    }
    WC_CUDA(cudaEventRecord(ctx->ev[19], stream));
    pl.stage = 2;
    return WC_OK;
}

extern "C" int wc_newref_shard_finish(wc_ctx* ctx, const unsigned long long* recv_key_d, const int* recv_j_d,
                                      const int* recv_cnt_d, int32_t* idx_d, double* dist_d, void* stream_v) {
    WC_CHECK_ARG(ctx != nullptr && recv_key_d != nullptr && recv_j_d != nullptr && recv_cnt_d != nullptr);
    wc_shard_plan& pl = ctx->shard;
    if (!pl.valid || pl.stage != 2) { wc_set_error("wc_newref_shard_finish: call wc_newref_shard_sweep first"); return WC_ERR_ARG; }
    cudaStream_t stream = static_cast<cudaStream_t>(stream_v);
    WC_CUDA(cudaSetDevice(ctx->device));
    pl.stage = 0;
    pl.valid = 0;
    const int rows = pl.row1 - pl.row0;
    int nslow = 0;
    int* d_meta = static_cast<int*>(ctx->buf[SLOT_RBMETA].p);
    int* d_row_cs = static_cast<int*>(ctx->buf[SLOT_ROWCS].p);
    int* d_row_ce = static_cast<int*>(ctx->buf[SLOT_ROWCE].p);
    int* slow = static_cast<int*>(ctx->buf[SLOT_SLOW].p);
    long long launches = 4 + (pl.gridA > 0) + (pl.gridB > 0) + (pl.pivots > 0 ? 3 : 0);
    if (rows > 0) {
        WC_CHECK_ARG(idx_d != nullptr && dist_d != nullptr);
        const int nrb1 = std::max(pl.nrb, 1);
        FinArgs fa;
        fa.X = pl.corrected; fa.N = pl.N; fa.S = pl.S; fa.norms = static_cast<double*>(ctx->buf[SLOT_NORMS].p);
        fa.row_cs = d_row_cs; fa.row_ce = d_row_ce; fa.row_begin = pl.row0; fa.row_end = pl.row1;
        fa.rb_seg_first = d_meta + 2 * nrb1; fa.rb_seg_count = d_meta + 3 * nrb1;
        fa.cand_key = static_cast<u64*>(ctx->buf[SLOT_CAND_D].p); fa.cand_j = static_cast<int*>(ctx->buf[SLOT_CAND_J].p);
        fa.seg_cnt = static_cast<int*>(ctx->buf[SLOT_SEGCNT].p); fa.seg_flag = static_cast<int*>(ctx->buf[SLOT_SEGFLAG].p);
        fa.cap = pl.cap; fa.k = pl.k; fa.shortcap = pl.k <= (pl.f16 ? 96 : 128) ? 256 : 512; fa.mcoef = pl.mcoef;
        fa.idx_out = idx_d; fa.dist_out = dist_d; fa.slow_list = slow + 1; fa.slow_count = slow; fa.slow_bias = 0;
        fa.vec = (pl.S % 4 == 0 && (reinterpret_cast<uintptr_t>(pl.corrected) & 31) == 0) ? 4 : 1;
        fa.in_key = recv_key_d; fa.in_j = recv_j_d; fa.in_cnt = recv_cnt_d; fa.in_cap = pl.in_cap;
        fa.in_nsrc = pl.world; fa.in_src_rows = pl.rows_per; fa.madd = pl.madd; fa.madd_p = nullptr;
        fa.row_thr = pl.thr != nullptr ? pl.thr + pl.row0 : nullptr;
        WC_CUDA(cudaEventRecord(ctx->ev[4], stream));
        long long fin_launches = 0;
        int rcf;
        if ((rcf = launch_finalize(ctx, stream, fa, rows, pl.f16 != 0, &fin_launches))) return rcf;
        launches += fin_launches - 1;
        WC_CUDA(cudaEventRecord(ctx->ev[5], stream));
        int k6_stats[4] = {0, 0, 0, 0};
        WC_CUDA(cudaMemcpyAsync(&nslow, slow, sizeof(int), cudaMemcpyDeviceToHost, stream));
        if (ctx->k6_stats_d != nullptr) WC_CUDA(cudaMemcpyAsync(k6_stats, ctx->k6_stats_d, 4 * sizeof(int), cudaMemcpyDeviceToHost, stream));
        WC_CUDA(cudaStreamSynchronize(stream));
        ctx->counter[8] = k6_stats[1];
        ctx->counter[9] = k6_stats[2];
    ctx->counter[10] = k6_stats[0];
    ctx->counter[11] = k6_stats[3];
        if (nslow > 0) {
            const int batch = 64;
            double* scratch;
            int rc;
            if ((rc = wc_reserve(ctx, SLOT_SCRATCH, (size_t)std::min(nslow, batch) * pl.N * sizeof(double), (void**)&scratch)))
                return rc;
            WC_CUDA(cudaEventRecord(ctx->ev[6], stream));
            for (int off = 0; off < nslow; off += batch) {
                ExhArgs ea;
                ea.X = pl.corrected; ea.N = pl.N; ea.S = pl.S; ea.row_cs = d_row_cs; ea.row_ce = d_row_ce; ea.row_begin = pl.row0;
                ea.slow_list = slow + 1; ea.list_off = off; ea.scratch = scratch; ea.k = pl.k; ea.idx_out = idx_d; ea.dist_out = dist_d;
                wc_exhaustive_kernel<<<std::min(batch, nslow - off), EXH_THREADS, 0, stream>>>(ea);
                ++launches;
            }
            WC_CUDA(cudaGetLastError());
            WC_CUDA(cudaEventRecord(ctx->ev[7], stream));
        }
    }
    WC_CUDA(cudaStreamSynchronize(stream));
    float ms, ms2;
    WC_CUDA(cudaEventElapsedTime(&ms, ctx->ev[0], ctx->ev[1])); ctx->phase_ms[0] = ms;
    WC_CUDA(cudaEventElapsedTime(&ms, ctx->ev[2], ctx->ev[16])); ctx->phase_ms[8] = ms;
    WC_CUDA(cudaEventElapsedTime(&ms2, ctx->ev[18], ctx->ev[19])); ctx->phase_ms[9] = ms2;
    ctx->phase_ms[1] = (double)ms + (double)ms2;
    if (rows > 0) { WC_CUDA(cudaEventElapsedTime(&ms, ctx->ev[4], ctx->ev[5])); ctx->phase_ms[2] = ms; }
    if (nslow > 0) { WC_CUDA(cudaEventElapsedTime(&ms, ctx->ev[6], ctx->ev[7])); ctx->phase_ms[3] = ms; }
    ctx->counter[0] = launches;
    ctx->counter[1] = nslow;
    ctx->counter[2] = pl.tiles_plain;
    ctx->counter[3] = pl.tilesA + pl.tilesB;
    ctx->counter[4] = std::max(pl.gridA, pl.gridB);
    ctx->counter[7] = pl.f16 | (pl.pivots << 4);
    return WC_OK;
}
```

### wisecondor_b200/device.py

```python
import ctypes

import numpy as np

from . import _cabi, _mem
from ._mem import ptr as _ptr, stream_ptr as _stream_ptr, require as _require_cuda

F64, I32, U8 = np.float64, np.int32, np.uint8


def newref_topk(corrected, chrom_bins, row_begin, row_end, refsize, out_idx=None, out_dist=None):
    _require_cuda(corrected, F64, "corrected")
    n, s = corrected.shape
    cb = np.ascontiguousarray(chrom_bins, dtype=np.int32)
    rows = int(row_end) - int(row_begin)
    if out_idx is None:
        out_idx = _mem.empty((max(rows, 0), refsize), I32, like=corrected)
    if out_dist is None:
        out_dist = _mem.empty((max(rows, 0), refsize), F64, like=corrected)
    ctx = _cabi.context(_mem.device_index(corrected))
    rc = _cabi.lib().wc_newref_topk(ctx.handle, _ptr(corrected), n, s, cb.ctypes.data_as(ctypes.c_void_p), len(cb),
                                    int(row_begin), int(row_end), int(refsize), _ptr(out_idx), _ptr(out_dist),
                                    _stream_ptr(corrected))
    _cabi.check(rc)
    return out_idx, out_dist


def newref_topk_host(corrected, chrom_bins, row_begin, row_end, refsize, device=0, out_idx=None, out_dist=None):
    X = np.ascontiguousarray(corrected, dtype=np.float64)
    n, s = X.shape
    cb = np.ascontiguousarray(chrom_bins, dtype=np.int32)
    rows = int(row_end) - int(row_begin)
    idx = np.empty((max(rows, 0), refsize), dtype=np.int32) if out_idx is None else out_idx
    dist = np.empty((max(rows, 0), refsize), dtype=np.float64) if out_dist is None else out_dist
    if idx.shape != (max(rows, 0), refsize) or idx.dtype != np.int32 or not idx.flags.c_contiguous or \
            dist.shape != idx.shape or dist.dtype != np.float64 or not dist.flags.c_contiguous:
        raise _cabi.WisecondorError("out_idx / out_dist must be C-contiguous int32 / float64 arrays of shape rows x refsize")
    ctx = _cabi.context(device)
    rc = _cabi.lib().wc_newref_topk_host(ctx.handle, X.ctypes.data_as(ctypes.c_void_p), n, s,
                                         cb.ctypes.data_as(ctypes.c_void_p), len(cb), int(row_begin), int(row_end),
                                         int(refsize), idx.ctypes.data_as(ctypes.c_void_p),
                                         dist.ctypes.data_as(ctypes.c_void_p))
    _cabi.check(rc)
    return idx, dist


I64 = np.int64


def shard_dims(n, refsize, world, rank, device=0, ctx=None):
    ctx = ctx or _cabi.context(device)
    out = (ctypes.c_longlong * 6)()
    _cabi.check(_cabi.lib().wc_newref_shard_dims(ctx.handle, int(n), int(refsize), int(world), int(rank), out))
    return {"rows_per": int(out[0]), "in_cap": int(out[1]), "thr_len": int(out[2]), "row0": int(out[3]),
            "row1": int(out[4]), "blocks": int(out[5])}


def shard_begin(corrected, chrom_bins, refsize, rank, world, thr, ctx=None):
    _require_cuda(corrected, F64, "corrected")
    _require_cuda(thr, I64, "thr")
    n, s = corrected.shape
    cb = np.ascontiguousarray(chrom_bins, dtype=np.int32)
    ctx = ctx or _cabi.context(_mem.device_index(corrected))
    _cabi.check(_cabi.lib().wc_newref_shard_begin(ctx.handle, _ptr(corrected), n, s, cb.ctypes.data_as(ctypes.c_void_p), len(cb),
                                                  int(refsize), int(rank), int(world), _ptr(thr), _stream_ptr(corrected)))


def shard_sweep(thr, in_key, in_j, in_cnt, ctx=None):
    _require_cuda(thr, I64, "thr")
    _require_cuda(in_key, I64, "in_key")
    _require_cuda(in_j, I32, "in_j")
    _require_cuda(in_cnt, I32, "in_cnt")
    ctx = ctx or _cabi.context(_mem.device_index(thr))
    _cabi.check(_cabi.lib().wc_newref_shard_sweep(ctx.handle, _ptr(thr), _ptr(in_key), _ptr(in_j), _ptr(in_cnt), _stream_ptr(thr)))


def shard_finish(recv_key, recv_j, recv_cnt, out_idx, out_dist, ctx=None):
    _require_cuda(recv_key, I64, "recv_key")
    _require_cuda(recv_j, I32, "recv_j")
    _require_cuda(recv_cnt, I32, "recv_cnt")
    _require_cuda(out_idx, I32, "out_idx")
    _require_cuda(out_dist, F64, "out_dist")
    ctx = ctx or _cabi.context(_mem.device_index(recv_key))
    _cabi.check(_cabi.lib().wc_newref_shard_finish(ctx.handle, _ptr(recv_key), _ptr(recv_j), _ptr(recv_cnt), _ptr(out_idx),
                                                   _ptr(out_dist), _stream_ptr(recv_key)))
    return out_idx, out_dist


def last_search_stats(device=0):
    ctx = _cabi.context(device)
    return {
        "center_norms_ms": ctx.phase_ms(0), "dist_topk_ms": ctx.phase_ms(1), "finalize_ms": ctx.phase_ms(2),
        "dist_topk_first_pass_ms": ctx.phase_ms(8),
        "finalize_rescore_ms": ctx.phase_ms(10),
        "exhaustive_ms": ctx.phase_ms(3), "launches": ctx.counter(0), "exhaustive_rows": ctx.counter(1),
        "tiles": ctx.counter(3), "tiles_plain": ctx.counter(2), "ctas": ctx.counter(4),
        "filter": max(0, ctx.counter(7)) & 3,
        "pivots": max(0, ctx.counter(7)) >> 4,
        "k6_live_entries": ctx.counter(8),
        "k6_shortlisted": ctx.counter(9),
        "k6_live_max": ctx.counter(11),
        "k6_rows_cta_select": ctx.counter(10),
    }


CALL_DTYPE = np.dtype([("sample", np.int32), ("chrom", np.int32), ("x", np.int32), ("y", np.int32), ("z", np.float64)])


def _ints(values):
    arr = np.ascontiguousarray(values, dtype=np.int32)
    return arr, arr.ctypes.data_as(ctypes.c_void_p)


def pad32(b):
    return (int(b) + 31) // 32 * 32


class ReferenceTable(object):

    def __init__(self, indexes, distances, masked_sizes, cutoff, device=0):
        self.masked_sizes = [int(v) for v in masked_sizes]
        self.n, self.k = int(indexes.shape[0]), int(indexes.shape[1])
        self.cutoff = float(cutoff)
        idx = _mem.to_device(np.ascontiguousarray(indexes, dtype=np.int32), device)
        dst = _mem.to_device(np.ascontiguousarray(distances, dtype=np.float64), device)
        self.device = idx.device
        self.table = _mem.empty((self.n, _cabi.lib().wc_table_stride(self.k)), I32, like=idx)
        self.count = _mem.empty((self.n,), I32, like=idx)
        self.rev_off = _mem.empty((self.n + 1,), I32, like=idx)
        self.rev_idx = _mem.empty((self.n, self.table.shape[1]), I32, like=idx)
        cb, cbp = _ints(self.masked_sizes)
        ctx = _cabi.context(_mem.device_index(idx))
        rc = _cabi.lib().wc_test_table(ctx.handle, _ptr(idx), _ptr(dst), self.n, self.k, cbp, len(cb), self.cutoff,
                                       _ptr(self.table), _ptr(self.count), _ptr(self.rev_off), _ptr(self.rev_idx),
                                       _stream_ptr(idx))
        _cabi.check(rc)
        _mem.synchronize(idx)


def test_prep(counts, masked_raw, pca_mean, pca_components, nsamples=None):
    _require_cuda(counts, I32, "counts")
    _require_cuda(masked_raw, I32, "masked_raw")
    b, nraw = counts.shape
    n = masked_raw.shape[0]
    dev = counts
    if pca_components is None:
        ncomp = 0
        pca_mean = pca_components = _mem.empty((0,), F64, like=dev)
    else:
        _require_cuda(pca_mean, F64, "pca_mean")
        _require_cuda(pca_components, F64, "pca_components")
        ncomp = pca_components.shape[0]
    ldb = pad32(b)
    out = _mem.empty((n, ldb), F64, like=dev)
    ctx = _cabi.context(_mem.device_index(dev))
    rc = _cabi.lib().wc_test_prep(ctx.handle, _ptr(counts), b, nraw, _ptr(masked_raw), n, _ptr(pca_mean),
                                  _ptr(pca_components), ncomp, _ptr(out), ldb, _stream_ptr(dev))
    _cabi.check(rc)
    return out


def apply_pca(x, pca_mean, pca_components):
    _require_cuda(x, F64, "x")
    _require_cuda(pca_mean, F64, "pca_mean")
    _require_cuda(pca_components, F64, "pca_components")
    b, n = x.shape
    dev = x
    ldb = pad32(b)
    out = _mem.empty((n, ldb), F64, like=dev)
    ctx = _cabi.context(_mem.device_index(dev))
    rc = _cabi.lib().wc_apply_pca(ctx.handle, _ptr(x), b, n, _ptr(pca_mean), _ptr(pca_components),
                                  pca_components.shape[0], _ptr(out), ldb, _stream_ptr(dev))
    _cabi.check(rc)
    return out


def zscore_batch(test, nsamples, table, z_threshold, repeats, copy_init=None):
    _require_cuda(test, F64, "test")
    if copy_init is not None:
        _require_cuda(copy_init, F64, "copy_init")
        if copy_init.shape != test.shape:
            raise _cabi.WisecondorError("copy_init must have the shape of test")
    n, ldb = test.shape
    b = int(nsamples)
    dev = test
    z = _mem.empty((b, n), F64, like=dev)
    r = _mem.empty((b, n), F64, like=dev)
    sizes = _mem.empty((b, n), I32, like=dev)
    asdef = _mem.empty((b,), F64, like=dev)
    ctx = _cabi.context(_mem.device_index(dev))
    rc = _cabi.lib().wc_zscore_batch(ctx.handle, _ptr(test), _ptr(copy_init) if copy_init is not None else None, n, b, ldb,
                                     _ptr(table.table), _ptr(table.count), _ptr(table.rev_off), _ptr(table.rev_idx), table.k,
                                     float(z_threshold), int(repeats), _ptr(z), _ptr(r), _ptr(sizes), _ptr(asdef),
                                     _stream_ptr(dev))
    _cabi.check(rc)
    return z, r, sizes, asdef


def segment_batch(z, refsizes, masked_sizes, chromosomes, minrefbins, z_threshold, min_search=3, max_calls=256, r=None,
                  mineffectsize=0.0):
    _require_cuda(z, F64, "z")
    _require_cuda(refsizes, I32, "refsizes")
    if mineffectsize != 0:
        _require_cuda(r, F64, "r")
        if r.shape != z.shape:
            raise _cabi.WisecondorError("r must have the shape of z")
    b, n = z.shape
    dev = z
    cb, cbp = _ints(masked_sizes)
    sel, selp = _ints(chromosomes)
    cwz = _mem.empty((b, len(sel)), F64, like=dev)
    cleaned = _mem.empty((b, len(sel)), I32, like=dev)
    ctx = _cabi.context(_mem.device_index(dev))
    while True:
        calls = _mem.empty((b, max_calls * CALL_DTYPE.itemsize), U8, like=dev)
        ncalls = _mem.empty((b,), I32, like=dev)
        rc = _cabi.lib().wc_segment_batch(ctx.handle, _ptr(z), _ptr(r) if r is not None else None, _ptr(refsizes), n, b,
                                          cbp, len(cb), selp, len(sel), int(minrefbins), float(z_threshold),
                                          float(mineffectsize), int(min_search), _ptr(cwz), _ptr(cleaned),
                                          _ptr(calls), _ptr(ncalls), int(max_calls), _stream_ptr(dev))
        if rc != 0 and b"max_calls" in _cabi.lib().wc_last_error() and max_calls < (1 << 16):
            max_calls *= 8
            continue
        _cabi.check(rc)
        break
    nc = _mem.to_host(ncalls)
    raw = _mem.to_host(calls).view(CALL_DTYPE).reshape(b, max_calls)
    rows = [raw[i, :nc[i]] for i in range(b)]
    flat = np.concatenate(rows) if rows else np.zeros(0, dtype=CALL_DTYPE)
    flat = flat[np.lexsort((flat["x"], flat["chrom"], flat["sample"]))]
    return cwz, cleaned, flat


def last_test_stats(device=0):
    ctx = _cabi.context(device)
    pairs = []
    while len(pairs) < 64:
        n = ctx.counter(16 + len(pairs))
        if n < 0:
            break
        pairs.append(int(n))
    return {"prep_ms": ctx.phase_ms(6), "zscore_ms": ctx.phase_ms(4), "segment_ms": ctx.phase_ms(5),
            "zscore_launches": ctx.counter(5), "segment_launches": ctx.counter(6), "zscore_pairs_per_pass": pairs}


def newref_normalize(counts):
    _require_cuda(counts, I32, "counts")
    s, nraw = counts.shape
    dev = counts
    ctx = _cabi.context(_mem.device_index(dev))
    mask_d = _mem.empty((nraw,), U8, like=dev)
    _cabi.check(_cabi.lib().wc_newref_mask(ctx.handle, _ptr(counts), s, nraw, _ptr(mask_d), _stream_ptr(dev)))
    mask = _mem.to_host(mask_d).astype(bool)
    masked_raw = _mem.to_device(np.flatnonzero(mask).astype(np.int32), like=dev)
    n = int(masked_raw.shape[0])
    masked = _mem.empty((n, s), F64, like=dev)
    if n > 0:
        _cabi.check(_cabi.lib().wc_newref_normalize(ctx.handle, _ptr(counts), s, nraw, _ptr(masked_raw), n, _ptr(masked),
                                                    _stream_ptr(dev)))
    return masked, mask


def top_eigenpairs(gram, ncomp):
    s = gram.shape[0]
    try:
        from scipy.linalg import eigh
        w, v = eigh(gram, subset_by_index=[max(0, s - ncomp), s - 1])
    except ImportError:
        w, v = np.linalg.eigh(gram)
        w, v = w[-ncomp:], v[:, -ncomp:]
    order = np.argsort(w)[::-1]
    w, v = w[order], v[:, order]
    return np.ascontiguousarray(v), np.sqrt(np.maximum(w, 0.0))


def pca_fit_apply(masked, ncomp=3):
    _require_cuda(masked, F64, "masked")
    n, s = masked.shape
    dev = masked
    ctx = _cabi.context(_mem.device_index(dev))
    mean = _mem.empty((n,), F64, like=dev)
    gram = _mem.empty((s, s), F64, like=dev)
    _cabi.check(_cabi.lib().wc_pca_gram(ctx.handle, _ptr(masked), n, s, _ptr(mean), _ptr(gram), _stream_ptr(dev)))
    vec, sigma = top_eigenpairs(_mem.to_host(gram), ncomp)
    if not (sigma > 0).all():
        raise _cabi.WisecondorError("PCA: fewer than %d non-zero singular values (degenerate sample matrix)" % ncomp)
    vec_d = _mem.to_device(vec, like=dev)
    comps = _mem.empty((ncomp, n), F64, like=dev)
    corrected = _mem.empty((n, s), F64, like=dev)
    sig = np.ascontiguousarray(sigma, dtype=np.float64)
    _cabi.check(_cabi.lib().wc_pca_apply(ctx.handle, _ptr(masked), n, s, _ptr(mean), _ptr(vec_d),
                                         sig.ctypes.data_as(ctypes.c_void_p), ncomp, _ptr(comps), _ptr(corrected),
                                         _stream_ptr(dev)))
    comps_h = _mem.to_host(comps)
    signs = np.sign(comps_h[np.arange(ncomp), np.argmax(np.abs(comps_h), axis=1)])
    signs[signs == 0] = 1.0
    return corrected, comps_h * signs[:, None], _mem.to_host(mean)
```

Before: 478.4 billion.

## Deduplicate symmetric shortlist pairs in exact rescoring and pack half-warp work items

Shortlists are now sorted per row and a new mark kernel binary-searches each candidate's own shortlist for the reverse pair. When both rows hold the pair, only one owner (picked by parity) rescores it and the result is mirrored to the other row, so symmetric pairs are not rescored twice. Rescore work is also reorganised into 16-entry half groups, with two halves packed per warp and a second target row staged in each smem slot. In exchange this adds a sort and a mark kernel, extra own_j/own_m buffers, binary-search traffic, and more complex mirroring logic in the rescore kernel.

```diff
diff --git a/wisecondor_b200/csrc/wc_common.cuh b/wisecondor_b200/csrc/wc_common.cuh
--- a/wisecondor_b200/csrc/wc_common.cuh
+++ b/wisecondor_b200/csrc/wc_common.cuh
@@ -34,7 +34,7 @@
     size_t bytes = 0;
 };
 
-enum { WC_NBUF = 56, WC_NPHASE = 12, WC_NCOUNTER = 12 };
+enum { WC_NBUF = 56, WC_NPHASE = 12, WC_NCOUNTER = 14 };
 
 enum {
     SLOT_XC = 0, SLOT_NORMS, SLOT_ROWCS, SLOT_ROWCE, SLOT_RBMETA, SLOT_CAND_D, SLOT_CAND_J, SLOT_SEGCNT,
@@ -45,7 +45,7 @@
     SLOT_T_REVCNT = 44, SLOT_T_REVCUR, SLOT_T_DIRTY, SLOT_T_PAIRS,
     SLOT_S_ZC = 32, SLOT_S_META, SLOT_S_STATUS, SLOT_S_RC, SLOT_S_AUX,
     SLOT_P_FIRST = 40,
-    SLOT_FIN_J = 48, SLOT_FIN_D, SLOT_FIN_P, SLOT_FIN_GRP
+    SLOT_FIN_J = 48, SLOT_FIN_D, SLOT_FIN_P, SLOT_FIN_GRP, SLOT_FIN_OWN
 };
 
 struct wc_shard_plan {
diff --git a/wisecondor_b200/csrc/wc_search.cu b/wisecondor_b200/csrc/wc_search.cu
--- a/wisecondor_b200/csrc/wc_search.cu
+++ b/wisecondor_b200/csrc/wc_search.cu
@@ -608,6 +608,54 @@
     return da < db || (da == db && ja < jb);
 }
 
+template <int EPL, int STRIDE>
+__device__ __forceinline__ void bin_sort_step(int (&v)[EPL], int lane, int size) {
+#pragma unroll
+    for (int t = 0; t < EPL; ++t) {
+        const bool up = ((t * 32 + lane) & size) == 0;
+        if (STRIDE >= 32) {
+            const int t2 = t ^ (STRIDE >> 5);
+            if (t2 > t && (v[t2] < v[t]) == up) { const int x = v[t]; v[t] = v[t2]; v[t2] = x; }
+        } else {
+            const int o = __shfl_xor_sync(0xffffffffu, v[t], STRIDE);
+            v[t] = (((lane & STRIDE) == 0) == up) ? min(v[t], o) : max(v[t], o);
+        }
+    }
+}
+
+template <int EPL>
+__device__ __forceinline__ void bin_sort(int (&v)[EPL], int lane) {
+#pragma unroll 1
+    for (int size = 2; size <= 32 * EPL; size <<= 1) {
+        if (EPL >= 16 && size > 256) bin_sort_step<EPL, (EPL >= 16 ? 256 : 1)>(v, lane, size);
+        if (EPL >= 8 && size > 128) bin_sort_step<EPL, (EPL >= 8 ? 128 : 1)>(v, lane, size);
+        if (size > 64) bin_sort_step<EPL, 64>(v, lane, size);
+        if (size > 32) bin_sort_step<EPL, 32>(v, lane, size);
+        if (size > 16) bin_sort_step<EPL, 16>(v, lane, size);
+        if (size > 8) bin_sort_step<EPL, 8>(v, lane, size);
+        if (size > 4) bin_sort_step<EPL, 4>(v, lane, size);
+        if (size > 2) bin_sort_step<EPL, 2>(v, lane, size);
+        bin_sort_step<EPL, 1>(v, lane, size);
+    }
+}
+
+template <int EPL>
+__device__ __forceinline__ void sort_shortlist_n(const int* src, int* dst, int p, int lane) {
+    int v[EPL];
+#pragma unroll
+    for (int t = 0; t < EPL; ++t) v[t] = t * 32 + lane < p ? src[t * 32 + lane] : 0x7fffffff;
+    bin_sort<EPL>(v, lane);
+#pragma unroll
+    for (int t = 0; t < EPL; ++t)
+        if (t * 32 + lane < p) dst[t * 32 + lane] = v[t];
+}
+
+__device__ __forceinline__ void sort_shortlist(const int* src, int* dst, int p, int lane) {
+    if (p <= 128) sort_shortlist_n<4>(src, dst, p, lane);
+    else if (p <= 256) sort_shortlist_n<8>(src, dst, p, lane);
+    else sort_shortlist_n<16>(src, dst, p, lane);
+}
+
 struct FinArgs {
     const double* X;
     int N, S;
@@ -648,8 +696,13 @@
     const int* row_list;
     const int* row_count;
     int* stats;
+    int dedup;
+    int* sl_o;
+    int* own_j;
+    int2* own_m;
     int* sl_b;
     int* bkt_hist;
+    int* bkt_fill;
     int bkt_shift;
 };
 
@@ -810,15 +863,13 @@
         return;
     }
     if (SPLIT) {
-        for (int e = tid; e < p; e += FT) a.sl_j[(size_t)rloc * a.shortcap + e] = ex_j[e];
+        if (a.dedup) {
+            if (warp == 0) sort_shortlist(ex_j, a.sl_j + (size_t)rloc * a.shortcap, p, lane);
+        } else {
+            for (int e = tid; e < p; e += FT) a.sl_j[(size_t)rloc * a.shortcap + e] = ex_j[e];
+        }
         if (tid == 0) {
             a.sl_p[rloc] = p;
-            const int ng = (p + 31) >> 5;
-            int jmin = 0x7fffffff;
-            for (int e = 0; e < p; ++e) jmin = min(jmin, ex_j[e]);
-            const int bkt = min(jmin >> a.bkt_shift, FIN_BUCKETS - 1);
-            a.sl_b[rloc] = bkt;
-            atomicAdd(a.bkt_hist + bkt, ng);
             if (a.stats != nullptr) { atomicAdd(a.stats, total); atomicAdd(a.stats + 1, p); }
         }
         return;
@@ -915,6 +966,15 @@
     for (int b = blockIdx.x; b < n; b += gridDim.x) {
         finalize_row<FT, SPLIT>(a, a.row_list[b], fin_raw);
         __syncthreads();
+    }
+    if (SPLIT && a.dedup) {
+        const int lane = threadIdx.x & 31;
+        const int rows = a.row_end - a.row_begin;
+        for (int r = blockIdx.x * (FT / 32) + (int)(threadIdx.x >> 5); r < rows; r += gridDim.x * (FT / 32)) {
+            if (a.sl_b[r] != 1) continue;
+            int* sl = a.sl_j + (size_t)r * a.shortcap;
+            sort_shortlist(sl, sl, a.sl_p[r], lane);
+        }
     }
 }
 
@@ -1657,9 +1717,9 @@
     }
     WC_CUDA(cudaEventRecord(ctx->ev[5], stream));
 
-    int nslow = 0, k6_stats[4] = {0, 0, 0, 0};
+    int nslow = 0, k6_stats[K6_NSTATS] = {};
     WC_CUDA(cudaMemcpyAsync(&nslow, slow, sizeof(int), cudaMemcpyDeviceToHost, stream));
-    if (ctx->k6_stats_d != nullptr) WC_CUDA(cudaMemcpyAsync(k6_stats, ctx->k6_stats_d, 4 * sizeof(int), cudaMemcpyDeviceToHost, stream));
+    if (ctx->k6_stats_d != nullptr) WC_CUDA(cudaMemcpyAsync(k6_stats, ctx->k6_stats_d, sizeof(k6_stats), cudaMemcpyDeviceToHost, stream));
     unsigned long long f16_flag = 0;
     if (f16_stats_d != nullptr) WC_CUDA(cudaMemcpyAsync(&f16_flag, f16_stats_d + 1, sizeof(f16_flag), cudaMemcpyDeviceToHost, stream));
     WC_CUDA(cudaStreamSynchronize(stream));
@@ -1670,10 +1730,7 @@
         ctx->k5_f16 = keep;
         return rc;
     }
-    ctx->counter[8] = k6_stats[1];
-    ctx->counter[9] = k6_stats[2];
-    ctx->counter[10] = k6_stats[0];
-    ctx->counter[11] = k6_stats[3];
+    set_k6_counters(ctx, k6_stats);
     long long launches = (sym ? 5 : 4) + pivot_launches + fin_launches;
     if (nslow > 0) {
         ctx->d2h_rows_done = 0;
diff --git a/wisecondor_b200/csrc/wc_search_fin.cuh b/wisecondor_b200/csrc/wc_search_fin.cuh
--- a/wisecondor_b200/csrc/wc_search_fin.cuh
+++ b/wisecondor_b200/csrc/wc_search_fin.cuh
@@ -149,30 +149,23 @@
     double window = fmax(dv, 0.0) + a.mcoef * (a.norms[row] + fabs(dv)) + madd_of(a);
     if (!(window > 1e-300)) window = 1e-300;
     const u64 wkey = key_of_tau(window);
-    int p = 0, jmin = 0x7fffffff;
+    int p = 0;
+    int* my_j = a.sl_j + (size_t)rloc * a.shortcap;
 #pragma unroll
     for (int t = 0; t < SEL_EPL; ++t) {
         const bool keep = t * 32 + lane < kept && d[t] <= wkey;
         const unsigned bm = __ballot_sync(0xffffffffu, keep);
         const int pos = p + __popc(bm & ((1u << lane) - 1u));
-        if (keep && pos < a.shortcap) {
-            const int j = en_j[t * 32 + lane];
-            a.sl_j[(size_t)rloc * a.shortcap + pos] = j;
-            jmin = min(jmin, j);
-        }
+        if (keep && pos < a.shortcap) my_j[pos] = en_j[t * 32 + lane];
         p += __popc(bm);
     }
-#pragma unroll
-    for (int o = 16; o > 0; o >>= 1) jmin = min(jmin, __shfl_xor_sync(0xffffffffu, jmin, o));
     if (lane == 0) {
         if (p > a.shortcap) {
             a.slow_list[atomicAdd(a.slow_count, 1)] = rloc + a.slow_bias;
             a.sl_p[rloc] = -1;
         } else {
             a.sl_p[rloc] = p;
-            const int bkt = min(jmin >> a.bkt_shift, FIN_BUCKETS - 1);
-            a.sl_b[rloc] = bkt;
-            atomicAdd(a.bkt_hist + bkt, (p + 31) >> 5);
+            a.sl_b[rloc] = 1;
             if (stats != nullptr) { atomicAdd(stats, kept); atomicAdd(stats + 1, p); atomicMax(stats + 2, kept); }
         }
     }
@@ -353,7 +346,7 @@
     const double dscale = (double)scale;
     u64* my_k = a.sl_k + (size_t)rloc * a.shortcap;
     int* my_j = a.sl_j + (size_t)rloc * a.shortcap;
-    int p = 0, jmin = 0x7fffffff;
+    int p = 0;
     sweep([&](u64 key, int j, bool valid) {
         const bool keep = valid && key <= wkey;
         const unsigned bm = __ballot_sync(0xffffffffu, keep);
@@ -361,7 +354,6 @@
         if (keep && pos < a.shortcap) {
             my_j[pos] = j;
             my_k[pos] = key;
-            jmin = min(jmin, j);
         }
         p += __popc(bm);
         if (refine && keep) {
@@ -388,36 +380,84 @@
             const u64 wkey2 = window_key(fmin(vstar, v2));
             if (wkey2 < wkey) {
                 int q = 0;
-                jmin = 0x7fffffff;
                 for (int e0 = 0; e0 < p; e0 += 32) {
                     const int e = e0 + lane;
                     const bool keep = e < p && __ldcg(my_k + e) <= wkey2;
                     const int j = e < p ? __ldcg(my_j + e) : 0;
                     __syncwarp();
                     const unsigned bm = __ballot_sync(0xffffffffu, keep);
-                    if (keep) {
-                        my_j[q + __popc(bm & ((1u << lane) - 1u))] = j;
-                        jmin = min(jmin, j);
-                    }
+                    if (keep) my_j[q + __popc(bm & ((1u << lane) - 1u))] = j;
                     q += __popc(bm);
                 }
                 p = q;
             }
         }
     }
+    if (lane == 0) {
+        a.sl_p[rloc] = p;
+        a.sl_b[rloc] = 1;
+        if (stats != nullptr) { atomicAdd(stats, kept); atomicAdd(stats + 1, p); atomicMax(stats + 2, kept); }
+    }
+}
+
+constexpr int MK_WARPS = 8;
+
+__global__ void __launch_bounds__(MK_WARPS * 32) wc_fin_mark_kernel(const FinArgs a) {
+    const int lane = threadIdx.x & 31, warp = threadIdx.x >> 5;
+    const int rloc = blockIdx.x * MK_WARPS + warp;
+    const int rows = a.row_end - a.row_begin;
+    if (rloc >= rows) return;
+    const int p = a.sl_p[rloc];
+    const int row = a.row_begin + rloc;
+    const int* my_j = a.sl_j + (size_t)rloc * a.shortcap;
+    int q = 0, jmin = 0x7fffffff;
+    for (int e0 = 0; e0 < p; e0 += 32) {
+        const int e = e0 + lane;
+        bool own = e < p;
+        const int j = own ? my_j[e] : 0;
+        int mirror = -1;
+        if (own && a.dedup && j >= a.row_begin && j < a.row_end) {
+            const int jl = j - a.row_begin;
+            const int pj = a.sl_p[jl];
+            const int* lj = a.sl_j + (size_t)jl * a.shortcap;
+            int lo = 0, hi = pj;
+            while (lo < hi) {
+                const int m = (lo + hi) >> 1;
+                if (lj[m] < row) lo = m + 1; else hi = m;
+            }
+            if (lo < pj && lj[lo] == row) {
+                const int owner = ((row + j) & 1) == 0 ? min(row, j) : max(row, j);
+                if (owner == row) mirror = jl * a.shortcap + lo;
+                else own = false;
+            }
+        }
+        const unsigned bm = __ballot_sync(0xffffffffu, own);
+        if (own) {
+            const size_t o = (size_t)rloc * a.shortcap + q + __popc(bm & ((1u << lane) - 1u));
+            a.own_j[o] = j;
+            a.own_m[o] = make_int2(e, mirror);
+            jmin = min(jmin, j);
+        }
+        q += __popc(bm);
+    }
 #pragma unroll
     for (int o = 16; o > 0; o >>= 1) jmin = min(jmin, __shfl_xor_sync(0xffffffffu, jmin, o));
     if (lane == 0) {
-        a.sl_p[rloc] = p;
-        const int bkt = min(jmin >> a.bkt_shift, FIN_BUCKETS - 1);
-        a.sl_b[rloc] = bkt;
-        atomicAdd(a.bkt_hist + bkt, (p + 31) >> 5);
-        if (stats != nullptr) { atomicAdd(stats, kept); atomicAdd(stats + 1, p); atomicMax(stats + 2, kept); }
-    }
-}
-
-__global__ void __launch_bounds__(FIN_BUCKETS) wc_fin_bucket_scan_kernel(int* __restrict__ hist, int* __restrict__ total) {
+        a.sl_o[rloc] = q;
+        if (q > 0) {
+            const int bkt = min(jmin >> a.bkt_shift, FIN_BUCKETS - 1);
+            a.sl_b[rloc] = bkt;
+            atomicAdd(a.bkt_hist + bkt, (q + 15) >> 4);
+            if (a.stats != nullptr) atomicAdd(a.stats + 3, q);
+        }
+    }
+}
+
+__global__ void __launch_bounds__(FIN_BUCKETS) wc_fin_bucket_scatter_kernel(int rows, const int* __restrict__ sl_o, const int* __restrict__ sl_b,
+                                                                         const int* __restrict__ hist, int* __restrict__ fill,
+                                                                         int* __restrict__ grp, int* __restrict__ total) {
     __shared__ int s_w[32];
+    __shared__ int s_base[FIN_BUCKETS];
     const int tid = threadIdx.x, lane = tid & 31, warp = tid >> 5;
     const int v = hist[tid];
     int incl = v;
@@ -430,19 +470,17 @@
     __syncthreads();
     int base = 0;
     for (int w = 0; w < warp; ++w) base += s_w[w];
-    hist[tid] = base + incl - v;
-    if (tid == FIN_BUCKETS - 1) *total = base + incl;
-}
-
-__global__ void wc_fin_bucket_scatter_kernel(int rows, const int* __restrict__ sl_p, const int* __restrict__ sl_b,
-                                             int* __restrict__ cursor, int* __restrict__ grp) {
-    const int r = blockIdx.x * blockDim.x + threadIdx.x;
+    s_base[tid] = base + incl - v;
+    if (blockIdx.x == 0 && tid == FIN_BUCKETS - 1) *total = base + incl;
+    __syncthreads();
+    const int r = blockIdx.x * FIN_BUCKETS + tid;
     if (r >= rows) return;
-    const int p = sl_p[r];
-    if (p <= 0) return;
-    const int ng = (p + 31) >> 5;
-    const int base = atomicAdd(cursor + sl_b[r], ng);
-    for (int g = 0; g < ng; ++g) grp[base + g] = (r << 4) | g;
+    const int q = sl_o[r];
+    if (q <= 0) return;
+    const int ng = (q + 15) >> 4;
+    const int b = sl_b[r];
+    const int at = s_base[b] + atomicAdd(fill + b, ng);
+    for (int g = 0; g < ng; ++g) grp[at + g] = (r << 5) | g;
 }
 
 struct RescoreArgs {
@@ -450,14 +488,16 @@
     int S;
     int row_begin;
     int shortcap;
-    const int* sl_j;
     double* sl_d;
-    const int* sl_p;
+    const int* sl_o;
+    const int* own_j;
+    const int2* own_m;
     const int* grp;
     const int* grp_count;
     int C;
     int nchunks;
     int stride;
+    int tstride;
     int nslot;
     int gstride;
     int slot_bytes;
@@ -489,33 +529,47 @@
     const int tid = threadIdx.x, lane = tid & 31, warp = tid >> 5;
     const int nslot = a.nslot;
     const int D = nslot / W;
-    const uint32_t slot_bytes = G4 ? (uint32_t)a.slot_bytes : 33u * (uint32_t)a.stride;
+    const uint32_t slot_bytes = G4 ? (uint32_t)a.slot_bytes : 34u * (uint32_t)a.stride;
     if (tid == 0) {
         for (int s = 0; s < nslot; ++s) { mbar_init(&full[s], 1); mbar_init(&empty[s], 32); }
         mbar_fence_init();
         if (G4) tma_prefetch_desc(&xmap);
     }
     __syncthreads();
-    const int ngroups = *a.grp_count;
+    const int nhalf = *a.grp_count;
+    const int nitems = (nhalf + 1) >> 1;
     const int grid = gridDim.x, b = blockIdx.x;
     const int per_wave = W * grid;
-    const int nfull = ngroups / per_wave;
-    const int rem = ngroups - nfull * per_wave;
+    const int nfull = nitems / per_wave;
+    const int rem = nitems - nfull * per_wave;
     const int nact = rem > b ? (rem - b + grid - 1) / grid : 0;
     const int nwaves = nfull + (nact > 0 ? 1 : 0);
     const int nchunks = a.nchunks, C = a.C;
-    const size_t row_bytes = (size_t)a.S * 8;
+    const uint32_t tgt_off = G4 ? 8u * (uint32_t)a.gstride : 32u * (uint32_t)a.stride;
+    struct Half { int rloc, h, cnt, hl; bool real, two; };
+    auto half_of = [&](int item) -> Half {
+        Half x;
+        x.two = 2 * item + 1 < nhalf;
+        const int hh = x.two ? lane >> 4 : 0;
+        const int desc = a.grp[2 * item + hh];
+        x.rloc = desc >> 5;
+        x.h = desc & 31;
+        x.cnt = min(16, a.sl_o[x.rloc] - x.h * 16);
+        x.hl = lane & 15;
+        x.real = (lane >> 4) == hh && x.hl < x.cnt;
+        if (x.hl >= x.cnt) x.hl = x.cnt - 1;
+        x.hl += hh * 16;
+        return x;
+    };
 
     if (warp < W) {
         const int w = warp;
         for (int wave = 0; wave < nwaves; ++wave) {
             const int wact = wave < nfull ? W : nact;
             if (w >= wact) break;
-            const int desc = a.grp[(size_t)(wave * W + w) * grid + b];
-            const int rloc = desc >> 4, gi = desc & 15;
-            const int p = a.sl_p[rloc];
-            const int cnt = min(32, p - gi * 32);
-            const int mylane = lane < cnt ? lane : cnt - 1;
+            const Half x = half_of((wave * W + w) * grid + b);
+            const size_t own = (size_t)x.rloc * a.shortcap + x.h * 16 + (x.hl & 15);
+            const int2 om = x.real ? a.own_m[own] : make_int2(0, -1);
             double acc = 0.0;
             const int k0 = wave * nchunks;
             for (int c = 0; c < nchunks; ++c) {
@@ -524,20 +578,20 @@
                 const uint32_t sb = slots_u32 + (uint32_t)slot * slot_bytes;
                 const uint32_t cb = G4 ? sb + (uint32_t)(lane >> 2) * (uint32_t)a.gstride + (uint32_t)(lane & 3) * (uint32_t)a.stride +
                                              (((lane >> 2) & 1) ? RS_G4_SHIFT * 8u : 0u)
-                                       : sb + (uint32_t)mylane * (uint32_t)a.stride;
-                const uint32_t xb = G4 ? sb + 8u * (uint32_t)a.gstride : sb + 32u * (uint32_t)a.stride;
+                                       : sb + (uint32_t)x.hl * (uint32_t)a.stride;
+                const uint32_t xb = sb + tgt_off + (x.hl >= 16 ? (uint32_t)a.tstride : 0u);
                 const int n = min(C, a.S - c * C);
                 int t = 0;
                 for (; t + 8 <= n; t += 8) {
-                    double v[8], x[8];
+                    double v[8], xx[8];
 #pragma unroll
                     for (int u = 0; u < 4; ++u) {
                         lds_v2f64(cb + (uint32_t)(t + 2 * u) * 8u, v[2 * u], v[2 * u + 1]);
-                        lds_v2f64(xb + (uint32_t)(t + 2 * u) * 8u, x[2 * u], x[2 * u + 1]);
+                        lds_v2f64(xb + (uint32_t)(t + 2 * u) * 8u, xx[2 * u], xx[2 * u + 1]);
                     }
 #pragma unroll
                     for (int u = 0; u < 8; ++u) {
-                        const double d = __dsub_rn(v[u], x[u]);
+                        const double d = __dsub_rn(v[u], xx[u]);
                         acc = __dadd_rn(acc, __dmul_rn(d, d));
                     }
                 }
@@ -552,7 +606,10 @@
                 }
                 mbar_arrive(&empty[slot]);
             }
-            if (lane < cnt) a.sl_d[(size_t)rloc * a.shortcap + gi * 32 + lane] = acc;
+            if (x.real) {
+                a.sl_d[(size_t)x.rloc * a.shortcap + om.x] = acc;
+                if (om.y >= 0) a.sl_d[om.y] = acc;
+            }
         }
     } else {
         const int w = (warp - W) % W, r = (warp - W) / W;
@@ -560,22 +617,22 @@
         for (int wave = 0; wave < nwaves; ++wave) {
             const int wact = wave < nfull ? W : nact;
             if (w >= wact) break;
-            const int desc = a.grp[(size_t)(wave * W + w) * grid + b];
-            const int rloc = desc >> 4, gi = desc & 15;
-            const int p = a.sl_p[rloc];
-            const int cnt = min(32, p - gi * 32);
-            const double* src = nullptr;
-            if (!G4 && mine && lane < cnt) src = a.X + (size_t)a.sl_j[(size_t)rloc * a.shortcap + gi * 32 + lane] * a.S;
+            const Half x = half_of((wave * W + w) * grid + b);
+            const int j = a.own_j[(size_t)x.rloc * a.shortcap + x.h * 16 + (x.hl & 15)];
+            const double* src = !G4 && mine && x.real ? a.X + (size_t)j * a.S : nullptr;
+            const int cnt_b = __shfl_sync(0xffffffffu, x.cnt, 16);
+            const int nrows = x.two ? x.cnt + cnt_b + 2 : x.cnt + 1;
+            const double* xsrc = a.X + (size_t)(a.row_begin + x.rloc) * a.S;
+            const double* xsrc_b = reinterpret_cast<const double*>(__shfl_sync(0xffffffffu, reinterpret_cast<uintptr_t>(xsrc), 16));
             int j0 = 0, j1 = 0, j2 = 0, j3 = 0;
             bool issue = false;
             if (G4) {
-                j0 = a.sl_j[(size_t)rloc * a.shortcap + gi * 32 + min(lane, cnt - 1)];
+                j0 = j;
                 j1 = __shfl_down_sync(0xffffffffu, j0, 1);
                 j2 = __shfl_down_sync(0xffffffffu, j0, 2);
                 j3 = __shfl_down_sync(0xffffffffu, j0, 3);
                 issue = (lane & 3) == 0 && (lane >> 2) % R == r;
             }
-            const double* xsrc = a.X + (size_t)(a.row_begin + rloc) * a.S;
             const int k0 = wave * nchunks;
             for (int c = 0; c < nchunks; ++c) {
                 const uint32_t bytes = (uint32_t)min(C, a.S - c * C) * 8u;
@@ -583,26 +640,22 @@
                 const int use = (k0 + c) / D, slot = w * D + (k0 + c) - use * D;
                 if (use > 0) mbar_wait(&empty[slot], (uint32_t)((use - 1) & 1));
                 const uint32_t sb = slots_u32 + (uint32_t)slot * slot_bytes;
+                if (r == 0 && lane == 0) {
+                    mbar_arrive_expect_tx(&full[slot], G4 ? 32u * (uint32_t)a.stride + (x.two ? 2u : 1u) * bytes : (uint32_t)nrows * bytes);
+                    bulk_g2s(sb + tgt_off, xsrc + off, bytes, &full[slot]);
+                    if (x.two) bulk_g2s(sb + tgt_off + (uint32_t)a.tstride, xsrc_b + off, bytes, &full[slot]);
+                }
                 if (G4) {
-                    if (r == 0 && lane == 0) {
-                        mbar_arrive_expect_tx(&full[slot], 32u * (uint32_t)a.stride + bytes);
-                        bulk_g2s(sb + 8u * (uint32_t)a.gstride, xsrc + off, bytes, &full[slot]);
-                    }
                     if (issue) {
                         const int q = lane >> 2;
                         tma_gather4(sb + (uint32_t)q * (uint32_t)a.gstride, &xmap, c * C - ((q & 1) ? RS_G4_SHIFT : 0), j0, j1, j2, j3, &full[slot]);
                     }
-                } else {
-                    if (r == 0 && lane == 0) {
-                        mbar_arrive_expect_tx(&full[slot], (uint32_t)(cnt + 1) * bytes);
-                        bulk_g2s(sb + 32u * (uint32_t)a.stride, xsrc + off, bytes, &full[slot]);
-                    }
-                    if (src != nullptr) bulk_g2s(sb + (uint32_t)lane * (uint32_t)a.stride, src + off, bytes, &full[slot]);
+                } else if (src != nullptr) {
+                    bulk_g2s(sb + (uint32_t)lane * (uint32_t)a.stride, src + off, bytes, &full[slot]);
                 }
             }
         }
     }
-    (void)row_bytes;
 }
 
 struct RankArgs {
@@ -733,10 +786,22 @@
     return WC_OK;
 }
 
+constexpr int K6_NSTATS = 6;
+
+static void set_k6_counters(wc_ctx* ctx, const int (&s)[K6_NSTATS]) {
+    ctx->counter[8] = s[2];
+    ctx->counter[9] = s[5];
+    ctx->counter[10] = s[1];
+    ctx->counter[11] = s[4];
+    ctx->counter[12] = s[3];
+    ctx->counter[13] = (s[0] + 1) / 2;
+}
+
 static int launch_finalize(wc_ctx* ctx, cudaStream_t stream, FinArgs fa, int rows, bool wide, long long* launches) {
     const size_t fin_smem = (size_t)FIN_ECAP * 12 + (size_t)fa.shortcap * 12 + HIST_BINS * 4;
     const bool split = ctx->k6_split != 0 && fa.S % 2 == 0 && fa.S >= 8 && (reinterpret_cast<uintptr_t>(fa.X) & 15) == 0 && rows > 0;
     fa.sl_j = nullptr; fa.sl_p = nullptr; fa.grp = nullptr; fa.grp_count = nullptr; fa.row_list = nullptr; fa.row_count = nullptr; fa.stats = nullptr;
+    fa.dedup = 0; fa.sl_o = nullptr; fa.own_j = nullptr; fa.own_m = nullptr; fa.bkt_fill = nullptr;
     ctx->k6_stats_d = nullptr;
     ctx->phase_ms[10] = 0.0;
     ctx->timed_mask &= ~(1u << 10);
@@ -754,22 +819,28 @@
     }
     int rc;
     double* sl_d;
-    const int gpr = fa.shortcap / 32;
+    const int hpr = fa.shortcap / 16;
     if ((rc = wc_reserve(ctx, SLOT_FIN_J, (size_t)rows * fa.shortcap * sizeof(int), (void**)&fa.sl_j))) return rc;
     if ((rc = wc_reserve(ctx, SLOT_FIN_D, (size_t)rows * fa.shortcap * sizeof(double), (void**)&sl_d))) return rc;
     fa.sl_k = reinterpret_cast<u64*>(sl_d);
-    if ((rc = wc_reserve(ctx, SLOT_FIN_P, (2 * (size_t)rows + 8 + FIN_BUCKETS) * sizeof(int), (void**)&fa.sl_p))) return rc;
-    if ((rc = wc_reserve(ctx, SLOT_FIN_GRP, (size_t)rows * (gpr + 1) * sizeof(int), (void**)&fa.grp))) return rc;
+    if ((rc = wc_reserve(ctx, SLOT_FIN_P, (3 * (size_t)rows + 8 + 2 * FIN_BUCKETS) * sizeof(int), (void**)&fa.sl_p))) return rc;
+    if ((rc = wc_reserve(ctx, SLOT_FIN_GRP, (size_t)rows * (hpr + 1) * sizeof(int), (void**)&fa.grp))) return rc;
+    if ((rc = wc_reserve(ctx, SLOT_FIN_OWN, (size_t)rows * fa.shortcap * (sizeof(int2) + sizeof(int)), (void**)&fa.own_m))) return rc;
+    fa.own_j = reinterpret_cast<int*>(fa.own_m + (size_t)rows * fa.shortcap);
     fa.grp_count = fa.sl_p + rows;
     int* big_count = fa.sl_p + rows + 1;
     int* stats = fa.sl_p + rows + 2;
     fa.sl_b = fa.sl_p + rows + 8;
-    fa.bkt_hist = fa.sl_b + rows;
+    fa.sl_o = fa.sl_b + rows;
+    fa.bkt_hist = fa.sl_o + rows;
+    fa.bkt_fill = fa.bkt_hist + FIN_BUCKETS;
     fa.bkt_shift = 0;
     while (((fa.N - 1) >> fa.bkt_shift) >= FIN_BUCKETS) ++fa.bkt_shift;
-    WC_CUDA(cudaMemsetAsync(fa.bkt_hist, 0, FIN_BUCKETS * sizeof(int), stream));
-    int* big_list = fa.grp + (size_t)rows * gpr;
-    WC_CUDA(cudaMemsetAsync(fa.grp_count, 0, 5 * sizeof(int), stream));
+    fa.dedup = 2 * (long long)rows >= fa.N && (long long)rows * fa.shortcap <= 0x7fffffffLL ? 1 : 0;
+    WC_CUDA(cudaMemsetAsync(fa.sl_b, 0, (size_t)rows * sizeof(int), stream));
+    WC_CUDA(cudaMemsetAsync(fa.bkt_hist, 0, 2 * FIN_BUCKETS * sizeof(int), stream));
+    int* big_list = fa.grp + (size_t)rows * hpr;
+    WC_CUDA(cudaMemsetAsync(fa.grp_count, 0, 8 * sizeof(int), stream));
     fa.row_list = nullptr; fa.row_count = nullptr; fa.stats = stats;
     if (ctx->k6_select != 0) {
         wc_fin_select_hist_kernel<<<(rows + SELH_WARPS - 1) / SELH_WARPS, SELH_WARPS * 32, 0, stream>>>(fa, big_list, big_count, stats);
@@ -791,13 +862,14 @@
         }
         WC_CUDA(cudaGetLastError());
     }
-    wc_fin_bucket_scan_kernel<<<1, FIN_BUCKETS, 0, stream>>>(fa.bkt_hist, fa.grp_count);
-    wc_fin_bucket_scatter_kernel<<<(rows + 255) / 256, 256, 0, stream>>>(rows, fa.sl_p, fa.sl_b, fa.bkt_hist, fa.grp);
+    wc_fin_mark_kernel<<<(rows + MK_WARPS - 1) / MK_WARPS, MK_WARPS * 32, 0, stream>>>(fa);
+    wc_fin_bucket_scatter_kernel<<<(rows + FIN_BUCKETS - 1) / FIN_BUCKETS, FIN_BUCKETS, 0, stream>>>(rows, fa.sl_o, fa.sl_b, fa.bkt_hist,
+                                                                                                    fa.bkt_fill, fa.grp, fa.grp_count);
     WC_CUDA(cudaGetLastError());
     WC_CUDA(cudaEventRecord(ctx->ev[20], stream));
     RescoreArgs ra;
-    ra.X = fa.X; ra.S = fa.S; ra.row_begin = fa.row_begin; ra.shortcap = fa.shortcap; ra.sl_j = fa.sl_j; ra.sl_d = sl_d;
-    ra.sl_p = fa.sl_p; ra.grp = fa.grp; ra.grp_count = fa.grp_count;
+    ra.X = fa.X; ra.S = fa.S; ra.row_begin = fa.row_begin; ra.shortcap = fa.shortcap; ra.sl_d = sl_d;
+    ra.sl_o = fa.sl_o; ra.own_j = fa.own_j; ra.own_m = fa.own_m; ra.grp = fa.grp; ra.grp_count = fa.grp_count;
     const int W = ctx->k6_warps > 0 ? ctx->k6_warps : 4;
     const int R = ctx->k6_prod > 0 ? ctx->k6_prod : 2;
     bool g4 = ctx->k6_g4 != 0 && ctx->encode_tiled != nullptr && fa.S >= 64 && fa.N >= 4;
@@ -817,7 +889,8 @@
             ra.nchunks = (fa.S + C - 1) / C;
             ra.stride = cbox * 8;
             ra.gstride = (4 * ra.stride + 127) / 128 * 128;
-            ra.slot_bytes = 8 * ra.gstride + (C * 8 + 127) / 128 * 128;
+            ra.tstride = (C * 8 + 127) / 128 * 128;
+            ra.slot_bytes = 8 * ra.gstride + 2 * ra.tstride;
             slot_bytes = (size_t)ra.slot_bytes;
             cuuint64_t dims[2] = {(cuuint64_t)fa.S, (cuuint64_t)fa.N};
             cuuint64_t strides[1] = {(cuuint64_t)fa.S * sizeof(double)};
@@ -836,8 +909,9 @@
         ra.C = C;
         ra.nchunks = (fa.S + C - 1) / C;
         ra.stride = C * 8 + 16;
+        ra.tstride = ra.stride;
         ra.gstride = 0; ra.slot_bytes = 0;
-        slot_bytes = (size_t)33 * ra.stride;
+        slot_bytes = (size_t)34 * ra.stride;
     }
     ra.nslot = (int)std::min<size_t>(RS_MAX_SLOTS, ((size_t)226 * 1024 - RS_HEADER) / slot_bytes);
     if (ra.nslot < 2 * W) { wc_set_error("K6: chunk of %d samples leaves %d ring slots for %d consumer warps", C, ra.nslot, W); return WC_ERR_ARG; }
@@ -863,7 +937,7 @@
     wc_fin_rank_kernel<<<(rows + RK_WARPS - 1) / RK_WARPS, RK_WARPS * 32, 0, stream>>>(ka);
     WC_CUDA(cudaGetLastError());
     ctx->timed_mask |= 1u << 10;
-    ctx->k6_stats_d = big_count;
+    ctx->k6_stats_d = fa.grp_count;
     *launches = 6;
     return WC_OK;
 }
diff --git a/wisecondor_b200/csrc/wc_search_shard.cuh b/wisecondor_b200/csrc/wc_search_shard.cuh
--- a/wisecondor_b200/csrc/wc_search_shard.cuh
+++ b/wisecondor_b200/csrc/wc_search_shard.cuh
@@ -362,14 +362,11 @@
         if ((rcf = launch_finalize(ctx, stream, fa, rows, pl.f16 != 0, &fin_launches))) return rcf;
         launches += fin_launches - 1;
         WC_CUDA(cudaEventRecord(ctx->ev[5], stream));
-        int k6_stats[4] = {0, 0, 0, 0};
+        int k6_stats[K6_NSTATS] = {};
         WC_CUDA(cudaMemcpyAsync(&nslow, slow, sizeof(int), cudaMemcpyDeviceToHost, stream));
-        if (ctx->k6_stats_d != nullptr) WC_CUDA(cudaMemcpyAsync(k6_stats, ctx->k6_stats_d, 4 * sizeof(int), cudaMemcpyDeviceToHost, stream));
+        if (ctx->k6_stats_d != nullptr) WC_CUDA(cudaMemcpyAsync(k6_stats, ctx->k6_stats_d, sizeof(k6_stats), cudaMemcpyDeviceToHost, stream));
         WC_CUDA(cudaStreamSynchronize(stream));
-        ctx->counter[8] = k6_stats[1];
-        ctx->counter[9] = k6_stats[2];
-    ctx->counter[10] = k6_stats[0];
-    ctx->counter[11] = k6_stats[3];
+        set_k6_counters(ctx, k6_stats);
         if (nslow > 0) {
             const int batch = 64;
             double* scratch;
diff --git a/wisecondor_b200/device.py b/wisecondor_b200/device.py
--- a/wisecondor_b200/device.py
+++ b/wisecondor_b200/device.py
@@ -98,6 +98,8 @@
         "pivots": max(0, ctx.counter(7)) >> 4,
         "k6_live_entries": ctx.counter(8),
         "k6_shortlisted": ctx.counter(9),
+        "k6_shortlist_total": ctx.counter(12),
+        "k6_work_items": ctx.counter(13),
         "k6_live_max": ctx.counter(11),
         "k6_rows_cta_select": ctx.counter(10),
     }
```

Measured after the change: 496.7 billion (median of 6 runs). 3.8% higher.
